# liuliu/ccv

Measured on AMD Instinct MI355X. Metric: images/sec fwd+bwd VGG-D 224x224 bs256, higher is better.
Workload: dtype f32 (Winograd-domain / fc GEMMs: exact bf16x3 split, all 9 products, fp32 accumulate); 1 GPU; VGG-D (ccv vgg_d_params, 225x225x3 crop, NHWC) forward+backward+SGD, batch 256 per GPU, random-init weights; global_batch=256, parallelism=dp1, conv_relu=convolution epilogue (NNC_MI355X_CONV_ALGO_FUSE_RELU)

## Files before the change

### ccv_amd/csrc/cmd_conv.cpp

```cpp
#include "gemm_launch.h"
#include "winograd.h"
#include "wino_fused.h"
#include "wino_wgrad_fused.h"
#include "conv_c3.h"

using namespace nnc;

namespace {

static size_t align256(size_t x) { return (x + 255) & ~(size_t)255; }

static thread_local int tl_relu_want = 0, tl_relu_done = 0;
static thread_local int tl_mask_want = 0, tl_mask_done = 0;
static thread_local Image4 tl_mask = { 0, 0, 0, 0, 0, 0, 0, 0, 0 };
static bool mask_fits(const Image4& dst)
{
	const Image4& m = tl_mask;
	return m.p && m.n == dst.n && m.h == dst.h && m.w == dst.w && m.c == dst.c && m.sc == 1 && aligned16(m.p) && m.sw % 4 == 0 && m.sh % 4 == 0 && (m.n == 1 || m.sn % 4 == 0);
}

struct conv_geom_t {
	int N, H, W, C;
	int OH, OW, K;
	int kh, kw, Cg, Kg, groups;
	int sy, sx, pby, pbx, dy, dx;
};

static bool conv_geometry(const ccv_nnc_cmd_t& cmd, const ccv_nnc_hint_t& hint, const Image4& a, const Image4& b, const ccv_nnc_tensor_t* w, conv_geom_t* g)
{
	g->N = a.n; g->H = a.h; g->W = a.w; g->C = a.c;
	g->OH = b.h; g->OW = b.w; g->K = b.c;
	g->groups = cmd.info.convolution.groups > 0 ? cmd.info.convolution.groups : 1;
	g->kh = cmd.info.size.dim[0]; g->kw = cmd.info.size.dim[1];
	if (g->K != cmd.info.convolution.count || g->K % g->groups || g->C % g->groups || a.n != b.n) return false;
	g->Cg = g->C / g->groups; g->Kg = g->K / g->groups;
	g->sy = hint.stride.dim[0] > 0 ? hint.stride.dim[0] : 1;
	g->sx = hint.stride.dim[1] > 0 ? hint.stride.dim[1] : 1;
	g->pby = hint.border.begin[0]; g->pbx = hint.border.begin[1];
	g->dy = cmd.info.convolution.dilation[0] > 1 ? cmd.info.convolution.dilation[0] : 1;
	g->dx = cmd.info.convolution.dilation[1] > 1 ? cmd.info.convolution.dilation[1] : 1;
	(void)w;
	return true;
}

static bool image_fits_int(const Image4& t)
{
	return (long)t.h * t.sh < 0x7fffffffL && (long)t.w * t.sw < 0x7fffffffL && (long)(t.h - 1) * t.sh + (long)(t.w - 1) * t.sw + t.c < 0x7fffffffL;
}

static bool pixel_linear(const Image4& t)
{
	return t.sc == 1 && t.sh == (long)t.w * t.sw && (t.n == 1 || t.sn == (long)t.h * t.sh);
}

static bool conv_pointwise(const conv_geom_t& g, const Image4& in, const Image4& out)
{
	return g.kh == 1 && g.kw == 1 && g.sy == 1 && g.sx == 1 && g.pby == 0 && g.pbx == 0 && g.groups == 1 && g.OH == g.H && g.OW == g.W && pixel_linear(in) && pixel_linear(out)
		&& (long)g.N * g.H * g.W <= 0x7fffffffL;
}

enum { CONV_ALGO_IMPLICIT_GEMM = 0, CONV_ALGO_WINOGRAD = 1, CONV_ALGO_WINOGRAD_FUSED = 2, CONV_ALGO_COUNT = 3 };

static unsigned blocks_exact(const size_t n, const int threads) { return (unsigned)((n + threads - 1) / threads); }

struct wino_plan_t {
	int TH, TW, T;
	size_t u_bytes, v_bytes, m_bytes;
	size_t total() const { return u_bytes + v_bytes + m_bytes; }
};

static bool wino_plan(const conv_geom_t& g, const int dst_h, const int dst_w, const int C_src, const int C_dst, wino_plan_t* p)
{
	if (g.kh != 3 || g.kw != 3 || g.sy != 1 || g.sx != 1 || g.dy != 1 || g.dx != 1 || g.groups != 1) return false;
	if (C_src % 4 || C_dst % 4 || g.pby < 0 || g.pby > 2 || g.pbx < 0 || g.pbx > 2) return false;
	p->TH = (dst_h + 3) / 4; p->TW = (dst_w + 3) / 4;
	const long T = (long)g.N * p->TH * p->TW;
	if (T <= 0 || T * (C_src > C_dst ? C_src : C_dst) > 0x7fffffffL) return false;
	p->T = (int)T;
	p->u_bytes = (sizeof(float) * 36 * (size_t)C_src * C_dst + 255) & ~(size_t)255;
	p->v_bytes = (sizeof(float) * 36 * (size_t)T * C_src + 255) & ~(size_t)255;
	p->m_bytes = (sizeof(float) * 36 * (size_t)T * C_dst + 255) & ~(size_t)255;
	return true;
}

static int wino_slice_images(const int N, const int tiles_per_image, const int C_src, const int C_dst)
{
	const long kb = tune(TUNE_WINO_SLICE_KB);
	if (kb <= 0) return N;
	const double per_image = 36.0 * sizeof(float) * (double)tiles_per_image * (double)(C_src + C_dst);
	long nb = (long)((double)kb * 1024.0 / per_image);
	if (nb < 1) nb = 1;
	return nb > N ? N : (int)nb;
}

template <bool FLIP>
static int conv_wino_run(const char* name, const conv_geom_t& g, const wino_plan_t& p, const Image4& src, const float* w, const float* bias, const Image4& dst, const int pad_y, const int pad_x, const int flags, ccv_nnc_stream_context_t* const ctx)
{
	const int Cs = src.c, Cd = dst.c;
	const int per_image = p.TH * p.TW;
	const int nb = wino_slice_images(g.N, per_image, Cs, Cd);
	const size_t v_bytes = nb == g.N ? p.v_bytes : (sizeof(float) * 36 * (size_t)nb * per_image * Cs + 255) & ~(size_t)255;
	const size_t m_bytes = nb == g.N ? p.m_bytes : (sizeof(float) * 36 * (size_t)nb * per_image * Cd + 255) & ~(size_t)255;
	char* ws = (char*)workspace_of(ctx, p.u_bytes + v_bytes + m_bytes);
	if (!ws) return CCV_NNC_EXEC_OOM;
	float* const U = (float*)ws;
	float* const V = (float*)(ws + p.u_bytes);
	float* const M = (float*)(ws + p.u_bytes + v_bytes);
	hipStream_t stream = stream_of(ctx);
	hipLaunchKernelGGL(HIP_KERNEL_NAME(wino_weight_kernel<FLIP>), dim3(blocks_exact((size_t)Cs * Cd, 256)), dim3(256), 0, stream, w, U, g.K, g.C);
	HIP_ENFORCE(hipGetLastError());
	for (int n0 = 0; n0 < g.N; n0 += nb) {
		const int ns = g.N - n0 < nb ? g.N - n0 : nb;
		const int T = ns * per_image;
		WinoTiles ti;
		ti.TH = p.TH; ti.TW = p.TW; ti.T = T;
		ti.H = src.h; ti.W = src.w; ti.sn = src.sn; ti.sh = src.sh; ti.sw = src.sw; ti.oy = -pad_y; ti.ox = -pad_x; ti.C4 = Cs / 4;
		ti.relu = (!FLIP && tl_relu_want) ? 1 : 0;
		if (ti.relu) tl_relu_done = 1;
		ti.mask = 0; ti.m_sn = ti.m_sh = ti.m_sw = 0;
		ti.d_c4.init(ti.C4); ti.d_tw.init(ti.TW); ti.d_th.init(ti.TH);
		hipLaunchKernelGGL(wino_input_kernel, dim3(blocks_exact((size_t)T * ti.C4, 256)), dim3(256), 0, stream, (const float*)src.p + (long)n0 * src.sn, V, ti);
		HIP_ENFORCE(hipGetLastError());
		MatLoader<true, true> la, lb;
		la.p = V; la.ldr = Cs; la.ldk = 1; la.R = T; la.K = Cs;
		lb.p = U; lb.ldr = Cs; lb.ldk = 1; lb.R = Cd; lb.K = Cs;
		GemmOut out = { M, Cd, 1, 0, 1.f, 0 };
		const int ret = gemm_run(name, la, lb, out, T, Cd, Cs, 36, (long)T * Cs, (long)Cd * Cs, (long)T * Cd, 0L, 1, flags, ctx);
		if (ret != CCV_NNC_EXEC_SUCCESS) return ret;
		ti.H = dst.h; ti.W = dst.w; ti.sn = dst.sn; ti.sh = dst.sh; ti.sw = dst.sw; ti.C4 = Cd / 4;
		ti.d_c4.init(ti.C4);
		if (FLIP && mask_fits(dst)) {
			ti.mask = tl_mask.p + (long)n0 * tl_mask.sn; ti.m_sn = tl_mask.sn; ti.m_sh = tl_mask.sh; ti.m_sw = tl_mask.sw;
			tl_mask_done = 1;
		}
		hipLaunchKernelGGL(wino_output_kernel, dim3(blocks_exact((size_t)T * ti.C4, 256)), dim3(256), 0, stream, (const float*)M, bias, dst.p + (long)n0 * dst.sn, ti);
		HIP_ENFORCE(hipGetLastError());
	}
	return CCV_NNC_EXEC_SUCCESS;
}

struct wino_fused_plan_t {
	int GH, GW, GYn, GXn, groups, KB, CCn;
	size_t uf_bytes;
};

static bool wino_fused_plan(const conv_geom_t& g, const Image4& src, const Image4& dst, wino_fused_plan_t* p)
{
	if (g.kh != 3 || g.kw != 3 || g.sy != 1 || g.sx != 1 || g.dy != 1 || g.dx != 1 || g.groups != 1) return false;
	if (src.c % WF_CC || src.c < 2 * WF_CC || src.sc != 1 || dst.sc != 1 || !aligned16(src.p) || src.sw % 4 || src.sh % 4 || (src.n > 1 && src.sn % 4)) return false;
	if (dst.c % 4 || !aligned16(dst.p) || dst.sw % 4 || dst.sh % 4 || (dst.n > 1 && dst.sn % 4)) return false;
	if (((long)(dst.h - 1) * dst.sh + (long)(dst.w - 1) * dst.sw + dst.c) * 4 >= (long)WF_OOB) return false;
	if (((long)(src.h - 1) * src.sh + (long)(src.w - 1) * src.sw + src.c) * 4 >= (long)WF_OOB) return false;
	const int TH = (dst.h + 3) / 4, TW = (dst.w + 3) / 4;
	static const int shapes[3][2] = { { 4, 4 }, { 2, 8 }, { 8, 2 } };
	long best = -1;
	for (int i = 0; i < 3; i++) {
		const long cover = (long)((TH + shapes[i][0] - 1) / shapes[i][0]) * ((TW + shapes[i][1] - 1) / shapes[i][1]);
		if (best < 0 || cover < best) { best = cover; p->GH = shapes[i][0]; p->GW = shapes[i][1]; }
	}
	p->GYn = (TH + p->GH - 1) / p->GH; p->GXn = (TW + p->GW - 1) / p->GW;
	const long groups = (long)src.n * p->GYn * p->GXn;
	p->KB = (dst.c + WF_KT - 1) / WF_KT; p->CCn = src.c / WF_CC;
	if (groups <= 0 || (groups + 3) / 4 * p->KB > 0x7fffffffL || (size_t)p->CCn * WF_U_FLOATS * 4 > 0xffffffffUL) return false;
	p->groups = (int)groups;
	p->uf_bytes = (sizeof(float) * (size_t)p->KB * p->CCn * WF_U_FLOATS + 255) & ~(size_t)255;
	return true;
}

static size_t wino_fused_scratch_bound(const int Kout, const int Cred)
{
	if (Cred % WF_CC || Kout <= 0) return 0;
	return ((sizeof(float) * (size_t)((Kout + WF_KT - 1) / WF_KT) * (Cred / WF_CC) * WF_U_FLOATS + 255) & ~(size_t)255);
}

static size_t wino_fused_mask_bound(const conv_geom_t& g)
{
	if (!tl_mask_want) return 0;
	const long TH = (g.H + 3) / 4, TW = (g.W + 3) / 4;
	long most = 0;
	static const int shapes[3][2] = { { 4, 4 }, { 2, 8 }, { 8, 2 } };
	for (int i = 0; i < 3; i++) {
		const long cover = ((TH + shapes[i][0] - 1) / shapes[i][0]) * ((TW + shapes[i][1] - 1) / shapes[i][1]);
		if (cover > most) most = cover;
	}
	return (size_t)g.N * most * ((g.C + WF_KT - 1) / WF_KT) * 1024;
}

template <bool FLIP>
static int conv_wino_fused_run(const char* name, const conv_geom_t& g, const wino_fused_plan_t& p, const Image4& src, const float* w, const float* bias, const Image4& dst, const int pad_y, const int pad_x, ccv_nnc_stream_context_t* const ctx)
{
	size_t bits_bytes = FLIP && mask_fits(dst) && (long)p.groups * p.KB <= 0x7fffffffL ? (size_t)p.groups * p.KB * 1024 : 0;
	float* UF = (float*)workspace_of(ctx, p.uf_bytes + bits_bytes);
	if (!UF && bits_bytes) { bits_bytes = 0; UF = (float*)workspace_of(ctx, p.uf_bytes); }
	if (!UF) return CCV_NNC_EXEC_OOM;
	hipStream_t stream = stream_of(ctx);
	unsigned* const bits = bits_bytes ? (unsigned*)((char*)UF + p.uf_bytes) : 0;
	if (bits) {
		const dim3 grid((unsigned)((long)p.groups * p.KB));
		const Image4& m = tl_mask;
		if (p.GH == 4) hipLaunchKernelGGL(HIP_KERNEL_NAME(wino_mask_pack_kernel<4, 4>), grid, dim3(256), 0, stream, (const float*)m.p, m.sn, m.sh, m.sw, bits, dst.h, dst.w, dst.c, p.GYn, p.GXn, p.KB);
		else if (p.GH == 2) hipLaunchKernelGGL(HIP_KERNEL_NAME(wino_mask_pack_kernel<2, 8>), grid, dim3(256), 0, stream, (const float*)m.p, m.sn, m.sh, m.sw, bits, dst.h, dst.w, dst.c, p.GYn, p.GXn, p.KB);
		else hipLaunchKernelGGL(HIP_KERNEL_NAME(wino_mask_pack_kernel<8, 2>), grid, dim3(256), 0, stream, (const float*)m.p, m.sn, m.sh, m.sw, bits, dst.h, dst.w, dst.c, p.GYn, p.GXn, p.KB);
		HIP_ENFORCE(hipGetLastError());
		tl_mask_done = 1;
	}
	const int Kout = dst.c, Cred = src.c;
	hipLaunchKernelGGL(HIP_KERNEL_NAME(wino_weight_frag_kernel<FLIP>), dim3(blocks_exact((size_t)p.KB * WF_KT * Cred, 256)), dim3(256), 0, stream, w, UF, Kout, Cred, g.K, g.C);
	HIP_ENFORCE(hipGetLastError());
	WinoFusedArgs a;
	a.src = src.p; a.dst = dst.p; a.uf = UF; a.bias = bias;
	a.s_sn = src.sn; a.s_sh = src.sh; a.s_sw = src.sw; a.d_sn = dst.sn; a.d_sh = dst.sh; a.d_sw = dst.sw;
	a.H = src.h; a.W = src.w; a.OH = dst.h; a.OW = dst.w; a.pad_y = pad_y; a.pad_x = pad_x;
	a.GYn = p.GYn; a.GXn = p.GXn; a.groups = p.groups; a.C = Cred; a.K = Kout; a.CCn = p.CCn; a.KB = p.KB;
	a.dst_image_bytes = (unsigned)(((long)(dst.h - 1) * dst.sh + (long)(dst.w - 1) * dst.sw + dst.c) * 4);
	a.src_image_bytes = (unsigned)(((long)(src.h - 1) * src.sh + (long)(src.w - 1) * src.sw + src.c) * 4);
	a.uf_kb_bytes = (unsigned)((size_t)p.CCn * WF_U_FLOATS * 4);
	long wgs = tune(TUNE_WINO_FUSED_GRID) > 0 ? tune(TUNE_WINO_FUSED_GRID) : device_cu_count();
	int team = p.KB % 8 == 0 ? 8 : (p.KB % 4 == 0 ? 4 : (p.KB % 2 == 0 ? 2 : 1));
	while (team > 1 && wgs < 8 * team) team >>= 1;
	if (wgs < 8 * team) wgs = 8 * team;
	const unsigned grid = (unsigned)(wgs / (8 * team) * (8 * team));
	a.team = team;
	a.relu = (!FLIP && tl_relu_want) ? 1 : 0;
	if (a.relu) tl_relu_done = 1;
	a.mask_bits = bits;
	note_kernel(name);
	char prof_name[96];
	snprintf(prof_name, sizeof(prof_name), bits ? "%s|nnc::wino_fused_kernel<%d, %d, 0, true>" : "%s|nnc::wino_fused_kernel<%d, %d>", name, p.GH, p.GW);
	const long T = (long)src.n * ((dst.h + 3) / 4) * ((dst.w + 3) / 4);
	ProfScope prof(prof_name, 2.0 * 36.0 * (double)T * Kout * Cred, 0, (int)T, Kout, Cred, 36, 1, stream);
	if (bits) {
		if (p.GH == 4) hipLaunchKernelGGL(HIP_KERNEL_NAME(wino_fused_kernel<4, 4, 0, true>), dim3(grid), dim3(256), 0, stream, a);
		else if (p.GH == 2) hipLaunchKernelGGL(HIP_KERNEL_NAME(wino_fused_kernel<2, 8, 0, true>), dim3(grid), dim3(256), 0, stream, a);
		else hipLaunchKernelGGL(HIP_KERNEL_NAME(wino_fused_kernel<8, 2, 0, true>), dim3(grid), dim3(256), 0, stream, a);
	} else if (p.GH == 4) hipLaunchKernelGGL(HIP_KERNEL_NAME(wino_fused_kernel<4, 4>), dim3(grid), dim3(256), 0, stream, a);
	else if (p.GH == 2) hipLaunchKernelGGL(HIP_KERNEL_NAME(wino_fused_kernel<2, 8>), dim3(grid), dim3(256), 0, stream, a);
	else hipLaunchKernelGGL(HIP_KERNEL_NAME(wino_fused_kernel<8, 2>), dim3(grid), dim3(256), 0, stream, a);
	HIP_ENFORCE(hipGetLastError());
	return CCV_NNC_EXEC_SUCCESS;
}

static bool wino_fused_preferred(const int C_red, const wino_fused_plan_t& p, const Image4& dst)
{
	const long maxc = tune(TUNE_WINO_FUSED_MAX_C);
	if (C_red <= maxc) return true;
	const long tiles = (long)((dst.h + 3) / 4) * ((dst.w + 3) / 4), padded = (long)p.GYn * p.GH * p.GXn * p.GW;
	return C_red <= 2 * maxc && padded * 5 < tiles * 6;
}

struct wino_wgrad_plan_t {
	wino_plan_t t;
	int splits;
	size_t w_bytes, du_bytes, head_bytes, bp_bytes;
	long blocks;
	size_t total() const { return head_bytes + t.v_bytes + w_bytes + du_bytes + bp_bytes; }
};

static bool wino_wgrad_plan(const conv_geom_t& g, wino_wgrad_plan_t* p)
{
	if (!wino_plan(g, g.OH, g.OW, g.C, g.K, &p->t)) return false;
	const long tiles = (long)((g.K + 127) / 128) * ((g.C + 127) / 128) * 36;
	long s = ((long)device_cu_count() * 8 + tiles - 1) / tiles;
	const long max_s = p->t.T / (GEMM_BK * 8);
	if (s > max_s) s = max_s;
	if (s > 64) s = 64;
	p->splits = s <= 1 ? 1 : (int)(((s < 8 ? 8 : s) + 7) & ~7);
	p->w_bytes = p->t.m_bytes;
	p->du_bytes = (sizeof(float) * 36 * (size_t)g.K * g.C + 255) & ~(size_t)255;
	p->head_bytes = p->splits > 1 ? sizeof(float) * 36 * (size_t)g.K * g.C * p->splits : 0;
	const size_t colsum_bound = sizeof(float) * (size_t)device_cu_count() * 4 * g.K;
	if (p->head_bytes < colsum_bound) p->head_bytes = colsum_bound;
	p->head_bytes = (p->head_bytes + 255) & ~(size_t)255;
	p->blocks = ((long)p->t.T * (g.K / 4) + 255) / 256;
	p->bp_bytes = sizeof(float) * (size_t)p->blocks * g.K;
	return true;
}

static int conv_wino_wgrad(const conv_geom_t& g, const wino_wgrad_plan_t& p, const Image4& gr, const Image4& a, float* dw, float* dbias, bool* bias_done, const int flags, ccv_nnc_stream_context_t* const ctx)
{
	char* ws = (char*)workspace_of(ctx, p.total());
	if (!ws) return CCV_NNC_EXEC_OOM;
	float* const V = (float*)(ws + p.head_bytes);
	float* const W = (float*)(ws + p.head_bytes + p.t.v_bytes);
	float* const dU = (float*)(ws + p.head_bytes + p.t.v_bytes + p.w_bytes);
	float* const BP = (float*)(ws + p.head_bytes + p.t.v_bytes + p.w_bytes + p.du_bytes);
	const bool fuse_bias = dbias && 256 % (g.K / 4) == 0;
	const int acc = (flags & CCV_NNC_ACCUMULATE_OUTPUT) ? 1 : 0;
	hipStream_t stream = stream_of(ctx);
	const int per_image = p.t.TH * p.t.TW;
	const int nb = wino_slice_images(g.N, per_image, g.C, g.K);
	for (int n0 = 0; n0 < g.N; n0 += nb) {
		const int ns = g.N - n0 < nb ? g.N - n0 : nb;
		const int T = ns * per_image;
		WinoTiles ti;
		ti.TH = p.t.TH; ti.TW = p.t.TW; ti.T = T;
		ti.H = a.h; ti.W = a.w; ti.sn = a.sn; ti.sh = a.sh; ti.sw = a.sw; ti.oy = -g.pby; ti.ox = -g.pbx; ti.C4 = g.C / 4;
		ti.d_c4.init(ti.C4); ti.d_tw.init(ti.TW); ti.d_th.init(ti.TH);
		hipLaunchKernelGGL(wino_input_kernel, dim3(blocks_exact((size_t)T * ti.C4, 256)), dim3(256), 0, stream, (const float*)a.p + (long)n0 * a.sn, V, ti);
		HIP_ENFORCE(hipGetLastError());
		ti.H = gr.h; ti.W = gr.w; ti.sn = gr.sn; ti.sh = gr.sh; ti.sw = gr.sw; ti.oy = 0; ti.ox = 0; ti.C4 = g.K / 4;
		ti.d_c4.init(ti.C4);
		const long blocks = ((long)T * (g.K / 4) + 255) / 256;
		const float* const grs = (const float*)gr.p + (long)n0 * gr.sn;
		if (fuse_bias) hipLaunchKernelGGL(HIP_KERNEL_NAME(wino_outgrad_kernel<true>), dim3((unsigned)blocks), dim3(256), 0, stream, grs, W, ti, BP);
		else hipLaunchKernelGGL(HIP_KERNEL_NAME(wino_outgrad_kernel<false>), dim3((unsigned)blocks), dim3(256), 0, stream, grs, W, ti, (float*)0);
		HIP_ENFORCE(hipGetLastError());
		MatLoader<false, true> la, lb;
		la.p = W; la.ldr = 1; la.ldk = g.K; la.R = g.K; la.K = T;
		lb.p = V; lb.ldr = 1; lb.ldk = g.C; lb.R = g.C; lb.K = T;
		GemmOut out = { dU, g.C, 1, 0, 1.f, n0 > 0 ? 1 : 0 };
		int splits = p.splits;
		if (nb < g.N) {
			const long max_s = T / (GEMM_BK * 8);
			if (splits > max_s) splits = max_s <= 1 ? 1 : (int)(max_s & ~7L);
			if (splits < 8) splits = 1;
		}
		const int ret = gemm_run("conv_wgrad_wino", la, lb, out, g.K, g.C, T, 36, (long)T * g.K, (long)T * g.C, (long)g.K * g.C, 0L, splits, flags, ctx);
		if (ret != CCV_NNC_EXEC_SUCCESS) return ret;
		if (fuse_bias) {
			const int r = colsum_f32(BP, blocks, g.K, g.K, dbias, acc || n0 > 0, ctx);
			if (r != CCV_NNC_EXEC_SUCCESS) return r;
		}
	}
	hipLaunchKernelGGL(wino_wgrad_final_kernel, dim3(blocks_exact((size_t)g.K * g.C, 256)), dim3(256), 0, stream, (const float*)dU, dw, g.K, g.C, acc);
	HIP_ENFORCE(hipGetLastError());
	if (bias_done) *bias_done = fuse_bias;
	return CCV_NNC_EXEC_SUCCESS;
}

struct wino_wgrad_fused_plan_t {
	int TH, TW, GYn, GXn, groups, kblocks, cblocks, slices, per_slice;
	size_t partial_bytes, bias_bytes, du_bytes;
	size_t total() const { return partial_bytes + bias_bytes + du_bytes; }
};
static bool wino_wgrad_fused_plan(const conv_geom_t& g, wino_wgrad_fused_plan_t* p)
{
	if (g.kh != 3 || g.kw != 3 || g.sy != 1 || g.sx != 1 || g.dy != 1 || g.dx != 1 || g.groups != 1) return false;
	if (g.C % WG_CB || g.K % WG_KB || g.pby < 0 || g.pby > 2 || g.pbx < 0 || g.pbx > 2) return false;
	p->TH = (g.OH + 3) / 4; p->TW = (g.OW + 3) / 4;
	p->GYn = (p->TH + WG_GH - 1) / WG_GH; p->GXn = (p->TW + WG_GW - 1) / WG_GW;
	const long groups = (long)g.N * p->GYn * p->GXn;
	if (groups <= 0 || groups > 0x7fffffffL) return false;
	p->groups = (int)groups;
	p->kblocks = g.K / WG_KB; p->cblocks = g.C / WG_CB;
	const long nb = (long)p->kblocks * p->cblocks;
	long s = (device_cu_count() / nb) & ~7L;
	if (s < 8) s = 8;
	while (s > 8 && (groups + s - 1) / s < 8) s -= 8;
	p->slices = (int)s;
	p->per_slice = (int)((groups + s - 1) / s);
	p->partial_bytes = (sizeof(float) * 36 * (size_t)s * g.K * g.C + 255) & ~(size_t)255;
	p->bias_bytes = (sizeof(float) * 4 * (size_t)s * g.K + 255) & ~(size_t)255;
	p->du_bytes = (sizeof(float) * 36 * (size_t)g.K * g.C + 255) & ~(size_t)255;
	return true;
}
static bool wino_wgrad_fused_images_ok(const Image4& a, const Image4& gr, const float* dw)
{
	const auto ok = [](const Image4& t) { return t.sc == 1 && aligned16(t.p) && t.sw % 4 == 0 && t.sh % 4 == 0 && (t.n == 1 || t.sn % 4 == 0) && ((long)(t.h - 1) * t.sh + (long)(t.w - 1) * t.sw + t.c) * 4 < 0x7ffff000L; };
	return ok(a) && ok(gr) && dw != 0;
}
static bool wino_wgrad_fused_preferred(const conv_geom_t& g)
{
	const long m = tune(TUNE_WINO_WGRAD_FUSED_MAX);
	return m > 0 && g.C <= m && g.K <= m;
}
static int conv_wino_wgrad_fused(const conv_geom_t& g, const wino_wgrad_fused_plan_t& p, const Image4& gr, const Image4& a, float* dw, float* dbias, bool* bias_done, const int flags, ccv_nnc_stream_context_t* const ctx)
{
	char* const ws = (char*)workspace_of(ctx, p.total());
	if (!ws) return CCV_NNC_EXEC_OOM;
	hipStream_t stream = stream_of(ctx);
	WinoWgradFusedArgs k;
	k.a = a.p; k.g = gr.p; k.partial = (float*)ws; k.bias_partial = dbias ? (float*)(ws + p.partial_bytes) : 0;
	k.a_sn = a.sn; k.a_sh = a.sh; k.a_sw = a.sw; k.g_sn = gr.sn; k.g_sh = gr.sh; k.g_sw = gr.sw;
	k.H = a.h; k.W = a.w; k.OH = gr.h; k.OW = gr.w; k.pad_y = g.pby; k.pad_x = g.pbx;
	k.GYn = p.GYn; k.GXn = p.GXn; k.groups = p.groups; k.C = g.C; k.K = g.K; k.kblocks = p.kblocks; k.cblocks = p.cblocks;
	k.slices = p.slices; k.per_slice = p.per_slice;
	k.a_image_bytes = (unsigned)(((long)(a.h - 1) * a.sh + (long)(a.w - 1) * a.sw + a.c) * 4);
	k.g_image_bytes = (unsigned)(((long)(gr.h - 1) * gr.sh + (long)(gr.w - 1) * gr.sw + gr.c) * 4);
	note_kernel("conv_wgrad_wino_fused");
	{
		const long T = (long)g.N * p.TH * p.TW;
		ProfScope prof("conv_wgrad_wino_fused|nnc::wino_wgrad_fused_kernel", 2.0 * 36.0 * (double)T * g.K * g.C, 0, g.K, g.C, (int)T, 36, p.slices, stream);
		hipLaunchKernelGGL(HIP_KERNEL_NAME(wino_wgrad_fused_kernel<0>), dim3((unsigned)(p.slices * p.kblocks * p.cblocks)), dim3(256), 0, stream, k);
		HIP_ENFORCE(hipGetLastError());
	}
	const long n = 36L * g.K * g.C;
	const int acc = (flags & CCV_NNC_ACCUMULATE_OUTPUT) ? 1 : 0;
	float* const dU = (float*)(ws + p.partial_bytes + p.bias_bytes);
	hipLaunchKernelGGL(wino_wgrad_fused_fold_kernel, dim3(blocks_exact((size_t)n, 256)), dim3(256), 0, stream, (const float*)k.partial, (const float*)k.bias_partial, dU, dbias, n, g.K, p.slices, acc);
	HIP_ENFORCE(hipGetLastError());
	hipLaunchKernelGGL(wino_wgrad_final_kernel, dim3(blocks_exact((size_t)g.K * g.C, 256)), dim3(256), 0, stream, (const float*)dU, dw, g.K, g.C, acc);
	HIP_ENFORCE(hipGetLastError());
	if (bias_done) *bias_done = dbias != 0;
	return CCV_NNC_EXEC_SUCCESS;
}

static bool wino_images_ok(const Image4& src, const Image4& dst, const float* w, const float* bias)
{
	return src.sc == 1 && dst.sc == 1 && aligned16(src.p) && aligned16(dst.p) && aligned16(w) && (!bias || aligned16(bias)) &&
		src.sw % 4 == 0 && src.sh % 4 == 0 && (src.n == 1 || src.sn % 4 == 0) && dst.sw % 4 == 0 && dst.sh % 4 == 0 && (dst.n == 1 || dst.sn % 4 == 0);
}

static bool wino_preferred(const wino_plan_t& p, const int C_src, const int C_dst)
{
	return C_src >= 32 && C_dst >= 32 && p.T >= 32;
}

static bool conv_c3_ok(const conv_geom_t& g, const Image4& a, const Image4& b)
{
	if (g.C != 3 || g.kh != 3 || g.kw != 3 || g.sy < 1 || g.sx < 1 || g.sy > 4 || g.sx > 4 || g.dy != 1 || g.dx != 1 || g.groups != 1) return false;
	if (g.K != 16 && g.K != 32 && g.K != 64) return false;
	if (a.sc != 1 || a.sw != 3 || b.sc != 1 || !aligned16(b.p) || b.sw % 4 || b.sh % 4 || (b.n > 1 && b.sn % 4)) return false;
	if ((long)a.h * a.sh >= 0x7fffffffL) return false;
	if (((long)(b.h - 1) * b.sh + (long)(b.w - 1) * b.sw + b.c) * 4 >= 0x7ffff000L) return false;
	return (long)b.n * b.h * ((b.w + 15) / 16) < 0x7fffffffL;
}
static void conv_c3_args(const conv_geom_t& g, const Image4& a, const float* w, const float* bias, const Image4& b, ConvC3Args* c)
{
	c->a = a.p; c->w = w; c->bias = bias; c->b = b.p;
	c->a_sn = a.sn; c->a_sh = a.sh; c->b_sn = b.sn; c->b_sh = b.sh; c->b_sw = b.sw;
	c->N = g.N; c->H = g.H; c->W = g.W; c->OH = g.OH; c->OW = g.OW; c->K = g.K; c->pad_y = g.pby; c->pad_x = g.pbx; c->sy = g.sy; c->sx = g.sx;
	c->groups_per_row = (g.OW + 15) / 16; c->groups = g.N * g.OH * c->groups_per_row;
	c->d_gpr.init(c->groups_per_row); c->d_oh.init(g.OH);
	c->b_image_bytes = (unsigned)((((long)b.h - 1) * b.sh + ((long)b.w - 1) * b.sw + b.c) * 4);
}
static int conv_c3_forw(const conv_geom_t& g, const Image4& a, const float* w, const float* bias, const Image4& b, ccv_nnc_stream_context_t* const ctx)
{
	ConvC3Args c;
	conv_c3_args(g, a, w, bias, b, &c);
	c.relu = tl_relu_want ? 1 : 0;
	if (c.relu) tl_relu_done = 1;
	hipStream_t stream = stream_of(ctx);
	const long want = ((long)c.groups + 3) / 4, cap = (long)device_cu_count() * 8;
	const unsigned grid = (unsigned)(want < cap ? want : cap);
	note_kernel("conv_fwd_c3");
	ProfScope prof("conv_fwd_c3|nnc::conv3x3_c3_fwd_kernel", 2.0 * g.N * g.OH * g.OW * (double)g.K * 27, 0, g.N * g.OH * g.OW, g.K, 27, 1, 1, stream);
	if (g.K == 64) hipLaunchKernelGGL(HIP_KERNEL_NAME(conv3x3_c3_fwd_kernel<4>), dim3(grid), dim3(256), 0, stream, c);
	else if (g.K == 32) hipLaunchKernelGGL(HIP_KERNEL_NAME(conv3x3_c3_fwd_kernel<2>), dim3(grid), dim3(256), 0, stream, c);
	else hipLaunchKernelGGL(HIP_KERNEL_NAME(conv3x3_c3_fwd_kernel<1>), dim3(grid), dim3(256), 0, stream, c);
	HIP_ENFORCE(hipGetLastError());
	return CCV_NNC_EXEC_SUCCESS;
}
static size_t conv_c3_wgrad_scratch_bound(const int K) { return sizeof(float) * (size_t)device_cu_count() * 4 * 4 * K * 32; }
static int conv_c3_wgrad(const conv_geom_t& g, const Image4& gr, const Image4& a, float* dw, float* dbias, const int flags, ccv_nnc_stream_context_t* const ctx)
{
	ConvC3Args c;
	conv_c3_args(g, a, 0, 0, gr, &c);
	const long want = ((long)c.groups + 3) / 4, cap = (long)device_cu_count() * 4;
	const unsigned grid = (unsigned)(want < cap ? want : cap);
	const int waves = (int)grid * 4;
	float* const part = (float*)workspace_of(ctx, sizeof(float) * (size_t)waves * g.K * 32);
	if (!part) return CCV_NNC_EXEC_OOM;
	hipStream_t stream = stream_of(ctx);
	note_kernel("conv_wgrad_c3");
	{
		ProfScope prof("conv_wgrad_c3|nnc::conv3x3_c3_wgrad_kernel", 2.0 * g.N * g.OH * g.OW * (double)g.K * 27, 0, g.K, 27, g.N * g.OH * g.OW, 1, 1, stream);
		if (g.K == 64) hipLaunchKernelGGL(HIP_KERNEL_NAME(conv3x3_c3_wgrad_kernel<4>), dim3(grid), dim3(256), 0, stream, c, part);
		else if (g.K == 32) hipLaunchKernelGGL(HIP_KERNEL_NAME(conv3x3_c3_wgrad_kernel<2>), dim3(grid), dim3(256), 0, stream, c, part);
		else hipLaunchKernelGGL(HIP_KERNEL_NAME(conv3x3_c3_wgrad_kernel<1>), dim3(grid), dim3(256), 0, stream, c, part);
	}
	HIP_ENFORCE(hipGetLastError());
	hipLaunchKernelGGL(convc3_wgrad_fold, dim3((unsigned)g.K), dim3(256), 0, stream, (const float*)part, (int)grid , g.K, dw, dbias, (flags & CCV_NNC_ACCUMULATE_OUTPUT) ? 1 : 0);
	HIP_ENFORCE(hipGetLastError());
	return CCV_NNC_EXEC_SUCCESS;
}

static int conv_forw_nhwc(const conv_geom_t& g, const Image4& a, const float* w, const float* bias, const Image4& b, const int algo, const int flags, ccv_nnc_stream_context_t* const ctx)
{
	if (a.sc != 1 || !pixel_linear(b) || !image_fits_int(a)) return CCV_NNC_EXEC_INVALID;
	if (algo != CONV_ALGO_IMPLICIT_GEMM && conv_c3_ok(g, a, b)) return conv_c3_forw(g, a, w, bias, b, ctx);
	wino_plan_t wp;
	wino_fused_plan_t fp;
	if (algo != CONV_ALGO_IMPLICIT_GEMM && algo != CONV_ALGO_WINOGRAD && g.pby <= 2 && g.pbx <= 2 && g.pby >= 0 && g.pbx >= 0 && wino_fused_plan(g, a, b, &fp) && (algo == CONV_ALGO_WINOGRAD_FUSED || wino_fused_preferred(g.C, fp, b))) {
		const int r = conv_wino_fused_run<false>("conv_fwd_wino_fused", g, fp, a, w, bias, b, g.pby, g.pbx, ctx);
		if (r != CCV_NNC_EXEC_OOM) return r;
	}
	if (algo != CONV_ALGO_IMPLICIT_GEMM && wino_plan(g, g.OH, g.OW, g.C, g.K, &wp) && wino_images_ok(a, b, w, bias) && (algo >= CONV_ALGO_WINOGRAD || wino_preferred(wp, g.C, g.K))) {
		const int r = conv_wino_run<false>("conv_fwd_wino", g, wp, a, w, bias, b, g.pby, g.pbx, flags, ctx);
		if (r != CCV_NNC_EXEC_OOM) return r;
	}
	const long M = (long)g.N * g.OH * g.OW;
	const int Kred = g.kh * g.kw * g.Cg;
	if (M > 0x7fffffffL) return CCV_NNC_EXEC_INVALID;
	const bool vec = (g.Cg % 4 == 0) && aligned16(a.p) && aligned16(w) && a.sw % 4 == 0 && a.sh % 4 == 0 && (a.n == 1 || a.sn % 4 == 0);
	GemmOut out = { b.p, b.sw, 1, bias, 1.f, 0 };
	if (vec && conv_pointwise(g, a, b)) {
		MatLoader<true, true> la, lb;
		la.p = a.p; la.ldr = a.sw; la.ldk = 1; la.R = (int)M; la.K = g.C;
		lb.p = w; lb.ldr = g.C; lb.ldk = 1; lb.R = g.K; lb.K = g.C;
		return gemm_run("conv_fwd_pointwise", la, lb, out, (int)M, g.K, g.C, 1, 0L, 0L, 0L, 0L, 1, flags, ctx);
	}
	KOrder ko;
	if (g.kh * g.kw > 1 && g.Cg % GEMM_BK == 0) ko.init(g.kh * g.kw, g.Cg);
#define CONV_FWD(VEC, INC) do { \
		Im2colKC<VEC, false, INC> la; \
		la.p = a.p; la.s_n = a.sn; la.s_h = (int)a.sh; la.s_w = (int)a.sw; la.H = g.H; la.W = g.W; \
		la.OW = g.OW; la.OHW = g.OH * g.OW; la.M = (int)M; la.C = g.Cg; la.KWC = g.kw * g.Cg; la.K = Kred; \
		la.my = g.sy; la.mx = g.sx; la.oy_off = -g.pby; la.ox_off = -g.pbx; la.ty = g.dy; la.tx = g.dx; la.dv_y = 1; la.dv_x = 1; \
		MatLoader<true, VEC> lb; \
		lb.p = w; lb.ldr = Kred; lb.ldk = 1; lb.R = g.Kg; lb.K = Kred; \
		return gemm_run("conv_fwd", la, lb, out, (int)M, g.Kg, Kred, g.groups, (long)g.Cg, (long)g.Kg * Kred, (long)g.Kg, (long)g.Kg, 1, flags, ctx, ko); \
	} while (0)
	if (vec) CONV_FWD(true, false);
	else CONV_FWD(false, false);
#undef CONV_FWD
}

static __global__ void __launch_bounds__(256) parity_filter_kernel(const float* __restrict__ w, float* __restrict__ f, const int K, const int C, const int kh, const int kw, const int ny, const int nx, const int ky_max, const int kx_max, const size_t total)
{
	for (size_t idx = (size_t)blockIdx.x * blockDim.x + threadIdx.x; idx < total; idx += (size_t)gridDim.x * blockDim.x) {
		size_t r = idx;
		const int k = (int)(r % K); r /= K;
		const int j = (int)(r % nx); r /= nx;
		const int i = (int)(r % ny); r /= ny;
		const int c = (int)r;
		f[idx] = w[(((size_t)k * kh + (ky_max - 2 * i)) * kw + (kx_max - 2 * j)) * C + c];
	}
}
static __global__ void __launch_bounds__(256) parity_scatter_kernel(const float* __restrict__ t, float* __restrict__ h, const int U, const int V, const int C4, const long h_sn, const long h_sh, const long h_sw, const int py, const int px, const size_t total)
{
	const int cn = C4 < 0 ? -C4 : C4;
	for (size_t idx = (size_t)blockIdx.x * blockDim.x + threadIdx.x; idx < total; idx += (size_t)gridDim.x * blockDim.x) {
		size_t r = idx;
		const int c = (int)(r % cn); r /= cn;
		const int v = (int)(r % V); r /= V;
		const int u = (int)(r % U); r /= U;
		const long o = (long)r * h_sn + (long)(2 * u + py) * h_sh + (long)(2 * v + px) * h_sw;
		if (C4 < 0) h[o + c] = t[idx];
		else *(float4*)(h + o + 4 * c) = ((const float4*)t)[idx];
	}
}
static bool conv_dgrad_parity_ok(const conv_geom_t& g)
{
	return g.sy == 2 && g.sx == 2 && g.dy == 1 && g.dx == 1 && g.groups == 1 && g.kh >= 1 && g.kw >= 1 && g.pby >= 0 && g.pbx >= 0 && g.pby < g.kh && g.pbx < g.kw && g.H >= 2 && g.W >= 2;
}
static size_t conv_dgrad_parity_prefix(const conv_geom_t& g)
{
	const size_t U = (g.H + 1) / 2, V = (g.W + 1) / 2;
	return align256(sizeof(float) * (size_t)g.N * U * V * g.C) + align256(sizeof(float) * (size_t)((g.kh + 1) / 2) * ((g.kw + 1) / 2) * g.C * g.K);
}
static size_t conv_dgrad_parity_scratch(const conv_geom_t& g)
{
	if (!conv_dgrad_parity_ok(g)) return 0;
	return conv_dgrad_parity_prefix(g) + gemm_workspace_bound((long)g.N * ((g.H + 1) / 2) * ((g.W + 1) / 2), g.C, (long)((g.kh + 1) / 2) * ((g.kw + 1) / 2) * g.K) + 256;
}
static int conv_forw_nhwc(const conv_geom_t& g, const Image4& a, const float* w, const float* bias, const Image4& b, const int algo, const int flags, ccv_nnc_stream_context_t* const ctx);
static int conv_dgrad_parity(const conv_geom_t& g, const Image4& gr, const float* w, const Image4& h, const int flags, ccv_nnc_stream_context_t* const ctx)
{
	const int U0 = (g.H + 1) / 2, V0 = (g.W + 1) / 2;
	const size_t tbytes = align256(sizeof(float) * (size_t)g.N * U0 * V0 * g.C);
	WorkspaceScope ws(ctx, conv_dgrad_parity_prefix(g), gemm_workspace_bound((long)g.N * U0 * V0, g.C, (long)((g.kh + 1) / 2) * ((g.kw + 1) / 2) * g.K));
	char* const p = (char*)ws.prefix();
	if (!p) return CCV_NNC_EXEC_OOM;
	float* const T = (float*)p;
	float* const Fw = (float*)(p + tbytes);
	hipStream_t stream = stream_of(ctx);
	const bool vec = g.C % 4 == 0 && aligned16(h.p) && h.sn % 4 == 0 && h.sh % 4 == 0 && h.sw % 4 == 0;
	for (int py = 0; py < 2; py++)
		for (int px = 0; px < 2; px++) {
			const int U = (g.H - py + 1) / 2, V = (g.W - px + 1) / 2;
			if (U <= 0 || V <= 0) continue;
			const int ky0 = (py + g.pby) & 1, kx0 = (px + g.pbx) & 1;
			const int ny = ky0 < g.kh ? (g.kh - ky0 + 1) / 2 : 0, nx = kx0 < g.kw ? (g.kw - kx0 + 1) / 2 : 0;
			const size_t cells = (size_t)g.N * U * V * (vec ? g.C / 4 : g.C);
			if (ny == 0 || nx == 0) {
				HIP_ENFORCE(hipMemsetAsync(T, 0, sizeof(float) * (size_t)g.N * U * V * g.C, stream));
			} else {
				const int ky_max = ky0 + 2 * (ny - 1), kx_max = kx0 + 2 * (nx - 1);
				const int pb_y = (ky_max - py - g.pby) / 2, pb_x = (kx_max - px - g.pbx) / 2;
				if (ky_max - py - g.pby < 0 || kx_max - px - g.pbx < 0) return CCV_NNC_EXEC_NO_KERNEL;
				const size_t fn = (size_t)g.C * ny * nx * g.K;
				hipLaunchKernelGGL(parity_filter_kernel, dim3(grid_for(fn, 256)), dim3(256), 0, stream, w, Fw, g.K, g.C, g.kh, g.kw, ny, nx, ky_max, kx_max, fn);
				HIP_ENFORCE(hipGetLastError());
				conv_geom_t q;
				q.N = g.N; q.H = g.OH; q.W = g.OW; q.C = g.K; q.OH = U; q.OW = V; q.K = g.C;
				q.kh = ny; q.kw = nx; q.Cg = g.K; q.Kg = g.C; q.groups = 1; q.sy = 1; q.sx = 1; q.pby = pb_y; q.pbx = pb_x; q.dy = 1; q.dx = 1;
				Image4 ti;
				ti.p = T; ti.n = g.N; ti.h = U; ti.w = V; ti.c = g.C; ti.sc = 1; ti.sw = g.C; ti.sh = (long)V * g.C; ti.sn = (long)U * V * g.C;
				const int r = conv_forw_nhwc(q, gr, Fw, 0, ti, CONV_ALGO_IMPLICIT_GEMM, flags & ~CCV_NNC_ACCUMULATE_OUTPUT, ctx);
				if (r != CCV_NNC_EXEC_SUCCESS) return r;
			}
			hipLaunchKernelGGL(parity_scatter_kernel, dim3(grid_for(cells, 256)), dim3(256), 0, stream, (const float*)T, h.p, U, V, vec ? g.C / 4 : -g.C, h.sn, h.sh, h.sw, py, px, cells);
			HIP_ENFORCE(hipGetLastError());
		}
	return CCV_NNC_EXEC_SUCCESS;
}

static int conv_dgrad_nhwc(const conv_geom_t& g, const Image4& gr, const float* w, const Image4& h, const int algo, const int flags, ccv_nnc_stream_context_t* const ctx)
{
	if (gr.sc != 1 || !pixel_linear(h) || !image_fits_int(gr)) return CCV_NNC_EXEC_INVALID;
	wino_plan_t wp;
	wino_fused_plan_t fp;
	if (algo != CONV_ALGO_IMPLICIT_GEMM && algo != CONV_ALGO_WINOGRAD && g.pby <= 2 && g.pbx <= 2 && g.pby >= 0 && g.pbx >= 0 && wino_fused_plan(g, gr, h, &fp) && (algo == CONV_ALGO_WINOGRAD_FUSED || wino_fused_preferred(g.K, fp, h))) {
		const int r = conv_wino_fused_run<true>("conv_dgrad_wino_fused", g, fp, gr, w, 0, h, 2 - g.pby, 2 - g.pbx, ctx);
		if (r != CCV_NNC_EXEC_OOM) return r;
	}
	if (algo != CONV_ALGO_IMPLICIT_GEMM && wino_plan(g, g.H, g.W, g.K, g.C, &wp) && wino_images_ok(gr, h, w, 0) && (algo >= CONV_ALGO_WINOGRAD || wino_preferred(wp, g.K, g.C))) {
		const int r = conv_wino_run<true>("conv_dgrad_wino", g, wp, gr, w, 0, h, 2 - g.pby, 2 - g.pbx, flags, ctx);
		if (r != CCV_NNC_EXEC_OOM) return r;
	}
	if (algo != CONV_ALGO_IMPLICIT_GEMM && !(flags & CCV_NNC_ACCUMULATE_OUTPUT) && conv_dgrad_parity_ok(g) && g.kh * g.kw > 1) {
		const int r = conv_dgrad_parity(g, gr, w, h, flags, ctx);
		if (r != CCV_NNC_EXEC_OOM && r != CCV_NNC_EXEC_NO_KERNEL) return r;
	}
	const long M = (long)g.N * g.H * g.W;
	const int Kred = g.kh * g.kw * g.Kg;
	if (M > 0x7fffffffL) return CCV_NNC_EXEC_INVALID;
	const bool vec = (g.Kg % 4 == 0) && (g.Cg % 4 == 0) && aligned16(gr.p) && aligned16(w) && gr.sw % 4 == 0 && gr.sh % 4 == 0 && (gr.n == 1 || gr.sn % 4 == 0);
	GemmOut out = { h.p, h.sw, 1, 0, 1.f, 0 };
	if (vec && conv_pointwise(g, h, gr)) {
		MatLoader<true, true> la;
		la.p = gr.p; la.ldr = gr.sw; la.ldk = 1; la.R = (int)M; la.K = g.K;
		MatLoader<false, true> lb;
		lb.p = w; lb.ldr = 1; lb.ldk = g.C; lb.R = g.C; lb.K = g.K;
		return gemm_run("conv_dgrad_pointwise", la, lb, out, (int)M, g.C, g.K, 1, 0L, 0L, 0L, 0L, 1, flags, ctx);
	}
	KOrder ko;
	if (g.kh * g.kw > 1 && g.Kg % GEMM_BK == 0) ko.init(g.kh * g.kw, g.Kg);
#define CONV_DGRAD(VEC, STRIDED, INC) do { \
		Im2colKC<VEC, STRIDED, INC> la; \
		la.p = gr.p; la.s_n = gr.sn; la.s_h = (int)gr.sh; la.s_w = (int)gr.sw; la.H = g.OH; la.W = g.OW; \
		la.OW = g.W; la.OHW = g.H * g.W; la.M = (int)M; la.C = g.Kg; la.KWC = g.kw * g.Kg; la.K = Kred; \
		la.my = 1; la.mx = 1; la.oy_off = g.pby; la.ox_off = g.pbx; la.ty = -g.dy; la.tx = -g.dx; la.dv_y = g.sy; la.dv_x = g.sx; \
		WgtDgradNC<VEC, INC> lb; \
		lb.p = w; lb.ko_stride = (long)g.kh * g.kw * g.Cg; lb.C = g.Cg; lb.Ko = g.Kg; lb.K = Kred; \
		return gemm_run("conv_dgrad", la, lb, out, (int)M, g.Cg, Kred, g.groups, (long)g.Kg, (long)g.Kg * g.kh * g.kw * g.Cg, (long)g.Cg, 0L, 1, flags, ctx, ko); \
	} while (0)
	if (g.sy != 1 || g.sx != 1) { if (vec) CONV_DGRAD(true, true, false); else CONV_DGRAD(false, true, false); }
	else { if (vec) CONV_DGRAD(true, false, false); else CONV_DGRAD(false, false, false); }
#undef CONV_DGRAD
}

static int conv_wgrad_nhwc(const conv_geom_t& g, const Image4& gr, const Image4& a, float* dw, float* dbias, bool* bias_done, const int algo, const int flags, ccv_nnc_stream_context_t* const ctx)
{
	if (bias_done) *bias_done = false;
	if (a.sc != 1 || !pixel_linear(gr) || !image_fits_int(a)) return CCV_NNC_EXEC_INVALID;
	if (algo != CONV_ALGO_IMPLICIT_GEMM && conv_c3_ok(g, a, gr)) {
		const int r = conv_c3_wgrad(g, gr, a, dw, dbias, flags, ctx);
		if (r == CCV_NNC_EXEC_SUCCESS && bias_done) *bias_done = dbias != 0;
		if (r != CCV_NNC_EXEC_OOM) return r;
	}
	wino_wgrad_fused_plan_t wfp;
	if (algo != CONV_ALGO_IMPLICIT_GEMM && algo != CONV_ALGO_WINOGRAD && wino_wgrad_fused_plan(g, &wfp) && wino_wgrad_fused_images_ok(a, gr, dw) && wino_wgrad_fused_preferred(g)) {
		const int r = conv_wino_wgrad_fused(g, wfp, gr, a, dw, dbias, bias_done, flags, ctx);
		if (r != CCV_NNC_EXEC_OOM) return r;
	}
	wino_wgrad_plan_t wp;
	if (algo != CONV_ALGO_IMPLICIT_GEMM && wino_wgrad_plan(g, &wp) && wino_images_ok(a, gr, dw, 0) && (algo >= CONV_ALGO_WINOGRAD || wino_preferred(wp.t, g.C, g.K))) {
		const int r = conv_wino_wgrad(g, wp, gr, a, dw, dbias, bias_done, flags, ctx);
		if (r != CCV_NNC_EXEC_OOM) return r;
	}
	const long P = (long)g.N * g.OH * g.OW;
	if (P > 0x7fffffffL) return CCV_NNC_EXEC_INVALID;
	const int NN = g.kh * g.kw * g.Cg;
	const bool vec = (g.Cg % 4 == 0) && (g.Kg % 4 == 0) && aligned16(a.p) && aligned16(gr.p) && a.sw % 4 == 0 && a.sh % 4 == 0 && (a.n == 1 || a.sn % 4 == 0) && gr.sw % 4 == 0;
	GemmOut out = { dw, (long)NN, 1, 0, 1.f, (flags & CCV_NNC_ACCUMULATE_OUTPUT) ? 1 : 0 };
	if (vec && conv_pointwise(g, a, gr)) {
		MatLoader<false, true> la, lb;
		la.p = gr.p; la.ldr = 1; la.ldk = gr.sw; la.R = g.K; la.K = (int)P;
		lb.p = a.p; lb.ldr = 1; lb.ldk = a.sw; lb.R = g.C; lb.K = (int)P;
		return gemm_run("conv_wgrad_pointwise", la, lb, out, g.K, g.C, (int)P, 1, 0L, 0L, 0L, 0L, 0, flags, ctx);
	}
#define CONV_WGRAD(VEC, INC) do { \
		MatLoader<false, VEC> la; \
		la.p = gr.p; la.ldr = 1; la.ldk = gr.sw; la.R = g.Kg; la.K = (int)P; \
		Im2colNC<VEC, INC> lb; \
		lb.p = a.p; lb.s_n = a.sn; lb.s_h = (int)a.sh; lb.s_w = (int)a.sw; lb.H = g.H; lb.W = g.W; lb.OW = g.OW; lb.OHW = g.OH * g.OW; \
		lb.C = g.Cg; lb.KWC = g.kw * g.Cg; lb.NN = NN; lb.K = (int)P; lb.sy = g.sy; lb.sx = g.sx; lb.py = g.pby; lb.px = g.pbx; lb.dy = g.dy; lb.dx = g.dx; \
		return gemm_run("conv_wgrad", la, lb, out, g.Kg, NN, (int)P, g.groups, (long)g.Kg, (long)g.Cg, (long)g.Kg * NN, 0L, 0, flags, ctx); \
	} while (0)
	if (vec) CONV_WGRAD(true, false);
	else CONV_WGRAD(false, false);
#undef CONV_WGRAD
}

template <class T> struct conv1x1_types;
template <> struct conv1x1_types<float> { typedef GemmOut Out; };
template <> struct conv1x1_types<half_t> { typedef GemmOutH Out; };
template <class LA, class LB> static int conv1x1_run(const char* name, float*, LA la, LB lb, const GemmOut out, int M, int N, int K, int z, long a_z, long b_z, long c_z, int splits, int flags, ccv_nnc_stream_context_t* ctx) { return gemm_run(name, la, lb, out, M, N, K, z, a_z, b_z, c_z, 0L, splits, flags, ctx); }
template <class LA, class LB> static int conv1x1_run(const char* name, half_t*, LA la, LB lb, const GemmOutH out, int M, int N, int K, int z, long a_z, long b_z, long c_z, int splits, int flags, ccv_nnc_stream_context_t* ctx) { return gemm_run_h(name, la, lb, out, M, N, K, z, a_z, b_z, c_z, 0L, splits, flags, ctx); }

static bool nchw_dense(const ccv_nnc_tensor_t* t, int* N, int* C, int* P)
{
	if (t->info.format != CCV_TENSOR_FORMAT_NCHW || !tensor_contiguous(t)) return false;
	const int nd = tensor_nd(t->info.dim);
	if (nd != 3 && nd != 4) return false;
	const int b = nd == 4;
	*N = b ? t->info.dim[0] : 1; *C = t->info.dim[b]; *P = t->info.dim[b + 1] * t->info.dim[b + 2];
	return true;
}
static bool conv1x1_cmd_ok(const ccv_nnc_cmd_t& cmd, const ccv_nnc_hint_t& hint)
{
	if (cmd.info.size.dim[0] != 1 || cmd.info.size.dim[1] != 1 || cmd.info.convolution.groups > 1) return false;
	for (int i = 0; i < 2; i++)
		if ((hint.stride.dim[i] > 1) || hint.border.begin[i] != 0 || hint.border.end[i] != 0) return false;
	return true;
}
template <class T> static bool chunk_aligned(const void* p) { return (((uintptr_t)p) & (4 * sizeof(T) - 1)) == 0; }

template <class T>
static int conv1x1_nchw_forw(const ccv_nnc_cmd_t cmd, const ccv_nnc_hint_t hint, const int flags, const ccv_nnc_tensor_t* a, const ccv_nnc_tensor_t* w, const ccv_nnc_tensor_t* bias, ccv_nnc_tensor_t* b, ccv_nnc_stream_context_t* const ctx)
{
	typedef typename conv1x1_types<T>::Out Out;
	int N, C, P, Nb, K, Pb;
	if (!conv1x1_cmd_ok(cmd, hint) || !nchw_dense(a, &N, &C, &P) || !nchw_dense(b, &Nb, &K, &Pb) || N != Nb || P != Pb) return CCV_NNC_EXEC_NO_KERNEL;
	if (K != cmd.info.convolution.count || !tensor_contiguous(w) || (long)tensor_count(w->info) != (long)K * C || (bias && (!tensor_contiguous(bias) || (int)tensor_count(bias->info) != K))) return CCV_NNC_EXEC_NO_KERNEL;
	if (P % 4 || C % 4 || ((long)C * P) % 4 || !chunk_aligned<T>(a->data.u8) || !chunk_aligned<T>(w->data.u8) || N <= 0 || P <= 0) return CCV_NNC_EXEC_NO_KERNEL;
	MatLoader<true, true> la;
	la.p = (const float*)w->data.u8; la.ldr = C; la.ldk = 1; la.R = K; la.K = C;
	MatLoader<false, true> lb;
	lb.p = (const float*)a->data.u8; lb.ldr = 1; lb.ldk = P; lb.R = P; lb.K = C;
	Out out = { (T*)b->data.u8, (long)P, 1, bias ? (const T*)bias->data.u8 : 0, 1.f, 0, 1 };
	out.bias_ldn = 0;
	return conv1x1_run("conv1x1_nchw_fwd", (T*)0, la, lb, out, K, P, C, N, 0L, (long)C * P, (long)K * P, 1, flags, ctx);
}

template <class T>
static int conv1x1_nchw_back(const ccv_nnc_cmd_t cmd, const ccv_nnc_hint_t hint, const int flags, const ccv_nnc_tensor_t* g, const ccv_nnc_tensor_t* a, const ccv_nnc_tensor_t* w, ccv_nnc_tensor_t* h, ccv_nnc_tensor_t* dw, ccv_nnc_tensor_t* dbias, ccv_nnc_stream_context_t* const ctx)
{
	typedef typename conv1x1_types<T>::Out Out;
	int N, K, P;
	if (!conv1x1_cmd_ok(cmd, hint) || !nchw_dense(g, &N, &K, &P) || K != cmd.info.convolution.count) return CCV_NNC_EXEC_NO_KERNEL;
	const ccv_nnc_tensor_t* shape_src = a ? a : h;
	int Na, C, Pa;
	if (!shape_src || !nchw_dense(shape_src, &Na, &C, &Pa) || Na != N || Pa != P) return CCV_NNC_EXEC_NO_KERNEL;
	if (h && (!nchw_dense(h, &Na, &C, &Pa) || Na != N || Pa != P || !w || !tensor_contiguous(w) || (long)tensor_count(w->info) != (long)K * C)) return CCV_NNC_EXEC_NO_KERNEL;
	if (dw && (!a || !tensor_contiguous(dw) || (long)tensor_count(dw->info) != (long)K * C)) return CCV_NNC_EXEC_NO_KERNEL;
	if (dbias && (!tensor_contiguous(dbias) || (int)tensor_count(dbias->info) != K)) return CCV_NNC_EXEC_NO_KERNEL;
	if (P % 4 || C % 4 || K % 4 || !chunk_aligned<T>(g->data.u8) || (a && !chunk_aligned<T>(a->data.u8)) || (w && !chunk_aligned<T>(w->data.u8)) || (long)N * P > 0x7fffffffL) return CCV_NNC_EXEC_NO_KERNEL;
	const int acc = (flags & CCV_NNC_ACCUMULATE_OUTPUT) ? 1 : 0;
	int ret;
	if (dw) {
		PlaneKC<true> la, lb;
		la.p = (const float*)g->data.u8; la.ldr = P; la.s_n = (long)K * P; la.R = K; la.K = N * P; la.P = P;
		lb.p = (const float*)a->data.u8; lb.ldr = P; lb.s_n = (long)C * P; lb.R = C; lb.K = N * P; lb.P = P;
		Out out = { (T*)dw->data.u8, (long)C, 1, 0, 1.f, acc, 0 };
		if ((ret = conv1x1_run("conv1x1_nchw_wgrad", (T*)0, la, lb, out, K, C, N * P, 1, 0L, 0L, 0L, 0, flags, ctx)) != CCV_NNC_EXEC_SUCCESS) return ret;
	}
	if (dbias && (ret = (sizeof(T) == sizeof(float) ? chan_sum_planes(g->data.f32, N, K, P, dbias->data.f32, acc, ctx) : chan_sum_planes_f16(g->data.u8, N, K, P, dbias->data.u8, acc, ctx))) != CCV_NNC_EXEC_SUCCESS) return ret;
	if (h) {
		MatLoader<false, true> la;
		la.p = (const float*)w->data.u8; la.ldr = 1; la.ldk = C; la.R = C; la.K = K;
		MatLoader<false, true> lb;
		lb.p = (const float*)g->data.u8; lb.ldr = 1; lb.ldk = P; lb.R = P; lb.K = K;
		Out out = { (T*)h->data.u8, (long)P, 1, 0, 1.f, 0, 0 };
		if ((ret = conv1x1_run("conv1x1_nchw_dgrad", (T*)0, la, lb, out, C, P, K, N, 0L, (long)K * P, (long)C * P, 1, flags, ctx)) != CCV_NNC_EXEC_SUCCESS) return ret;
	}
	return CCV_NNC_EXEC_SUCCESS;
}


static bool weights_shape(const ccv_nnc_tensor_t* w, int* K, int* kh, int* kw, int* Cg)
{
	if (!w || tensor_nd(w->info.dim) != 4 || !tensor_contiguous(w)) return false;
	const int* d = w->info.dim;
	if (w->info.format == CCV_TENSOR_FORMAT_NCHW) { *K = d[0]; *Cg = d[1]; *kh = d[2]; *kw = d[3]; }
	else if (w->info.format == CCV_TENSOR_FORMAT_NHWC) { *K = d[0]; *kh = d[1]; *kw = d[2]; *Cg = d[3]; }
	else return false;
	return true;
}

static void dense_nhwc_like(const ccv_nnc_tensor_t* like, const Image4& li, float* data, ccv_nnc_tensor_t* out)
{
	memset(out, 0, sizeof(*out));
	out->type = like->info.type & ~CCV_TENSOR_VIEW;
	out->info = like->info;
	out->info.format = CCV_TENSOR_FORMAT_NHWC;
	const int b = tensor_nd(like->info.dim) == 4;
	memset(out->info.dim, 0, sizeof(out->info.dim));
	if (b) out->info.dim[0] = li.n;
	out->info.dim[b] = li.h; out->info.dim[b + 1] = li.w; out->info.dim[b + 2] = li.c;
	out->data.f32 = data;
}

static int _conv_forw(const ccv_nnc_cmd_t cmd, const ccv_nnc_hint_t hint, const int flags, ccv_nnc_tensor_t* const* const inputs, const int input_size, ccv_nnc_tensor_t* const* const outputs, const int output_size, ccv_nnc_stream_context_t* const stream_context)
{
	if (input_size < 2 || output_size < 1 || !inputs[0] || !inputs[1] || !outputs[0]) return CCV_NNC_EXEC_INVALID;
	const ccv_nnc_tensor_t* a = inputs[0];
	const ccv_nnc_tensor_t* w = inputs[1];
	const ccv_nnc_tensor_t* bias = input_size > 2 ? inputs[2] : 0;
	ccv_nnc_tensor_t* b = outputs[0];
	if (CCV_GET_DATA_TYPE(a->info.datatype) != CCV_32F) return CCV_NNC_EXEC_INVALID;
	if (a->info.format != b->info.format) return CCV_NNC_EXEC_INVALID;
	if (a->info.format == CCV_TENSOR_FORMAT_NCHW && cmd.algorithm != CONV_ALGO_IMPLICIT_GEMM) {
		const int r = conv1x1_nchw_forw<float>(cmd, hint, flags, a, w, bias, b, stream_context);
		if (r != CCV_NNC_EXEC_NO_KERNEL) return r;
	}
	Image4 ai, bi;
	if (!image4(a, &ai) || !image4(b, &bi)) return CCV_NNC_EXEC_INVALID;
	int K, kh, kw, Cg;
	if (!weights_shape(w, &K, &kh, &kw, &Cg)) return CCV_NNC_EXEC_INVALID;
	conv_geom_t g;
	if (!conv_geometry(cmd, hint, ai, bi, 0, &g) || K != g.K || kh != g.kh || kw != g.kw || Cg != g.Cg) return CCV_NNC_EXEC_INVALID;
	if (bias && (bias->info.dim[0] != g.K || !tensor_contiguous(bias))) return CCV_NNC_EXEC_INVALID;
	const bool stage_io = a->info.format == CCV_TENSOR_FORMAT_NCHW, stage_w = w->info.format == CCV_TENSOR_FORMAT_NCHW;
	if (!stage_io && !stage_w) return conv_forw_nhwc(g, ai, w->data.f32, bias ? bias->data.f32 : 0, bi, cmd.algorithm, flags, stream_context);
	const size_t na = stage_io ? align256(sizeof(float) * tensor_count(a->info)) : 0, nb = stage_io ? align256(sizeof(float) * tensor_count(b->info)) : 0;
	const size_t nw = stage_w ? align256(sizeof(float) * tensor_count(w->info)) : 0;
	size_t inner = gemm_workspace_bound((long)g.N * g.OH * g.OW, g.Kg, (long)g.kh * g.kw * g.Cg);
	wino_plan_t wpl;
	if (cmd.algorithm != CONV_ALGO_IMPLICIT_GEMM && wino_plan(g, g.OH, g.OW, g.C, g.K, &wpl) && wpl.total() > inner) inner = wpl.total();
	if (cmd.algorithm != CONV_ALGO_IMPLICIT_GEMM && wino_fused_scratch_bound(g.K, g.C) > inner) inner = wino_fused_scratch_bound(g.K, g.C);
	WorkspaceScope ws(stream_context, na + nb + nw, inner);
	char* p = (char*)ws.prefix();
	if (!p) return CCV_NNC_EXEC_OOM;
	int ret;
	const float* wp = w->data.f32;
	if (stage_w) {
		if ((ret = weights_nchw_to_nhwc(w->data.f32, (float*)(p + na + nb), g.K, g.Cg, g.kh * g.kw, stream_context)) != CCV_NNC_EXEC_SUCCESS) return ret;
		wp = (const float*)(p + na + nb);
	}
	if (!stage_io) return conv_forw_nhwc(g, ai, wp, bias ? bias->data.f32 : 0, bi, cmd.algorithm, flags, stream_context);
	ccv_nnc_tensor_t at, bt;
	dense_nhwc_like(a, ai, (float*)p, &at);
	dense_nhwc_like(b, bi, (float*)(p + na), &bt);
	if ((ret = format_transform(a, &at, stream_context)) != CCV_NNC_EXEC_SUCCESS) return ret;
	Image4 as, bs;
	image4(&at, &as); image4(&bt, &bs);
	if ((ret = conv_forw_nhwc(g, as, wp, bias ? bias->data.f32 : 0, bs, cmd.algorithm, flags, stream_context)) != CCV_NNC_EXEC_SUCCESS) return ret;
	return format_transform(&bt, b, stream_context);
}

static int _conv_back(const ccv_nnc_cmd_t cmd, const ccv_nnc_hint_t hint, const int flags, ccv_nnc_tensor_t* const* const inputs, const int input_size, ccv_nnc_tensor_t* const* const outputs, const int output_size, ccv_nnc_stream_context_t* const stream_context)
{
	if (input_size < 2 || output_size < 1 || !inputs[0]) return CCV_NNC_EXEC_INVALID;
	const ccv_nnc_tensor_t* gt = inputs[0];
	const ccv_nnc_tensor_t* a = inputs[1];
	const ccv_nnc_tensor_t* w = input_size > 2 ? inputs[2] : 0;
	ccv_nnc_tensor_t* h = outputs[0];
	ccv_nnc_tensor_t* dw = output_size > 1 ? outputs[1] : 0;
	ccv_nnc_tensor_t* dbias = output_size > 2 ? outputs[2] : 0;
	if (CCV_GET_DATA_TYPE(gt->info.datatype) != CCV_32F) return CCV_NNC_EXEC_INVALID;
	if (gt->info.format == CCV_TENSOR_FORMAT_NCHW && cmd.algorithm != CONV_ALGO_IMPLICIT_GEMM) {
		const int r = conv1x1_nchw_back<float>(cmd, hint, flags, gt, a, w, h, dw, dbias, stream_context);
		if (r != CCV_NNC_EXEC_NO_KERNEL) return r;
	}
	Image4 gi;
	if (!image4(gt, &gi)) return CCV_NNC_EXEC_INVALID;
	const ccv_nnc_tensor_t* shape_src = a ? a : h;
	if (!shape_src || shape_src->info.format != gt->info.format) return CCV_NNC_EXEC_INVALID;
	Image4 ai;
	if (!image4(shape_src, &ai)) return CCV_NNC_EXEC_INVALID;
	const ccv_nnc_tensor_t* wshape = dw ? dw : w;
	int K, kh, kw, Cg;
	if (!weights_shape(wshape, &K, &kh, &kw, &Cg)) return CCV_NNC_EXEC_INVALID;
	if (w && dw && w->info.format != dw->info.format) return CCV_NNC_EXEC_INVALID;
	conv_geom_t g;
	if (!conv_geometry(cmd, hint, ai, gi, 0, &g) || K != g.K || kh != g.kh || kw != g.kw || Cg != g.Cg) return CCV_NNC_EXEC_INVALID;
	if (dw && !a) return CCV_NNC_EXEC_INVALID;
	if (h && (!w || !tensor_contiguous(w))) return CCV_NNC_EXEC_INVALID;
	Image4 hi;
	if (h && (!image4(h, &hi) || hi.h != g.H || hi.w != g.W || hi.c != g.C || hi.n != g.N || h->info.format != gt->info.format)) return CCV_NNC_EXEC_INVALID;
	if (dbias && (!tensor_contiguous(dbias) || dbias->info.dim[0] != g.K)) return CCV_NNC_EXEC_INVALID;
	const int acc = (flags & CCV_NNC_ACCUMULATE_OUTPUT) ? 1 : 0;
	const bool stage_io = gt->info.format == CCV_TENSOR_FORMAT_NCHW, stage_w = wshape->info.format == CCV_TENSOR_FORMAT_NCHW;
	const size_t wbytes = align256(sizeof(float) * (size_t)g.K * g.kh * g.kw * g.Cg);
	const size_t ng = stage_io ? align256(sizeof(float) * tensor_count(gt->info)) : 0;
	const size_t na = stage_io && a && dw ? align256(sizeof(float) * tensor_count(a->info)) : 0;
	const size_t nh = stage_io && h ? align256(sizeof(float) * tensor_count(h->info)) : 0;
	const size_t nw = stage_w && h ? wbytes : 0, ndw = stage_w && dw ? wbytes : 0;
	const long P = (long)g.N * g.OH * g.OW;
	size_t inner = gemm_workspace_bound(g.Kg, (long)g.kh * g.kw * g.Cg, P);
	const size_t inner_d = gemm_workspace_bound((long)g.N * g.H * g.W, g.Cg, (long)g.kh * g.kw * g.Kg), inner_b = sizeof(float) * (size_t)g.K * 4096;
	if (inner_d > inner) inner = inner_d;
	if (inner_b > inner) inner = inner_b;
	wino_plan_t wpl;
	if (h && cmd.algorithm != CONV_ALGO_IMPLICIT_GEMM && wino_plan(g, g.H, g.W, g.K, g.C, &wpl) && wpl.total() > inner) inner = wpl.total();
	wino_wgrad_plan_t wgp;
	if (dw && cmd.algorithm != CONV_ALGO_IMPLICIT_GEMM && wino_wgrad_plan(g, &wgp) && wgp.total() > inner) inner = wgp.total();
	wino_wgrad_fused_plan_t wfgp;
	if (dw && cmd.algorithm != CONV_ALGO_IMPLICIT_GEMM && wino_wgrad_fused_plan(g, &wfgp) && wfgp.total() > inner) inner = wfgp.total();
	if (h && cmd.algorithm != CONV_ALGO_IMPLICIT_GEMM && wino_fused_scratch_bound(g.C, g.K) + wino_fused_mask_bound(g) > inner) inner = wino_fused_scratch_bound(g.C, g.K) + wino_fused_mask_bound(g);
	if (h && cmd.algorithm != CONV_ALGO_IMPLICIT_GEMM && conv_dgrad_parity_scratch(g) > inner) inner = conv_dgrad_parity_scratch(g);
	if (dw && cmd.algorithm != CONV_ALGO_IMPLICIT_GEMM && g.C == 3 && conv_c3_wgrad_scratch_bound(g.K) > inner) inner = conv_c3_wgrad_scratch_bound(g.K);
	WorkspaceScope ws(stream_context, ng + na + nh + nw + ndw, inner);
	char* p = (char*)ws.prefix();
	if ((ng + na + nh + nw + ndw) && !p) return CCV_NNC_EXEC_OOM;
	int ret;
	ccv_nnc_tensor_t gs, as, hs;
	Image4 gim = gi, aim = ai, him = hi;
	if (stage_io) {
		dense_nhwc_like(gt, gi, (float*)p, &gs);
		if ((ret = format_transform(gt, &gs, stream_context)) != CCV_NNC_EXEC_SUCCESS) return ret;
		image4(&gs, &gim);
		if (na) {
			dense_nhwc_like(a, ai, (float*)(p + ng), &as);
			if ((ret = format_transform(a, &as, stream_context)) != CCV_NNC_EXEC_SUCCESS) return ret;
			image4(&as, &aim);
		}
		if (nh) { dense_nhwc_like(h, hi, (float*)(p + ng + na), &hs); image4(&hs, &him); }
	}
	bool bias_done = false;
	if (dw) {
		float* dwp = dw->data.f32;
		if (stage_w) {
			dwp = (float*)(p + ng + na + nh + nw);
			if (acc && (ret = weights_nchw_to_nhwc(dw->data.f32, dwp, g.K, g.Cg, g.kh * g.kw, stream_context)) != CCV_NNC_EXEC_SUCCESS) return ret;
		}
		if ((ret = conv_wgrad_nhwc(g, gim, aim, dwp, dbias ? dbias->data.f32 : 0, &bias_done, cmd.algorithm, flags, stream_context)) != CCV_NNC_EXEC_SUCCESS) return ret;
		if (stage_w && (ret = weights_nhwc_to_nchw(dwp, dw->data.f32, g.K, g.Cg, g.kh * g.kw, stream_context)) != CCV_NNC_EXEC_SUCCESS) return ret;
	}
	if (dbias && !bias_done) {
		if (!pixel_linear(gim)) return CCV_NNC_EXEC_INVALID;
		if ((ret = colsum_f32(gim.p, P, g.K, gim.sw, dbias->data.f32, acc, stream_context)) != CCV_NNC_EXEC_SUCCESS) return ret;
	}
	if (h) {
		const float* wp = w->data.f32;
		if (stage_w) {
			if ((ret = weights_nchw_to_nhwc(w->data.f32, (float*)(p + ng + na + nh), g.K, g.Cg, g.kh * g.kw, stream_context)) != CCV_NNC_EXEC_SUCCESS) return ret;
			wp = (const float*)(p + ng + na + nh);
		}
		if (tl_mask_want) tl_mask = aim;
		ret = conv_dgrad_nhwc(g, gim, wp, him, cmd.algorithm, flags, stream_context);
		tl_mask.p = 0;
		if (ret != CCV_NNC_EXEC_SUCCESS) return ret;
		if (stage_io && (ret = format_transform(&hs, h, stream_context)) != CCV_NNC_EXEC_SUCCESS) return ret;
	}
	return CCV_NNC_EXEC_SUCCESS;
}

static __global__ void __launch_bounds__(256) chan_bias_add_kernel(float* b, const float* bias, const size_t n, const int C, const long inner)
{
	const size_t stride = (size_t)gridDim.x * blockDim.x;
	for (size_t i = (size_t)blockIdx.x * blockDim.x + threadIdx.x; i < n; i += stride) b[i] += bias[(int)((inner == 1 ? i : i / inner) % C)];
}
static int _conv_transpose_forw(const ccv_nnc_cmd_t cmd, const ccv_nnc_hint_t hint, const int flags, ccv_nnc_tensor_t* const* const inputs, const int input_size, ccv_nnc_tensor_t* const* const outputs, const int output_size, ccv_nnc_stream_context_t* const stream_context)
{
	if (input_size < 2 || output_size < 1 || !inputs[0] || !inputs[1] || !outputs[0]) return CCV_NNC_EXEC_INVALID;
	ccv_nnc_tensor_t* a = inputs[0];
	ccv_nnc_tensor_t* w = inputs[1];
	ccv_nnc_tensor_t* bias = input_size > 2 ? inputs[2] : 0;
	ccv_nnc_tensor_t* b = outputs[0];
	Image4 ai, bi;
	if (!image4(a, &ai) || !image4(b, &bi) || a->info.format != b->info.format || !tensor_contiguous(b)) return CCV_NNC_EXEC_INVALID;
	if (bi.c != cmd.info.convolution.count) return CCV_NNC_EXEC_INVALID;
	ccv_nnc_cmd_t conv = cmd;
	conv.cmd = CCV_NNC_CONVOLUTION_BACKWARD;
	conv.info.convolution.count = ai.c;
	ccv_nnc_tensor_t* ins[3] = { a, 0, w };
	ccv_nnc_tensor_t* outs[1] = { b };
	const int ret = _conv_back(conv, hint, flags & ~CCV_NNC_ACCUMULATE_OUTPUT, ins, 3, outs, 1, stream_context);
	if (ret != CCV_NNC_EXEC_SUCCESS) return ret;
	if (bias) {
		if (!tensor_contiguous(bias) || (int)tensor_count(bias->info) != bi.c) return CCV_NNC_EXEC_INVALID;
		const size_t n = tensor_count(b->info);
		const long inner = b->info.format == CCV_TENSOR_FORMAT_NCHW ? (long)bi.h * bi.w : 1;
		hipLaunchKernelGGL(chan_bias_add_kernel, dim3(grid_for(n, 256)), dim3(256), 0, stream_of(stream_context), b->data.f32, (const float*)bias->data.f32, n, bi.c, inner);
		HIP_ENFORCE(hipGetLastError());
	}
	return CCV_NNC_EXEC_SUCCESS;
}

static bool aligned8(const void* p) { return (((uintptr_t)p) & 7) == 0; }
static bool half_image_ok(const Image4& t) { return t.sc == 1 && aligned8(t.p) && t.sw % 4 == 0 && t.sh % 4 == 0 && (t.n == 1 || t.sn % 4 == 0) && image_fits_int(t); }

static bool conv_h_small_tiles(const conv_geom_t& g, const long M, const int N, const int Kred)
{
	if (g.groups != 1 || g_force_tile || g_force_splits) return false;
	const long tiles = ((M + 127) / 128) * ((N + 127) / 128);
	return tiles <= (long)device_cu_count() && Kred >= 2304;
}
static int conv_h_splits(const conv_geom_t& g, const long M, const int N, const int Kred)
{
	return g.groups == 1 && g_force_splits > 1 ? g_force_splits : 1;
}

static bool conv_h_planar_ok(const conv_geom_t& g, const long M, const int N, const int Kred, const long P, const void* dst)
{
	return tune(TUNE_GEMM_VEC_EPILOGUE) == 1 && g.groups == 1 && P % 4 == 0 && M % 4 == 0 && aligned8(dst) && conv_h_splits(g, M, N, Kred) == 1 && M * (long)N < 0x7fffffff0L && M <= 0x7fffffffL;
}

static double conv_h_bytes(const conv_geom_t& g) { return 2.0 * ((double)g.N * g.H * g.W * g.C + (double)g.K * g.kh * g.kw * g.Cg + (double)g.N * g.OH * g.OW * g.K); }
static int conv_forw_h(const conv_geom_t& g, const Image4& a, const void* w, const void* bias, const Image4& b, const int flags, ccv_nnc_stream_context_t* const ctx, void* const planar = 0)
{
	prof_next_bytes(conv_h_bytes(g));
	const long M = (long)g.N * g.OH * g.OW;
	const int Kred = g.kh * g.kw * g.Cg;
	GemmOutH out = { (half_t*)b.p, b.sw, 1, (const half_t*)bias, 1.f, 0, 0 };
	KOrder ko;
	if (g.kh * g.kw > 1 && g.Cg % GEMM_BK == 0) ko.init(g.kh * g.kw, g.Cg);
	Im2colKC<true, false, false> la;
	la.p = a.p; la.s_n = a.sn; la.s_h = (int)a.sh; la.s_w = (int)a.sw; la.H = g.H; la.W = g.W;
	la.OW = g.OW; la.OHW = g.OH * g.OW; la.M = (int)M; la.C = g.Cg; la.KWC = g.kw * g.Cg; la.K = Kred;
	la.my = g.sy; la.mx = g.sx; la.oy_off = -g.pby; la.ox_off = -g.pbx; la.ty = g.dy; la.tx = g.dx; la.dv_y = 1; la.dv_x = 1;
	MatLoader<true, true> lb;
	lb.p = (const float*)w; lb.ldr = Kred; lb.ldk = 1; lb.R = g.Kg; lb.K = Kred;
	if (!planar && g.C % 8 == 0 && a.sw % 8 == 0 && conv_pointwise(g, a, b)) {
		MatLoader<true, true> pa;
		pa.p = a.p; pa.ldr = a.sw; pa.ldk = 1; pa.R = (int)M; pa.K = g.C;
		return gemm_run_h("conv_fwd_h_pointwise", pa, lb, out, (int)M, g.K, g.C, 1, 0L, 0L, 0L, 0L, 1, flags, ctx);
	}
	if (planar) {
		EpiStoreHT epi;
		epi.c = (half_t*)planar; epi.bias = (const half_t*)bias; epi.M = (int)M; epi.N = g.Kg; epi.P = g.OH * g.OW;
		return gemm_run_h_planar("conv_fwd_h", la, lb, epi, Kred, ctx, ko, conv_h_small_tiles(g, M, g.Kg, Kred));
	}
	return gemm_run_h("conv_fwd_h", la, lb, out, (int)M, g.Kg, Kred, g.groups, (long)g.Cg, (long)g.Kg * Kred, (long)g.Kg, (long)g.Kg, conv_h_splits(g, M, g.Kg, Kred), flags, ctx, ko, conv_h_small_tiles(g, M, g.Kg, Kred));
}

static int conv_dgrad_h(const conv_geom_t& g, const Image4& gr, const void* w, const Image4& h, const int flags, ccv_nnc_stream_context_t* const ctx, void* const planar = 0)
{
	prof_next_bytes(conv_h_bytes(g));
	const long M = (long)g.N * g.H * g.W;
	const int Kred = g.kh * g.kw * g.Kg;
	GemmOutH out = { (half_t*)h.p, h.sw, 1, 0, 1.f, 0, 0 };
	if (!planar && g.C % 8 == 0 && g.K % 8 == 0 && gr.sw % 8 == 0 && conv_pointwise(g, h, gr)) {
		MatLoader<true, true> pa;
		pa.p = gr.p; pa.ldr = gr.sw; pa.ldk = 1; pa.R = (int)M; pa.K = g.K;
		MatLoader<false, true> pb;
		pb.p = (const float*)w; pb.ldr = 1; pb.ldk = g.C; pb.R = g.C; pb.K = g.K;
		return gemm_run_h("conv_dgrad_h_pointwise", pa, pb, out, (int)M, g.C, g.K, 1, 0L, 0L, 0L, 0L, 1, flags, ctx);
	}
	KOrder ko;
	if (g.kh * g.kw > 1 && g.Kg % GEMM_BK == 0) ko.init(g.kh * g.kw, g.Kg);
#define CONV_DGRAD_H(STRIDED) do { \
		Im2colKC<true, STRIDED, false> la; \
		la.p = gr.p; la.s_n = gr.sn; la.s_h = (int)gr.sh; la.s_w = (int)gr.sw; la.H = g.OH; la.W = g.OW; \
		la.OW = g.W; la.OHW = g.H * g.W; la.M = (int)M; la.C = g.Kg; la.KWC = g.kw * g.Kg; la.K = Kred; \
		la.my = 1; la.mx = 1; la.oy_off = g.pby; la.ox_off = g.pbx; la.ty = -g.dy; la.tx = -g.dx; la.dv_y = g.sy; la.dv_x = g.sx; \
		WgtDgradNC<true, false> lb; \
		lb.p = (const float*)w; lb.ko_stride = (long)g.kh * g.kw * g.Cg; lb.C = g.Cg; lb.Ko = g.Kg; lb.K = Kred; \
		if (planar) { \
			EpiStoreHT epi; \
			epi.c = (half_t*)planar; epi.bias = 0; epi.M = (int)M; epi.N = g.Cg; epi.P = g.H * g.W; \
			return gemm_run_h_planar("conv_dgrad_h", la, lb, epi, Kred, ctx, ko, conv_h_small_tiles(g, M, g.Cg, Kred)); \
		} \
		return gemm_run_h("conv_dgrad_h", la, lb, out, (int)M, g.Cg, Kred, g.groups, (long)g.Kg, (long)g.Kg * g.kh * g.kw * g.Cg, (long)g.Cg, 0L, conv_h_splits(g, M, g.Cg, Kred), flags, ctx, ko, conv_h_small_tiles(g, M, g.Cg, Kred)); \
// ... 210 lines not shown
		const int r = conv1x1_nchw_back<half_t>(cmd, hint, flags, gt, a, w, h, dw, dbias, stream_context);
		return r != CCV_NNC_EXEC_NO_KERNEL ? r : conv_nchw_half_back(cmd, hint, flags, gt, a, w, h, dw, dbias, stream_context);
	}
	if (gt->info.format != CCV_TENSOR_FORMAT_NHWC || shape_src->info.format != CCV_TENSOR_FORMAT_NHWC || wshape->info.format != CCV_TENSOR_FORMAT_NHWC || (w && w->info.format != CCV_TENSOR_FORMAT_NHWC) || (h && h->info.format != CCV_TENSOR_FORMAT_NHWC)) return CCV_NNC_EXEC_NO_KERNEL;
	Image4 gi, ai, hi;
	if (!image4(gt, &gi) || !image4(shape_src, &ai)) return CCV_NNC_EXEC_NO_KERNEL;
	int K, kh, kw, Cg;
	if (!weights_shape(wshape, &K, &kh, &kw, &Cg)) return CCV_NNC_EXEC_NO_KERNEL;
	conv_geom_t g;
	if (!conv_geometry(cmd, hint, ai, gi, 0, &g) || K != g.K || kh != g.kh || kw != g.kw || Cg != g.Cg) return CCV_NNC_EXEC_INVALID;
	if (dw && !a) return CCV_NNC_EXEC_INVALID;
	if (h && (!w || !tensor_contiguous(w))) return CCV_NNC_EXEC_INVALID;
	if (h && (!image4(h, &hi) || hi.h != g.H || hi.w != g.W || hi.c != g.C || hi.n != g.N)) return CCV_NNC_EXEC_INVALID;
	if (dbias && (!tensor_contiguous(dbias) || dbias->info.dim[0] != g.K)) return CCV_NNC_EXEC_INVALID;
	if (g.Cg % 4 || g.Kg % 4 || !half_image_ok(gi) || !pixel_linear(gi) || (long)g.N * g.OH * g.OW > 0x7fffffffL || (long)g.N * g.H * g.W > 0x7fffffffL) return CCV_NNC_EXEC_NO_KERNEL;
	if (dw && (!half_image_ok(ai) || !aligned8(dw->data.u8))) return CCV_NNC_EXEC_NO_KERNEL;
	if (h && (!pixel_linear(hi) || !aligned8(w->data.u8) || !aligned8(hi.p))) return CCV_NNC_EXEC_NO_KERNEL;
	int ret;
	if (dw && (ret = conv_wgrad_h(g, gi, ai, dw->data.u8, flags, stream_context)) != CCV_NNC_EXEC_SUCCESS) return ret;
	if (dbias && (ret = colsum_f16(gi.p, (long)g.N * g.OH * g.OW, g.K, gi.sw, dbias->data.u8, (flags & CCV_NNC_ACCUMULATE_OUTPUT) ? 1 : 0, stream_context)) != CCV_NNC_EXEC_SUCCESS) return ret;
	if (h && (ret = conv_dgrad_h(g, gi, w->data.u8, hi, flags, stream_context)) != CCV_NNC_EXEC_SUCCESS) return ret;
	return CCV_NNC_EXEC_SUCCESS;
}

static bool all_half(ccv_nnc_tensor_t* const* const inputs, const int input_size, ccv_nnc_tensor_t* const* const outputs, const int output_size)
{
	for (int i = 0; i < input_size + output_size; i++) {
		const ccv_nnc_tensor_t* t = i < input_size ? inputs[i] : outputs[i - input_size];
		if (t && CCV_GET_DATA_TYPE(t->info.datatype) != CCV_16F) return false;
	}
	return true;
}

static int conv_forw_dispatch(const ccv_nnc_cmd_t cmd, const ccv_nnc_hint_t hint, const int flags, ccv_nnc_tensor_t* const* const inputs, const int input_size, ccv_nnc_tensor_t* const* const outputs, const int output_size, ccv_nnc_stream_context_t* const stream_context)
{
	if (!any_half_tensor(inputs, input_size, outputs, output_size)) return _conv_forw(cmd, hint, flags, inputs, input_size, outputs, output_size, stream_context);
	if (all_half(inputs, input_size, outputs, output_size)) {
		const int r = _conv_forw_half(cmd, hint, flags, inputs, input_size, outputs, output_size, stream_context);
		if (r != CCV_NNC_EXEC_NO_KERNEL) return r;
	}
	return half_staged_exec(_conv_forw, cmd, hint, flags, inputs, input_size, outputs, output_size, stream_context);
}
static int conv_forw_entry(const ccv_nnc_cmd_t cmd, const ccv_nnc_hint_t hint, const int flags, ccv_nnc_tensor_t* const* const inputs, const int input_size, ccv_nnc_tensor_t* const* const outputs, const int output_size, ccv_nnc_stream_context_t* const stream_context);
static int _conv_forw_any(const ccv_nnc_cmd_t cmd, const ccv_nnc_hint_t hint, const int flags, ccv_nnc_tensor_t* const* const inputs, const int input_size, ccv_nnc_tensor_t* const* const outputs, const int output_size, ccv_nnc_stream_context_t* const stream_context)
{
	uint64_t sig;
	if (const int e = deferred_take_error(stream_context)) return e;
	if (deferred_try(_conv_forw_any, DEFER_CONV_FORWARD, cmd, hint, flags, inputs, input_size, outputs, output_size, stream_context, &sig)) return CCV_NNC_EXEC_SUCCESS;
	const int r = conv_forw_entry(cmd, hint, flags, inputs, input_size, outputs, output_size, stream_context);
	if (r == CCV_NNC_EXEC_SUCCESS) deferred_mark_good(sig);
	return r;
}
static int conv_forw_entry(const ccv_nnc_cmd_t cmd, const ccv_nnc_hint_t hint, const int flags, ccv_nnc_tensor_t* const* const inputs, const int input_size, ccv_nnc_tensor_t* const* const outputs, const int output_size, ccv_nnc_stream_context_t* const stream_context)
{
	MarkerScope marker(cmd.cmd);
	if (cmd.algorithm < 0 || !(cmd.algorithm & NNC_MI355X_CONV_ALGO_FUSE_RELU)) return conv_forw_dispatch(cmd, hint, flags, inputs, input_size, outputs, output_size, stream_context);
	if (flags & CCV_NNC_ACCUMULATE_OUTPUT) return CCV_NNC_EXEC_INVALID;
	ccv_nnc_cmd_t plain = cmd;
	plain.algorithm = (cmd.algorithm & 0xff) == 0xff ? -1 : (cmd.algorithm & 0xff);
	tl_relu_want = 1; tl_relu_done = 0;
	const int r = conv_forw_dispatch(plain, hint, flags, inputs, input_size, outputs, output_size, stream_context);
	const int done = tl_relu_done;
	tl_relu_want = 0; tl_relu_done = 0;
	if (r != CCV_NNC_EXEC_SUCCESS || done) return r;
	return relu_inplace(outputs[0], stream_context);
}
static int conv_back_dispatch(const ccv_nnc_cmd_t cmd, const ccv_nnc_hint_t hint, const int flags, ccv_nnc_tensor_t* const* const inputs, const int input_size, ccv_nnc_tensor_t* const* const outputs, const int output_size, ccv_nnc_stream_context_t* const stream_context);
static int conv_back_entry(const ccv_nnc_cmd_t cmd, const ccv_nnc_hint_t hint, const int flags, ccv_nnc_tensor_t* const* const inputs, const int input_size, ccv_nnc_tensor_t* const* const outputs, const int output_size, ccv_nnc_stream_context_t* const stream_context);
static int _conv_back_any(const ccv_nnc_cmd_t cmd, const ccv_nnc_hint_t hint, const int flags, ccv_nnc_tensor_t* const* const inputs, const int input_size, ccv_nnc_tensor_t* const* const outputs, const int output_size, ccv_nnc_stream_context_t* const stream_context)
{
	uint64_t sig;
	if (const int e = deferred_take_error(stream_context)) return e;
	if (deferred_try(_conv_back_any, DEFER_CONV_BACKWARD, cmd, hint, flags, inputs, input_size, outputs, output_size, stream_context, &sig)) return CCV_NNC_EXEC_SUCCESS;
	const int r = conv_back_entry(cmd, hint, flags, inputs, input_size, outputs, output_size, stream_context);
	if (r == CCV_NNC_EXEC_SUCCESS) deferred_mark_good(sig);
	return r;
}
static int conv_back_report(const int r, const int flags, ccv_nnc_tensor_t* const* const outputs, const int output_size, ccv_nnc_stream_context_t* const stream_context)
{
	if (r == CCV_NNC_EXEC_SUCCESS && g_comm_overlap_on.load(std::memory_order_relaxed))
	{
		if (flags & CCV_NNC_ACCUMULATE_OUTPUT) { for (int i = 1; i < output_size && i < 3; i++) comm_gradient_touched(outputs[i]); }
		else if (output_size > 1) comm_gradients_written(outputs + 1, output_size > 3 ? 2 : output_size - 1, stream_context);
	}
	return r;
}
static int conv_back_entry(const ccv_nnc_cmd_t cmd, const ccv_nnc_hint_t hint, const int flags, ccv_nnc_tensor_t* const* const inputs, const int input_size, ccv_nnc_tensor_t* const* const outputs, const int output_size, ccv_nnc_stream_context_t* const stream_context)
{
	MarkerScope marker(cmd.cmd);
	if (cmd.algorithm < 0 || !(cmd.algorithm & NNC_MI355X_CONV_ALGO_FUSE_RELU)) return conv_back_report(conv_back_dispatch(cmd, hint, flags, inputs, input_size, outputs, output_size, stream_context), flags, outputs, output_size, stream_context);
	ccv_nnc_cmd_t plain = cmd;
	plain.algorithm = (cmd.algorithm & 0xff) == 0xff ? -1 : (cmd.algorithm & 0xff);
	ccv_nnc_tensor_t* const h = output_size > 0 ? outputs[0] : 0;
	const ccv_nnc_tensor_t* const a = input_size > 1 ? inputs[1] : 0;
	if (!h) return conv_back_report(conv_back_dispatch(plain, hint, flags, inputs, input_size, outputs, output_size, stream_context), flags, outputs, output_size, stream_context);
	if ((flags & CCV_NNC_ACCUMULATE_OUTPUT) || !a || !tensor_contiguous(h) || !tensor_contiguous(a) || h->info.datatype != a->info.datatype || h->info.format != a->info.format || tensor_count(h->info) != tensor_count(a->info)) return CCV_NNC_EXEC_INVALID;
	tl_mask_want = 1; tl_mask_done = 0;
	const int r = conv_back_report(conv_back_dispatch(plain, hint, flags, inputs, input_size, outputs, output_size, stream_context), flags, outputs, output_size, stream_context);
	const int done = tl_mask_done;
	tl_mask_want = 0; tl_mask_done = 0; tl_mask.p = 0;
	if (r != CCV_NNC_EXEC_SUCCESS || done) return r;
	return relu_back_inplace(h, a, stream_context);
}
static int conv_back_dispatch(const ccv_nnc_cmd_t cmd, const ccv_nnc_hint_t hint, const int flags, ccv_nnc_tensor_t* const* const inputs, const int input_size, ccv_nnc_tensor_t* const* const outputs, const int output_size, ccv_nnc_stream_context_t* const stream_context)
{
	if (!any_half_tensor(inputs, input_size, outputs, output_size)) return _conv_back(cmd, hint, flags, inputs, input_size, outputs, output_size, stream_context);
	if (all_half(inputs, input_size, outputs, output_size)) {
		const int r = _conv_back_half(cmd, hint, flags, inputs, input_size, outputs, output_size, stream_context);
		if (r != CCV_NNC_EXEC_NO_KERNEL) return r;
	}
	return half_staged_exec(_conv_back, cmd, hint, flags, inputs, input_size, outputs, output_size, stream_context);
}

static int _conv_autotune(const ccv_nnc_cmd_t cmd, const size_t max_workspace_size, const ccv_nnc_hint_t hint, const int flags, ccv_nnc_tensor_t* const* const inputs, const int input_size, ccv_nnc_tensor_t* const* const outputs, const int output_size, ccv_nnc_stream_context_t* const stream_context)
{
	(void)max_workspace_size;
	if (any_half_tensor(inputs, input_size, outputs, output_size)) return -1;
	if (any_palettized(inputs, input_size)) return -1;
	{
		static int trials = -1;
		if (trials < 0) { const char* e = getenv("NNC_MI355X_CONV_AUTOTUNE"); trials = (e && *e == '0') ? 0 : 1; }
		if (!trials) return -1;
	}
	const bool fwd = cmd.cmd == CCV_NNC_CONVOLUTION_FORWARD;
	hipStream_t stream = stream_of(stream_context);
	hipEvent_t e0, e1;
	HIP_ENFORCE(hipEventCreate(&e0));
	HIP_ENFORCE(hipEventCreate(&e1));
	int best = 0, have_best = 0;
	float best_ms = 0;
	const int trial_flags = flags & ~CCV_NNC_ACCUMULATE_OUTPUT;
	for (int algo = 0; algo < CONV_ALGO_COUNT; algo++) {
		ccv_nnc_cmd_t c = cmd;
		c.algorithm = algo;
		float ms = 0;
		int ok = 1;
		for (int trial = 0; trial < 2 && ok; trial++) {
			HIP_ENFORCE(hipEventRecord(e0, stream));
			const int ret = fwd ? _conv_forw(c, hint, trial_flags, inputs, input_size, outputs, output_size, stream_context) : _conv_back(c, hint, trial_flags, inputs, input_size, outputs, output_size, stream_context);
			HIP_ENFORCE(hipEventRecord(e1, stream));
			HIP_ENFORCE(hipEventSynchronize(e1));
			if (ret != CCV_NNC_EXEC_SUCCESS) ok = 0;
			else HIP_ENFORCE(hipEventElapsedTime(&ms, e0, e1));
		}
		if (ok && (!have_best || ms < best_ms)) { best = algo; best_ms = ms; have_best = 1; }
	}
	HIP_ENFORCE(hipEventDestroy(e0));
	HIP_ENFORCE(hipEventDestroy(e1));
	return best;
}

}

extern "C" void _register_command_CCV_NNC_CONVOLUTION_FORWARD_backend_CCV_NNC_BACKEND_GPU_CUDNN(ccv_nnc_cmd_backend_registry_t* const registry)
{
	registry->tensor_formats = CCV_TENSOR_FORMAT_NCHW | CCV_TENSOR_FORMAT_NHWC;
	registry->tensor_datatypes = CCV_32F | CCV_16F;
	registry->tensor_memory = CCV_TENSOR_GPU_MEMORY;
	registry->algorithms = CONV_ALGO_COUNT;
	registry->exec = _conv_forw_any;
	registry->autotune = _conv_autotune;
	NNC_DEPALETTIZED(registry, _conv_forw_any);
}

extern "C" void _register_command_CCV_NNC_CONVOLUTION_BACKWARD_backend_CCV_NNC_BACKEND_GPU_CUDNN(ccv_nnc_cmd_backend_registry_t* const registry)
{
	registry->tensor_formats = CCV_TENSOR_FORMAT_NCHW | CCV_TENSOR_FORMAT_NHWC;
	registry->tensor_datatypes = CCV_32F | CCV_16F;
	registry->tensor_memory = CCV_TENSOR_GPU_MEMORY;
	registry->algorithms = CONV_ALGO_COUNT;
	registry->exec = _conv_back_any;
	registry->autotune = _conv_autotune;
	NNC_DEPALETTIZED(registry, _conv_back_any);
}

extern "C" void _register_command_CCV_NNC_CONVOLUTION_TRANSPOSE_FORWARD_backend_CCV_NNC_BACKEND_GPU_CUDNN(ccv_nnc_cmd_backend_registry_t* const registry)
{
	registry->tensor_formats = CCV_TENSOR_FORMAT_NCHW | CCV_TENSOR_FORMAT_NHWC;
	registry->tensor_datatypes = CCV_32F;
	registry->tensor_memory = CCV_TENSOR_GPU_MEMORY;
	registry->algorithms = 1;
	registry->exec = _conv_transpose_forw;
	NNC_HALF_STAGED(registry, _conv_transpose_forw);
	NNC_DEPALETTIZED(registry, nnc::half_staged<_conv_transpose_forw>);
}
```

### ccv_amd/csrc/common.h

```cpp
#pragma once
#include <hip/hip_runtime.h>
#include <atomic>
#include <stdio.h>
#include <stdlib.h>
#include <string.h>
#include <assert.h>
#include "../../include/nnc_mi355x.h"

#define HIP_ENFORCE(expr) do { \
	const hipError_t _st = (expr); \
	if (_st != hipSuccess) { \
		fprintf(stderr, "[%s:%d]:HIP - Error: %d (%s)\n", __FILE__, __LINE__, (int)_st, hipGetErrorString(_st)); \
		abort(); \
	} \
} while (0)

extern "C" void* nnc_staging_of(const ccv_nnc_stream_context_t* stream_context, size_t size);
extern "C" void* nnc_palette_of(const ccv_nnc_stream_context_t* stream_context, size_t size);

namespace nnc {

static inline int tensor_nd(const int dim[CCV_NNC_MAX_DIM_ALLOC])
{
	int i;
// ... 44 lines not shown

struct Image4 {
	float* p;
	int n, h, w, c;
	long sn, sh, sw, sc;
};
static inline bool image4(const ccv_nnc_tensor_t* t, Image4* o)
{
	const int nd = tensor_nd(t->info.dim);
	if (nd != 3 && nd != 4) return false;
	int st[CCV_NNC_MAX_DIM_ALLOC];
	tensor_strides(t, st);
	const int* d = t->info.dim;
	const int b = (nd == 4);
	o->p = t->data.f32;
	o->n = b ? d[0] : 1;
	o->sn = b ? st[0] : 0;
	if (t->info.format == CCV_TENSOR_FORMAT_NHWC) {
		o->h = d[b]; o->w = d[b + 1]; o->c = d[b + 2];
		o->sh = st[b]; o->sw = st[b + 1]; o->sc = st[b + 2];
	} else if (t->info.format == CCV_TENSOR_FORMAT_NCHW) {
		o->c = d[b]; o->h = d[b + 1]; o->w = d[b + 2];
		o->sc = st[b]; o->sh = st[b + 1]; o->sw = st[b + 2];
	} else
		return false;
	return true;
}

extern std::atomic<int> g_comm_pending;
void comm_flush(void);
void comm_release_context(const void* ctx);
extern std::atomic<int> g_comm_overlap_on;
extern std::atomic<unsigned long> g_comm_overlap_epoch;
void comm_gradients_written(ccv_nnc_tensor_t* const* ts, int n, ccv_nnc_stream_context_t* ctx);
void comm_gradient_touched(const ccv_nnc_tensor_t* t);
void comm_overlap_join(hipStream_t stream, unsigned long* seen);
hipStream_t stream_peek(const ccv_nnc_stream_context_t* ctx);
void stream_registered(int device, hipStream_t st);
typedef int (*exec_fn_t)(const ccv_nnc_cmd_t, const ccv_nnc_hint_t, const int, ccv_nnc_tensor_t* const*, const int, ccv_nnc_tensor_t* const*, const int, ccv_nnc_stream_context_t*);
enum { DEFER_CONV_FORWARD = 1, DEFER_CONV_BACKWARD = 2, DEFER_POOL_BACKWARD = 3, DEFER_BNORM_FORWARD = 4, DEFER_EWSUM_FORWARD = 5, DEFER_SGD_BATCH = 6 };
extern std::atomic<int> g_deferred_live;
bool deferred_try(exec_fn_t fn, int kind, const ccv_nnc_cmd_t cmd, const ccv_nnc_hint_t hint, int flags, ccv_nnc_tensor_t* const* inputs, int input_size, ccv_nnc_tensor_t* const* outputs, int output_size, ccv_nnc_stream_context_t* ctx, uint64_t* sig);
void deferred_mark_good(uint64_t sig);
int deferred_fuse_relu_forw(const ccv_nnc_tensor_t* a, ccv_nnc_tensor_t* b, ccv_nnc_stream_context_t* ctx);
int deferred_fuse_relu_back(const ccv_nnc_tensor_t* g, const ccv_nnc_tensor_t* b, ccv_nnc_tensor_t* h, ccv_nnc_stream_context_t* ctx);
bool deferred_signal_op(int emit, const ccv_nnc_stream_context_t* ctx, const ccv_nnc_stream_signal_t* signal);
bool deferred_trail_cmd(exec_fn_t fn, const ccv_nnc_cmd_t cmd, const ccv_nnc_hint_t hint, int flags, ccv_nnc_tensor_t* const* inputs, int input_size, ccv_nnc_tensor_t* const* outputs, int output_size, ccv_nnc_stream_context_t* ctx);
bool deferred_sgd_head(exec_fn_t fn, const ccv_nnc_cmd_t cmd, const ccv_nnc_hint_t hint, int flags, ccv_nnc_tensor_t* const* inputs, int input_size, ccv_nnc_tensor_t* const* outputs, int output_size, ccv_nnc_stream_context_t* ctx);
extern std::atomic<unsigned long> g_launch_seq;
void deferred_sgd_launched(const ccv_nnc_stream_context_t* ctx);
bool sgd_is_exec(exec_fn_t fn);
int sgd_forw_multi(const ccv_nnc_cmd_t* const* cmds, ccv_nnc_tensor_t* const* const* ins, ccv_nnc_tensor_t* const* const* outs, int n, ccv_nnc_stream_context_t* ctx);
void signal_emit_now(const ccv_nnc_stream_context_t* ctx, const ccv_nnc_stream_signal_t* signal);
void signal_wait_now(const ccv_nnc_stream_context_t* ctx, const ccv_nnc_stream_signal_t* signal);
void deferred_flush(const ccv_nnc_stream_context_t* ctx);
int deferred_take_error(const ccv_nnc_stream_context_t* ctx);
void deferred_suppress(int delta);
static inline void comm_flush_if_pending(void) { if (g_comm_pending) comm_flush(); if (g_deferred_live) deferred_flush(0); }

hipStream_t stream_of(const ccv_nnc_stream_context_t* ctx);
const unsigned* capture_tick_of(hipStream_t st);
void* workspace_of(const ccv_nnc_stream_context_t* ctx, size_t size);
const float* zero_page_of(const ccv_nnc_stream_context_t* ctx);
int device_cu_count(void);
struct cluster_sync_t { unsigned ticket, done; unsigned pad[62]; };
constexpr size_t CLUSTER_SYNC_BYTES = 2u << 20;
constexpr unsigned CLUSTER_SPIN_LIMIT = 1u << 21;
void* cluster_sync_of(const ccv_nnc_stream_context_t* ctx, size_t granule_bytes, unsigned* epoch, unsigned** timeout_word);
struct ClusterTurn {
	hipStream_t stream;
	int device;
	explicit ClusterTurn(const ccv_nnc_stream_context_t* ctx);
	~ClusterTurn();
	ClusterTurn(const ClusterTurn&) = delete;
	ClusterTurn& operator=(const ClusterTurn&) = delete;
};
long cluster_turns_chained(void);
void note_kernel(const char* name);

long tune(int key);
static inline int grid_for(size_t n, int threads)
{
	size_t b = (n + threads - 1) / threads;
	const long per_cu = tune(3 );
	const size_t cap = per_cu > 0 ? (size_t)device_cu_count() * (size_t)per_cu : (size_t)0x7fffffff;
	if (b > cap) b = cap;
	if (b < 1) b = 1;
	return (int)b;
}

struct WorkspaceScope {
	char* base;
	size_t prev, prev_limit;
	WorkspaceScope(const ccv_nnc_stream_context_t* ctx, size_t prefix_bytes, size_t inner_bytes);
	~WorkspaceScope();
	void* prefix() const { return base; }
};
size_t gemm_workspace_bound(long M, long N, long K);

int format_transform(const ccv_nnc_tensor_t* a, ccv_nnc_tensor_t* b, ccv_nnc_stream_context_t* ctx);
int transpose_half_to_float(const void* in, float* out, int batch, int R, int C, ccv_nnc_stream_context_t* ctx);
int transpose_float_to_half(const float* in, void* out, int batch, int R, int C, ccv_nnc_stream_context_t* ctx);
int transpose_half(const void* in, void* out, int batch, int R, int C, ccv_nnc_stream_context_t* ctx);
int transpose_half_rowsum(const void* in, void* out, int batch, int R, int C, float* row_partial, ccv_nnc_stream_context_t* ctx);
inline long transpose_half_rowsum_slices(const int batch, const int C) { return (long)batch * ((C + 63) / 64); }
int relu_inplace(ccv_nnc_tensor_t* t, ccv_nnc_stream_context_t* ctx);
int relu_back_inplace(ccv_nnc_tensor_t* h, const ccv_nnc_tensor_t* b, ccv_nnc_stream_context_t* ctx);
int weights_nchw_to_nhwc(const float* w, float* out, int K, int C, int khw, ccv_nnc_stream_context_t* ctx);
int weights_nhwc_to_nchw(const float* w, float* out, int K, int C, int khw, ccv_nnc_stream_context_t* ctx);

int colsum_f32(const float* x, long rows, int cols, long ld, float* out, int accumulate, ccv_nnc_stream_context_t* ctx);
int fill_f32(float* p, size_t n, float v, ccv_nnc_stream_context_t* ctx);
int chan_sum_planes(const float* x, long outer, int C, long inner, float* out, int accumulate, ccv_nnc_stream_context_t* ctx);

struct ProfScope {
	void* rec;
	hipStream_t stream;
	ProfScope(const char* name, double flops, double bytes, int M, int N, int K, int Z, int S, hipStream_t stream);
	~ProfScope();
};

void prof_next_bytes(double bytes);

struct MarkerScope {
	int active;
	explicit MarkerScope(uint32_t cmd);
	~MarkerScope();
};
void markers_enable(int on);
const char* command_row_name(uint32_t cmd);

extern int g_force_tile;
extern int g_force_splits;

enum {
	TUNE_WINO_SLICE_KB = 0,
	TUNE_WINO_FUSED_MAX_C,
	TUNE_WINO_FUSED_GRID,
	TUNE_GRID_WG_PER_CU,
	TUNE_WINO_WGRAD_FUSED_MAX,
	TUNE_GEMM_BUFFER_LOADS,
	TUNE_CONV_NCHW_HALF_F16,
	TUNE_BN_SMALL_PLANES,
	TUNE_SDPA_MFMA,
	TUNE_BN_CLUSTER,
	TUNE_GEMM_VEC_EPILOGUE,
	TUNE_POOL_ROWS,
	TUNE_GEMM_HALF_CHUNK8,
	TUNE_LSTM_PERSISTENT,
	TUNE_LSTM_ROWS,
	TUNE_GEMM_BF16X3,
	TUNE_BN_CLUSTER_SLOTS,
	TUNE_GEMM_BATCH_XCD,
	TUNE_COUNT
};
static_assert(TUNE_GRID_WG_PER_CU == 3, "grid_for() above names this key by value");
long tune(int key);

constexpr int FOLD_CH = 16, FOLD_PH = 16;
__device__ __forceinline__ float fold_slices(const float* __restrict__ p, const long slices, const int C, const int c, const int phase)
{
	float s0 = 0.f, s1 = 0.f, s2 = 0.f, s3 = 0.f;
	long i = phase;
	for (; i + 3 * FOLD_PH < slices; i += 4 * FOLD_PH) {
		s0 += p[i * C + c]; s1 += p[(i + FOLD_PH) * C + c]; s2 += p[(i + 2 * FOLD_PH) * C + c]; s3 += p[(i + 3 * FOLD_PH) * C + c];
	}
	for (; i < slices; i += FOLD_PH) s0 += p[i * C + c];
	return (s0 + s1) + (s2 + s3);
}
__device__ __forceinline__ float fold_phases(float (*red)[FOLD_CH], const int ch)
{
	float a[FOLD_PH];
#pragma unroll
	for (int k = 0; k < FOLD_PH; k++) a[k] = red[k][ch];
#pragma unroll
	for (int w = FOLD_PH / 2; w >= 1; w >>= 1)
#pragma unroll
		for (int k = 0; k < w; k++) a[k] = a[k] + a[k + w];
	return a[0];
}

typedef int (*nnc_exec_f)(const ccv_nnc_cmd_t, const ccv_nnc_hint_t, const int, ccv_nnc_tensor_t* const* const, const int, ccv_nnc_tensor_t* const* const, const int, ccv_nnc_stream_context_t* const);
int half_staged_exec(nnc_exec_f inner, const ccv_nnc_cmd_t cmd, const ccv_nnc_hint_t hint, const int flags, ccv_nnc_tensor_t* const* const inputs, const int input_size, ccv_nnc_tensor_t* const* const outputs, const int output_size, ccv_nnc_stream_context_t* const ctx);
template <nnc_exec_f F>
static int half_staged(const ccv_nnc_cmd_t cmd, const ccv_nnc_hint_t hint, const int flags, ccv_nnc_tensor_t* const* const inputs, const int input_size, ccv_nnc_tensor_t* const* const outputs, const int output_size, ccv_nnc_stream_context_t* const ctx)
{
	return half_staged_exec(F, cmd, hint, flags, inputs, input_size, outputs, output_size, ctx);
}
#define NNC_HALF_STAGED(registry, EXEC) do { if (((registry)->tensor_datatypes & CCV_32F) && !((registry)->tensor_datatypes & CCV_16F)) {  (registry)->tensor_datatypes |= CCV_16F; (registry)->exec = nnc::half_staged<EXEC>; } } while (0)
bool any_half_tensor(ccv_nnc_tensor_t* const* const inputs, const int input_size, ccv_nnc_tensor_t* const* const outputs, const int output_size);
int half_to_float(const void* in, float* out, size_t n, ccv_nnc_stream_context_t* ctx);
int float_to_half(const float* in, void* out, size_t n, ccv_nnc_stream_context_t* ctx);
int chan_sum_planes_f16(const void* x, long outer, int C, long inner, void* out, int accumulate, ccv_nnc_stream_context_t* ctx);
int colsum_f16(const void* x, long rows, int cols, long ld, void* out, int accumulate, ccv_nnc_stream_context_t* ctx);
int colsum_partials_f16(const float* partial, long slices, int cols, void* out, int accumulate, ccv_nnc_stream_context_t* ctx);

int depalettize(const void* input, int datatype, size_t input_length, int qbits, int number_in_blocks, void* output, size_t output_length, ccv_nnc_stream_context_t* ctx);
size_t palettized_bytes(int palette_datatype, size_t count, int qbits, int number_in_blocks);
bool any_palettized(ccv_nnc_tensor_t* const* const inputs, const int input_size);
int depalettized_exec(nnc_exec_f inner, const ccv_nnc_cmd_t cmd, const ccv_nnc_hint_t hint, const int flags, ccv_nnc_tensor_t* const* const inputs, const int input_size, ccv_nnc_tensor_t* const* const outputs, const int output_size, ccv_nnc_stream_context_t* const ctx);
template <nnc_exec_f F>
static int depalettized(const ccv_nnc_cmd_t cmd, const ccv_nnc_hint_t hint, const int flags, ccv_nnc_tensor_t* const* const inputs, const int input_size, ccv_nnc_tensor_t* const* const outputs, const int output_size, ccv_nnc_stream_context_t* const ctx)
{
	return depalettized_exec(F, cmd, hint, flags, inputs, input_size, outputs, output_size, ctx);
}
#define NNC_DEPALETTIZED(registry, EXEC) do { (registry)->tensor_datatypes |= CCV_QX; (registry)->exec = nnc::depalettized<EXEC>; } while (0)

typedef void (*register_fn_t)(ccv_nnc_cmd_backend_registry_t* const);

}
```

### ccv_amd/csrc/device_rt.cpp

```cpp
#include "common.h"
#include <atomic>
#include <pthread.h>
#include <dlfcn.h>
#include <vector>
#include <list>
#include <deque>
#include <mutex>
#include <unordered_map>

namespace {

struct device_local_t {
	hipStream_t stream;
	void* workspace;
	size_t workspace_size;
	int device;
	void* staging;
	size_t staging_size;
	void* palette;
	size_t palette_size;
	void* cluster_sync;
	unsigned cluster_epoch;
	unsigned long cluster_capture;
	unsigned long capture_alias;
	unsigned long comm_seen;
};
struct stream_cpu_t {
	ccv_nnc_stream_context_s super;
	size_t workspace_size;
	void* workspace;
};
struct stream_gpu_t {
	ccv_nnc_stream_context_s super;
	struct { size_t workspace_size; void* workspace; } cpu;
	device_local_t one;
	device_local_t* any;
	int any_size;
};
struct signal_gpu_t {
	ccv_nnc_stream_signal_s super;
	hipEvent_t event;
	unsigned long capture_id;
	int capture_dev;
};
constexpr int MAX_DEVICES = 64;
thread_local device_local_t tl_default[MAX_DEVICES];
thread_local struct { size_t workspace_size; void* workspace; } tl_default_cpu;
thread_local const char* tl_last_kernel = "";

struct mem_pressure_t { int device_id; nnc_mi355x_mem_pressure_f func; void* ctx; };
pthread_mutex_t g_mp_mutex = PTHREAD_MUTEX_INITIALIZER;
std::vector<mem_pressure_t>& g_mp = *new std::vector<mem_pressure_t>;

void trigger_mem_pressure()
{
	int device_id = 0;
	HIP_ENFORCE(hipGetDevice(&device_id));
	pthread_mutex_lock(&g_mp_mutex);
	for (size_t i = 0; i < g_mp.size(); i++)
		if (g_mp[i].func && g_mp[i].device_id == device_id) g_mp[i].func(device_id, g_mp[i].ctx);
	pthread_mutex_unlock(&g_mp_mutex);
	HIP_ENFORCE(hipSetDevice(device_id));
}

int current_device()
{
	int d = 0;
	HIP_ENFORCE(hipGetDevice(&d));
	return d;
}

std::atomic<unsigned long> g_pool_seq(0);
std::atomic<int> g_capture_active(0);
std::atomic<unsigned long> g_capture_id(0);
std::atomic<unsigned long> g_graph_max_end_seq(0);
hipStream_t g_cap_origin = 0;
int g_cap_device = 0;
constexpr int CAP_MAX_DEVICES = 64;
hipStream_t g_cap_rep[CAP_MAX_DEVICES];
hipEvent_t g_cap_relay[CAP_MAX_DEVICES];
int g_cap_keep_streams = -1;
inline bool pool_pinned(const unsigned long seq) { return g_capture_active.load(std::memory_order_acquire) > 0 || seq <= g_graph_max_end_seq.load(std::memory_order_acquire); }
inline bool stream_capturing(hipStream_t st)
{
	if (!st || g_capture_active.load(std::memory_order_acquire) <= 0) return false;
	hipStreamCaptureStatus status = hipStreamCaptureStatusNone;
	HIP_ENFORCE(hipStreamIsCapturing(st, &status));
	return status == hipStreamCaptureStatusActive;
}

void release_device_block(void* ptr, bool drained);
void pool_stream_created(int device, hipStream_t st);
void pool_stream_destroyed(int device, hipStream_t st);

bool is_any(const ccv_nnc_stream_context_t* ctx) { return (ctx->type & CCV_COMPUTE_DEVICE_ANY) == CCV_COMPUTE_DEVICE_ANY; }

device_local_t* bind(const ccv_nnc_stream_context_t* ctx)
{
	stream_gpu_t* s = (stream_gpu_t*)ctx;
	if (!is_any(ctx)) {
		if (current_device() != s->one.device) HIP_ENFORCE(hipSetDevice(s->one.device));
		return &s->one;
	}
	const int device = current_device();
	if (device >= s->any_size) {
		s->any = (device_local_t*)realloc(s->any, sizeof(device_local_t) * (device + 1));
		memset(s->any + s->any_size, 0, sizeof(device_local_t) * (device + 1 - s->any_size));
		s->any_size = device + 1;
	}
	device_local_t* l = s->any + device;
	if (!l->stream) {
		l->device = device;
		HIP_ENFORCE(hipStreamCreateWithFlags(&l->stream, hipStreamDefault));
		pool_stream_created(device, l->stream);
	}
	return l;
}

inline hipStream_t effective_stream(device_local_t* const l)
{
	if (g_capture_active.load(std::memory_order_acquire) > 0 && l->capture_alias == g_capture_id.load(std::memory_order_acquire) && l->capture_alias && l->device >= 0 && l->device < CAP_MAX_DEVICES && g_cap_rep[l->device]) return g_cap_rep[l->device];
	return l->stream;
}

}

namespace nnc {
int g_force_tile = 0;
int g_force_splits = 0;
static const char* const g_tune_names[TUNE_COUNT] = { "WINO_SLICE_KB", "WINO_FUSED_MAX_C", "WINO_FUSED_GRID", "GRID_WG_PER_CU", "WINO_WGRAD_FUSED_MAX", "GEMM_BUFFER_LOADS", "CONV_NCHW_HALF_F16", "BN_SMALL_PLANES", "SDPA_MFMA", "BN_CLUSTER", "GEMM_VEC_EPILOGUE", "POOL_ROWS", "GEMM_HALF_CHUNK8", "LSTM_PERSISTENT", "LSTM_ROWS", "GEMM_BF16X3", "BN_CLUSTER_SLOTS", "GEMM_BATCH_XCD" };
static long g_tune_values[TUNE_COUNT] = { 0, 128, 0, 0, 128, 1, 32, 1, 1, 1, 1, 1, 1, 1, 1, 1, 0, 1 };
static int g_tune_env_read = 0;
long tune(int key)
{
	if (!g_tune_env_read) {
		for (int i = 0; i < TUNE_COUNT; i++) {
			char name[64];
			snprintf(name, sizeof(name), "NNC_MI355X_%s", g_tune_names[i]);
			const char* v = getenv(name);
			if (v && *v) g_tune_values[i] = atol(v);
		}
		g_tune_env_read = 1;
	}
	return key >= 0 && key < TUNE_COUNT ? g_tune_values[key] : 0;
}
}
namespace nnc {

static inline device_local_t* joined(device_local_t* const l)
{
	if (g_comm_overlap_epoch.load(std::memory_order_acquire) != l->comm_seen) comm_overlap_join(l->stream, &l->comm_seen);
	return l;
}
std::atomic<unsigned long> g_launch_seq(0);
hipStream_t stream_of(const ccv_nnc_stream_context_t* ctx)
{
	g_launch_seq.fetch_add(1, std::memory_order_relaxed);
	if (g_comm_pending) comm_flush();
	if (g_deferred_live) deferred_flush(ctx);
	if (!ctx) return (hipStream_t)0;
	if (CCV_STREAM_GET_CONTEXT(ctx->type) != CCV_STREAM_CONTEXT_GPU) return (hipStream_t)0;
	return effective_stream(joined(bind(ctx)));
}
void stream_registered(const int device, hipStream_t st) { pool_stream_created(device, st); }
hipStream_t stream_peek(const ccv_nnc_stream_context_t* ctx)
{
	if (!ctx || CCV_STREAM_GET_CONTEXT(ctx->type) != CCV_STREAM_CONTEXT_GPU) return (hipStream_t)0;
	return effective_stream(bind(ctx));
}

static thread_local size_t tl_ws_prefix = 0;
static thread_local size_t tl_ws_limit = 0;

void* workspace_of(const ccv_nnc_stream_context_t* ctx, size_t size)
{
	if (tl_ws_limit && tl_ws_prefix + size > tl_ws_limit) return 0;
	char* p = (char*)ccv_nnc_stream_compat_get_workspace(ctx, tl_ws_prefix + size, CCV_TENSOR_GPU_MEMORY);
	return p ? p + tl_ws_prefix : 0;
}

WorkspaceScope::WorkspaceScope(const ccv_nnc_stream_context_t* ctx, size_t prefix_bytes, size_t inner_bytes)
{
	prefix_bytes = (prefix_bytes + 255) & ~(size_t)255;
	prev = tl_ws_prefix;
	prev_limit = tl_ws_limit;
	if (tl_ws_limit && tl_ws_prefix + prefix_bytes + inner_bytes > tl_ws_limit) { base = 0; return; }
	char* p = (char*)ccv_nnc_stream_compat_get_workspace(ctx, tl_ws_prefix + prefix_bytes + inner_bytes, CCV_TENSOR_GPU_MEMORY);
	base = p ? p + tl_ws_prefix : 0;
	if (!tl_ws_limit) tl_ws_limit = tl_ws_prefix + prefix_bytes + inner_bytes;
	tl_ws_prefix += prefix_bytes;
}
WorkspaceScope::~WorkspaceScope() { tl_ws_prefix = prev; tl_ws_limit = prev_limit; }

static unsigned* g_cluster_timeout = 0;
static pthread_mutex_t g_cluster_mutex = PTHREAD_MUTEX_INITIALIZER;
static void cluster_check_timeout()
{
	if (g_cluster_timeout && *(volatile unsigned*)g_cluster_timeout) {
		fprintf(stderr, "[nnc_mi355x] a cluster kernel gave up waiting for its sibling workgroups (code %u): its results are invalid\n", *(volatile unsigned*)g_cluster_timeout);
		abort();
	}
}
static struct { pthread_mutex_t mutex; hipEvent_t event; hipStream_t last; int have; } g_cluster_turn[MAX_DEVICES];
static pthread_once_t g_cluster_turn_once = PTHREAD_ONCE_INIT;
static long g_cluster_turns_chained = 0;
static void cluster_turn_init() { for (int i = 0; i < MAX_DEVICES; i++) pthread_mutex_init(&g_cluster_turn[i].mutex, 0); }
long cluster_turns_chained(void) { return __atomic_load_n(&g_cluster_turns_chained, __ATOMIC_RELAXED); }
ClusterTurn::ClusterTurn(const ccv_nnc_stream_context_t* ctx) : stream(stream_of(ctx)), device(current_device())
{
	pthread_once(&g_cluster_turn_once, cluster_turn_init);
	if (device < 0 || device >= MAX_DEVICES) { device = -1; return; }
	auto& t = g_cluster_turn[device];
	pthread_mutex_lock(&t.mutex);
	if (t.have && t.last != stream) {
		if (!t.event) HIP_ENFORCE(hipEventCreateWithFlags(&t.event, hipEventDisableTiming));
		HIP_ENFORCE(hipEventRecord(t.event, t.last));
		HIP_ENFORCE(hipStreamWaitEvent(stream, t.event, 0));
		__atomic_add_fetch(&g_cluster_turns_chained, 1, __ATOMIC_RELAXED);
	}
}
ClusterTurn::~ClusterTurn()
{
	if (device < 0) return;
	auto& t = g_cluster_turn[device];
	t.last = stream;
	t.have = 1;
	pthread_mutex_unlock(&t.mutex);
}
static void cluster_turn_forget(const int device, hipStream_t stream)
{
	pthread_once(&g_cluster_turn_once, cluster_turn_init);
	if (device < 0 || device >= MAX_DEVICES) return;
	auto& t = g_cluster_turn[device];
	pthread_mutex_lock(&t.mutex);
	if (t.have && t.last == stream) t.have = 0;
	pthread_mutex_unlock(&t.mutex);
}

void* cluster_sync_of(const ccv_nnc_stream_context_t* ctx, size_t granule_bytes, unsigned* epoch, unsigned** timeout_word)
{
	if (granule_bytes > CLUSTER_SYNC_BYTES - 256) return 0;
	if (g_deferred_live) deferred_flush(ctx);
	device_local_t* l;
	if (ctx && CCV_STREAM_GET_CONTEXT(ctx->type) == CCV_STREAM_CONTEXT_GPU) l = bind(ctx);
	else {
		const int device = current_device();
		if (device >= MAX_DEVICES) return 0;
		l = &tl_default[device];
		l->device = device;
	}
	if (!g_cluster_timeout) {
		pthread_mutex_lock(&g_cluster_mutex);
		if (!g_cluster_timeout) {
			unsigned* w = 0;
			HIP_ENFORCE(hipHostMalloc((void**)&w, 256, hipHostMallocDefault));
			memset(w, 0, 256);
			g_cluster_timeout = w;
		}
		pthread_mutex_unlock(&g_cluster_mutex);
	}
	if (!l->cluster_sync) {
		void* p = nnc_mi355x_malloc(l->device, CLUSTER_SYNC_BYTES);
		if (!p) return 0;
		HIP_ENFORCE(hipMemset(p, 0, CLUSTER_SYNC_BYTES));
		l->cluster_sync = p;
		l->cluster_epoch = 0;
	}
	hipStream_t const es = l->stream ? effective_stream(l) : (hipStream_t)0;
	if (es && stream_capturing(es) && l->cluster_capture != g_capture_id.load(std::memory_order_acquire)) {
		HIP_ENFORCE(hipMemsetAsync(l->cluster_sync, 0, CLUSTER_SYNC_BYTES, es));
		l->cluster_capture = g_capture_id.load(std::memory_order_acquire);
	}
	if (++l->cluster_epoch == 0) l->cluster_epoch = 1;
	*epoch = l->cluster_epoch;
	*timeout_word = g_cluster_timeout;
	return l->cluster_sync;
}

const float* zero_page_of(const ccv_nnc_stream_context_t* ctx)
{
	static void* pages[MAX_DEVICES];
	static pthread_mutex_t mutex = PTHREAD_MUTEX_INITIALIZER;
	const int device = (ctx && CCV_STREAM_GET_CONTEXT(ctx->type) == CCV_STREAM_CONTEXT_GPU) ? bind(ctx)->device : current_device();
	assert(device >= 0 && device < MAX_DEVICES);
// ... 1096 lines not shown
```

### ccv_amd/csrc/wino_fused.h

```cpp
#pragma once
#include <utility>
#include "winograd.h"

namespace nnc {

constexpr int WF_KT = 32;
constexpr int WF_CC = 8;
constexpr int WF_U_FLOATS = 36 * 64 * 2 * 2;
constexpr int WF_HP = 352;
constexpr int WF_P_FLOATS = 2 * WF_HP * 4;
constexpr int WF_P_PIECES = 11;
constexpr int WF_Z_AGPR = 30;
constexpr unsigned WF_OOB = 0x7ffff000u;

template <class F, int... I> __device__ __forceinline__ void wf_static_for_impl(F&& f, std::integer_sequence<int, I...>) { (f(GroupId<I>()), ...); }
template <int N, class F> __device__ __forceinline__ void wf_static_for(F&& f) { wf_static_for_impl(f, std::make_integer_sequence<int, N>()); }

typedef float f2 __attribute__((ext_vector_type(2)));

template <int GH, int GW>
struct WfGeom {
	static constexpr int RH = 4 * GH + 2, RW = 4 * GW + 2, NPIX = RH * RW;
	static_assert(GH * GW == 16 && NPIX <= WF_HP, "tile group must be 16 tiles whose patch region fits the buffer");
	static constexpr __host__ __device__ int cy(int yy) { return GH + (yy < 2 ? 1 : 0); }
// ... 316 lines not shown
				}
				__builtin_amdgcn_sched_barrier(0);
			});
		});
	};

	auto epilogue = [&](const Item& it, const int par) {
		NNC_ASM_NOPS("s_nop 15\n\ts_nop 15");
		if constexpr (DBG & 64) { if (a.bias == (const float*)1) a.dst[t] = acc[0][0][0] + acc[35][1][3] + acc[17][0][1]; return; }
		if constexpr (!(DBG & 32)) __builtin_amdgcn_s_barrier();
		constexpr int TS = 16 * 32 + 16;
		float* const st = ubuf + par * WF_U_FLOATS + wave * 2304;
		static_assert(4 * TS <= 2304, "staging area of a wave: a quarter of a U buffer");
		typedef unsigned int u4 __attribute__((ext_vector_type(4)));
		const __amdgpu_buffer_rsrc_t rs_dst = __builtin_amdgcn_make_buffer_rsrc((void*)(a.dst + (long)it.n * a.d_sn), 0, a.dst_image_bytes, 0x00020000);
		const int kq = it.kb * WF_KT + (lane & 7) * 4;
		const bool kok = (it.live != 0) & (kq < a.K);
		float bv[4];
#pragma unroll
		for (int i = 0; i < 4; i++) bv[i] = (a.bias && kq < a.K) ? a.bias[kq + i] : 0.f;
		const int dh4 = (int)a.d_sh * 4, dw4 = (int)a.d_sw * 4;
		const wf_rsrc_t rs_item = wf_make_rsrc(a.dst + (long)it.n * a.d_sn, a.dst_image_bytes);
		const int base_y = it.gy * GH * 4, base_x = it.gx * GW * 4;
		const unsigned s_item = (unsigned)base_y * (unsigned)dh4 + (unsigned)base_x * (unsigned)dw4 + (unsigned)it.kb * (WF_KT * 4);
		const int hy0 = a.OH - base_y, hx0 = a.OW - base_x;
		const int ly = lane >> 5, lx = (lane >> 3) & 3;
		const unsigned lane_off_item = kok ? (unsigned)(ly * dh4 + lx * dw4 + (lane & 7) * 16) : WF_OOB;
		const float relu_lo = a.relu ? 0.f : -__builtin_inff();
		unsigned mb[4] = { ~0u, ~0u, ~0u, ~0u };
		if constexpr (MASK) {
			const unsigned* const mp = a.mask_bits + ((((long)it.n * a.GYn + it.gy) * a.GXn + it.gx) * a.KB + it.kb) * 256 + lane;
#pragma unroll
			for (int r = 0; r < 4; r++) mb[r] = it.live ? mp[r * 64] : 0u;
		}
#pragma unroll
		for (int r = 0; r < 4; r++) {
#pragma unroll
			for (int j = 0; j < 2; j++) {
				float s[4][6];
				if constexpr (DBG & 2048) {
#pragma unroll
					for (int i = 0; i < 4; i++)
#pragma unroll
						for (int jj = 0; jj < 4; jj++) st[g * TS + (i * 4 + jj) * 32 + j * 16 + ti] = acc[i * 4 + jj][j][r];
					continue;
				}
#pragma unroll
				for (int zx = 0; zx < 6; zx++) {
					const float col[6] = { acc[0 * 6 + zx][j][r], acc[1 * 6 + zx][j][r], acc[2 * 6 + zx][j][r], acc[3 * 6 + zx][j][r], acc[4 * 6 + zx][j][r], acc[5 * 6 + zx][j][r] };
					float y[4];
					wino_at(col, y);
#pragma unroll
					for (int i = 0; i < 4; i++) s[i][zx] = y[i];
				}
#pragma unroll
				for (int i = 0; i < 4; i++) {
					float y[4];
					wino_at(s[i], y);
#pragma unroll
					for (int jj = 0; jj < 4; jj++) st[g * TS + (i * 4 + jj) * 32 + j * 16 + ti] = y[jj];
				}
			}
			__builtin_amdgcn_wave_barrier();
			if (r == 0) WF_WAIT_VMCNT(0);
			if constexpr (NEWST) {
#pragma unroll
				for (int e = 0; e < 8; e++) {
					const int tile = 4 * (e >> 1) + r;
					const int cy = (tile >> GWL) * 4 + (e & 1) * 2, cx = (tile & (GW - 1)) * 4;
					const float4 v = *(const float4*)(st + (e >> 1) * TS + ((e & 1) * 8 + (lane >> 3)) * 32 + (lane & 7) * 4);
					const unsigned soff = s_item + (unsigned)cy * (unsigned)dh4 + (unsigned)cx * (unsigned)dw4;
					const bool ok = (ly < hy0 - cy) & (lx < hx0 - cx);
					const unsigned voff = ok ? lane_off_item : WF_OOB;
					float o0 = wf_max(v.x + bv[0], relu_lo), o1 = wf_max(v.y + bv[1], relu_lo), o2 = wf_max(v.z + bv[2], relu_lo), o3 = wf_max(v.w + bv[3], relu_lo);
					if constexpr (MASK) {
						const unsigned m = mb[r] >> (4 * e);
						o0 = (m & 1) ? o0 : 0.f; o1 = (m & 2) ? o1 : 0.f; o2 = (m & 4) ? o2 : 0.f; o3 = (m & 8) ? o3 : 0.f;
					}
					if constexpr (DBG & 128) { NNC_PIN_V(o0); NNC_PIN_V(o1); NNC_PIN_V(o2); NNC_PIN_V(o3); }
					else wf_store16<ST_POLICY>(rs_item, voff, soff, o0, o1, o2, o3);
				}
			} else {
#pragma unroll
			for (int e = 0; e < 8; e++) {
				const int pid = e * 8 + (lane >> 3);
				const int gp = pid >> 4, px = pid & 15;
				const int tile = 4 * gp + r;
				const int oy = (it.gy * GH + (tile >> GWL)) * 4 + (px >> 2), ox = (it.gx * GW + (tile & (GW - 1))) * 4 + (px & 3);
				const float4 v = *(const float4*)(st + gp * TS + px * 32 + (lane & 7) * 4);
				const unsigned voff = (kok & (oy < a.OH) & (ox < a.OW)) ? (unsigned)(oy * dh4 + ox * dw4 + kq * 4) : WF_OOB;
				float o0 = v.x + bv[0], o1 = v.y + bv[1], o2 = v.z + bv[2], o3 = v.w + bv[3];
				if (a.relu) { o0 = fmaxf(o0, 0.f); o1 = fmaxf(o1, 0.f); o2 = fmaxf(o2, 0.f); o3 = fmaxf(o3, 0.f); }
				if constexpr (MASK) {
					const unsigned m = mb[r] >> (4 * e);
					o0 = (m & 1) ? o0 : 0.f; o1 = (m & 2) ? o1 : 0.f; o2 = (m & 4) ? o2 : 0.f; o3 = (m & 8) ? o3 : 0.f;
				}
				if constexpr (DBG & 128) { NNC_PIN_V(o0); NNC_PIN_V(o1); NNC_PIN_V(o2); NNC_PIN_V(o3); }
				else __builtin_amdgcn_raw_buffer_store_b128(u4{ __float_as_uint(o0), __float_as_uint(o1), __float_as_uint(o2), __float_as_uint(o3) }, rs_dst, voff, 0, 0);
			}
			}
			__builtin_amdgcn_wave_barrier();
		}
#pragma unroll
		for (int z = 0; z < 36; z++)
#pragma unroll
			for (int j = 0; j < 2; j++) acc[z][j] = floatx4{ 0.f, 0.f, 0.f, 0.f };
	};

	if constexpr (PAIR) {
		const int M = a.CCn >> 1;
		for (int ii = 0; ii < count; ii++) {
			const Item nxt = item_of(ii + 1 < count ? first + ii + 1 : first + ii);
			for (int m = 0; m < M; m++) {
				const bool last = m == M - 1;
				if constexpr (!(DBG & 256)) { if (m != 0 || ii == 0) WF_WAIT_VMCNT(0); }
				if constexpr (!(DBG & 32)) __builtin_amdgcn_s_barrier();
				if (last) set_patch(nxt);
				const unsigned sp = last ? 0u : (unsigned)(m + 1) * (2 * WF_CC * 4);
				trip(GroupId<0>(), GroupId<0>(), 0, sp, (unsigned)(2 * m + 1) * (WF_U_FLOATS * 4) + (unsigned)wave * 9216u);
				if constexpr (!(DBG & 256)) WF_WAIT_VMCNT(PS::W_ODD_START);
				if constexpr (!(DBG & 32)) __builtin_amdgcn_s_barrier();
				if (last) set_u(nxt);
				trip(GroupId<0>(), GroupId<1>(), 1, sp, (last ? 0u : (unsigned)(2 * m + 2) * (WF_U_FLOATS * 4)) + (unsigned)wave * 9216u);
			}
			epilogue(cur, 1);
			cur = nxt;
		}
	} else {
	int gtrip = 0;
	for (int ii = 0; ii < count; ii++) {
		const Item nxt = item_of(ii + 1 < count ? first + ii + 1 : first + ii);
		for (int cc = 0; cc < a.CCn; cc++, gtrip++) {
			const int par = gtrip & 1;
			if constexpr (!(DBG & 256)) { if (ii == 0 && cc == 0) WF_WAIT_VMCNT(0); else if (cc != 0) WF_WAIT_VMCNT(3); }
			if constexpr (!(DBG & 32)) __builtin_amdgcn_s_barrier();
			if (cc == a.CCn - 2) set_patch(nxt);
			if (cc == a.CCn - 1) set_u(nxt);
			const int c2 = cc + 2 >= a.CCn ? cc + 2 - a.CCn : cc + 2, c1 = cc + 1 >= a.CCn ? 0 : cc + 1;
			const unsigned sp = (unsigned)c2 * (WF_CC * 4), su = (unsigned)c1 * (WF_U_FLOATS * 4) + (unsigned)wave * 9216u;
			trip(GroupId<0>(), GroupId<0>(), par, sp, su);
		}
		epilogue(cur, (gtrip - 1) & 1);
		cur = nxt;
	}
	}
#undef WF_XFORM
}

template <int GH, int GW>
__global__ void __launch_bounds__(256) wino_mask_pack_kernel(const float* __restrict__ mask, const long m_sn, const long m_sh, const long m_sw, unsigned* __restrict__ bits, const int OH, const int OW, const int K, const int GYn, const int GXn, const int KB)
{
	constexpr int GWL = GW == 4 ? 2 : (GW == 8 ? 3 : (GW == 2 ? 1 : (GW == 16 ? 4 : 0)));
	static_assert(GH * GW == 16, "16 tiles per group");
	int b = (int)blockIdx.x;
	const int kb = b % KB; b /= KB;
	const int gx = b % GXn; b /= GXn;
	const int gy = b % GYn;
	const int n = b / GYn;
	const int r = (int)threadIdx.x >> 6, lane = (int)threadIdx.x & 63;
	const int kq = kb * WF_KT + (lane & 7) * 4;
	const float* const mp = mask + (long)n * m_sn + kq;
	unsigned m = 0;
#pragma unroll
	for (int e = 0; e < 8; e++) {
		const int pid = e * 8 + (lane >> 3);
		const int gp = pid >> 4, px = pid & 15;
		const int tile = 4 * gp + r;
		const int oy = (gy * GH + (tile >> GWL)) * 4 + (px >> 2), ox = (gx * GW + (tile & (GW - 1))) * 4 + (px & 3);
		if ((kq < K) & (oy < OH) & (ox < OW)) {
			const float4 v = *(const float4*)(mp + (long)oy * m_sh + (long)ox * m_sw);
			m |= ((v.x > 0.f ? 1u : 0u) | (v.y > 0.f ? 2u : 0u) | (v.z > 0.f ? 4u : 0u) | (v.w > 0.f ? 8u : 0u)) << (4 * e);
		}
	}
	bits[(size_t)blockIdx.x * 256 + threadIdx.x] = m;
}

}
```

### ccv_amd/csrc/wino_wgrad_fused.h

```cpp
#pragma once
#include "wino_fused.h"

namespace nnc {

typedef float f2v __attribute__((ext_vector_type(2)));

constexpr int WG_KB = 32, WG_CB = 64;
constexpr int WG_GH = 2, WG_GW = 4;
constexpr int WG_RH = 4 * WG_GH + 2, WG_RW = 4 * WG_GW + 2;
constexpr int WG_A_BYTES = WG_RH * WG_RW * WG_CB * 4;
constexpr int WG_G_BYTES = (4 * WG_GH) * (4 * WG_GW) * WG_KB * 4;
constexpr int WG_A_PIECES = WG_A_BYTES / 1024, WG_G_PIECES = WG_G_BYTES / 1024;
constexpr int WG_STAGE_BYTES = WG_A_BYTES + WG_G_BYTES;
static_assert(WG_A_BYTES % 1024 == 0 && WG_G_BYTES % 1024 == 0 && 2 * WG_STAGE_BYTES <= 160 * 1024, "two stages of whole DMA pieces in LDS");
constexpr int WG_A_PER_WAVE = (WG_A_PIECES + 3) / 4, WG_G_PER_WAVE = WG_G_PIECES / 4;
constexpr int WG_PIECES_PER_WAVE = WG_A_PER_WAVE + WG_G_PER_WAVE;

struct WinoWgradFusedArgs {
	const float* a;
	const float* g;
	float* partial;
	float* bias_partial;
	long a_sn, a_sh, a_sw, g_sn, g_sh, g_sw;
	int H, W, OH, OW;
	int pad_y, pad_x;
	int GYn, GXn;
	int groups;
	int C, K;
	int kblocks, cblocks;
	int slices;
	int per_slice;
	unsigned a_image_bytes, g_image_bytes;
};

template <int DBG = 0>
__global__ void __launch_bounds__(256, 1) wino_wgrad_fused_kernel(const WinoWgradFusedArgs p)
{
	__shared__ __attribute__((aligned(16))) float lds[2 * WG_STAGE_BYTES / 4 + 256];
	const int t = threadIdx.x, lane = t & 63;
	const int wave = __builtin_amdgcn_readfirstlane(t >> 6);
	const int wk = wave >> 1, wc = wave & 1;
	const int ch = lane & 15, slot = lane >> 4;
	const int nb = p.kblocks * p.cblocks;
	const int xcd = (int)blockIdx.x & 7, r = (int)blockIdx.x >> 3;
	const int slice = xcd * (p.slices >> 3) + r / nb, blk = r % nb;
	const int kb = blk / p.cblocks, cb = blk - kb * p.cblocks;
	int g_first = slice * p.per_slice, g_end = g_first + p.per_slice;
	if (g_end > p.groups) g_end = p.groups;
	const int gpi = p.GYn * p.GXn;

	floatx4 acc[36][2];
#pragma unroll
	for (int z = 0; z < 36; z++)
#pragma unroll
		for (int j = 0; j < 2; j++) acc[z][j] = floatx4{ 0.f, 0.f, 0.f, 0.f };
	float bsum = 0.f;

	int ayx[WG_A_PER_WAVE], gyx[WG_G_PER_WAVE];
#pragma unroll
	for (int i = 0; i < WG_A_PER_WAVE; i++) {
		const int q = wave + 4 * i, pi = q * 4 + (lane >> 4);
		ayx[i] = q < WG_A_PIECES ? ((pi / WG_RW) << 8 | (pi % WG_RW)) : 0xff00;
	}
#pragma unroll
	for (int i = 0; i < WG_G_PER_WAVE; i++) {
		const int pj = (wave + 4 * i) * 8 + (lane >> 3);
		gyx[i] = (pj / (4 * WG_GW)) << 8 | (pj % (4 * WG_GW));
	}
	const int a_coff = (cb * WG_CB + (lane & 15) * 4) * 4, g_coff = (kb * WG_KB + (lane & 7) * 4) * 4;
	const int a_sh4 = (int)p.a_sh * 4, a_sw4 = (int)p.a_sw * 4, g_sh4 = (int)p.g_sh * 4, g_sw4 = (int)p.g_sw * 4;
	const unsigned lds0 = __builtin_amdgcn_readfirstlane(wf_lds_addr(lds));
	wf_rsrc_t rs_a, rs_g;
	int aY0 = 0, aY1 = 0, aX0 = 0, aX1 = 0, gY1 = 0, gX1 = 0;
	auto set_group = [&](const int group) {
		const int n = group / gpi, gr = group - n * gpi;
		const int gy = gr / p.GXn, gx = gr - gy * p.GXn;
		const int ny0 = gy * 4 * WG_GH, nx0 = gx * 4 * WG_GW, nY0 = ny0 - p.pad_y, nX0 = nx0 - p.pad_x;
		rs_a = wf_make_rsrc(p.a + (long)n * p.a_sn + (long)nY0 * p.a_sh + (long)nX0 * p.a_sw, 0x7fff0000u);
		rs_g = wf_make_rsrc(p.g + (long)n * p.g_sn + (long)ny0 * p.g_sh + (long)nx0 * p.g_sw, 0x7fff0000u);
		aY0 = nY0 < 0 ? -nY0 : 0; aY1 = p.H - nY0 < WG_RH ? p.H - nY0 : WG_RH;
		aX0 = nX0 < 0 ? -nX0 : 0; aX1 = p.W - nX0 < WG_RW ? p.W - nX0 : WG_RW;
		gY1 = p.OH - ny0 < 4 * WG_GH ? p.OH - ny0 : 4 * WG_GH;
		gX1 = p.OW - nx0 < 4 * WG_GW ? p.OW - nx0 : 4 * WG_GW;
	};
	auto dma_piece = [&](auto ic, const int st, const bool live) {
		constexpr int i = decltype(ic)::value;
		if constexpr (i < WG_A_PER_WAVE) {
			const int Y = ayx[i] >> 8, X = ayx[i] & 255;
			const bool ok = live & (Y >= aY0) & (Y < aY1) & (X >= aX0) & (X < aX1);
			const unsigned voff = ok ? (unsigned)(Y * a_sh4 + X * a_sw4 + a_coff) : WF_OOB;
			const unsigned dst = wave + 4 * i < WG_A_PIECES ? lds0 + st * WG_STAGE_BYTES + (wave + 4 * i) * 1024 : lds0 + 2 * WG_STAGE_BYTES;
			wf_dma16(rs_a, lds, dst, voff, 0u);
		} else {
			constexpr int j = i - WG_A_PER_WAVE;
			const int y = gyx[j] >> 8, x = gyx[j] & 255;
			const bool ok = live & (y < gY1) & (x < gX1);
			const unsigned voff = ok ? (unsigned)(y * g_sh4 + x * g_sw4 + g_coff) : WF_OOB;
			wf_dma16(rs_g, lds, lds0 + st * WG_STAGE_BYTES + WG_A_BYTES + (wave + 4 * j) * 1024, voff, 0u);
		}
	};

	if (g_first < g_end) {
	set_group(g_first);
	NNC_ASM_NOPS("s_nop 4");
	wf_static_for<WG_PIECES_PER_WAVE>([&](auto nc) {
		constexpr int n = decltype(nc)::value, piece = n < 7 ? n : (n < 11 ? WG_A_PER_WAVE + (n - 7) : n - 4);
		dma_piece(GroupId<piece>(), 0, true);
	});

	for (int grp = g_first; grp < g_end; grp++) {
		const int st = (grp - g_first) & 1;
		if constexpr (!(DBG & 32)) {
			WF_WAIT_VMCNT(5);
			__builtin_amdgcn_s_barrier();
		}
		const bool has_next = grp + 1 < g_end;
		if (has_next) set_group(grp + 1);
		const float* const ab = lds + st * (WG_STAGE_BYTES / 4) + (4 * slot) * WG_CB + wc * 32 + 2 * ch;
		const float* const gb = lds + st * (WG_STAGE_BYTES / 4) + WG_A_BYTES / 4 + (4 * slot) * WG_KB + wk * 16 + ch;
		f2v W[36];
		if constexpr (DBG & 2) {
#pragma unroll
			for (int z = 0; z < 36; z++) W[z] = f2v{ 1.f + z, 2.f };
		} else {
			f2v e[4][4];
#pragma unroll
			for (int i = 0; i < 4; i++)
#pragma unroll
				for (int j = 0; j < 4; j++) e[i][j] = f2v{ gb[(i * (4 * WG_GW) + j) * WG_KB], gb[((4 + i) * (4 * WG_GW) + j) * WG_KB] };
			if (wc == 0 && cb == 0) {
#pragma unroll
				for (int i = 0; i < 4; i++) { const f2v r4 = (e[i][0] + e[i][1]) + (e[i][2] + e[i][3]); bsum += r4.x + r4.y; }
			}
			f2v t1[6][4];
#pragma unroll
			for (int j = 0; j < 4; j++) {
				const f2v col[4] = { e[0][j], e[1][j], e[2][j], e[3][j] };
				f2v y[6];
				wino_g4(col, y);
#pragma unroll
				for (int rr = 0; rr < 6; rr++) t1[rr][j] = y[rr];
			}
#pragma unroll
			for (int rr = 0; rr < 6; rr++) {
				f2v y[6];
				wino_g4(t1[rr], y);
#pragma unroll
				for (int q = 0; q < 6; q++) W[rr * 6 + q] = y[q];
			}
		}
#pragma unroll
		for (int z = 0; z < 36; z++) { NNC_PIN_V(W[z].x); NNC_PIN_V(W[z].y); }
		wf_static_for<2>([&](auto ksc) {
			constexpr int ks = decltype(ksc)::value;
			if constexpr (ks == 1 && !(DBG & 32)) {
				WF_WAIT_VMCNT(8);
				__builtin_amdgcn_s_barrier();
			}
			f2v V[36];
			if constexpr (DBG & 2) {
#pragma unroll
				for (int z = 0; z < 36; z++) V[z] = f2v{ 3.f, 1.f + z };
			} else {
				f2v sm[6][6];
#pragma unroll
				for (int c6 = 0; c6 < 6; c6++) {
					f2v col[6], y[6];
#pragma unroll
					for (int r6 = 0; r6 < 6; r6++) col[r6] = *(const f2v*)(ab + ((4 * ks + r6) * WG_RW + c6) * WG_CB);
					wino_bt(col, y);
#pragma unroll
					for (int r6 = 0; r6 < 6; r6++) sm[r6][c6] = y[r6];
				}
#pragma unroll
				for (int r6 = 0; r6 < 6; r6++) {
					f2v y[6];
					wino_bt(sm[r6], y);
#pragma unroll
					for (int q = 0; q < 6; q++) V[r6 * 6 + q] = y[q];
				}
			}
#pragma unroll
			for (int z = 0; z < 36; z++) { NNC_PIN_V(V[z].x); NNC_PIN_V(V[z].y); }
			NNC_ASM_NOPS("s_nop 1");
			wf_static_for<72>([&](auto mc) {
				constexpr int mm = decltype(mc)::value, z = mm >> 1, jf = mm & 1;
				if constexpr (!(DBG & 16)) {
					if constexpr (ks == 0 && jf == 0) WF_MFMA(acc[z][0], W[z].x, V[z].x, z < WF_Z_AGPR);
					else if constexpr (ks == 0) WF_MFMA(acc[z][1], W[z].x, V[z].y, z < WF_Z_AGPR);
					else if constexpr (jf == 0) WF_MFMA(acc[z][0], W[z].y, V[z].x, z < WF_Z_AGPR);
					else WF_MFMA(acc[z][1], W[z].y, V[z].y, z < WF_Z_AGPR);
				}
				constexpr int m = ks * 72 + mm;
// ... 46 lines not shown
```

### ccv_amd/csrc/winograd.h

```cpp
#pragma once
#include "mfma_gemm.h"

namespace nnc {

template <class T>
__device__ __forceinline__ void wino_bt(const T (&x)[6], T (&y)[6])
{
	const T a = x[4] - 4.f * x[2], b = x[3] - 4.f * x[1];
	const T c = x[4] - x[2], d = 2.f * (x[3] - x[1]);
	y[0] = 4.f * x[0] - 5.f * x[2] + x[4];
	y[1] = a + b;
	y[2] = a - b;
	y[3] = c + d;
	y[4] = c - d;
	y[5] = 4.f * x[1] - 5.f * x[3] + x[5];
}
template <class T>
__device__ __forceinline__ void wino_g(const T (&x)[3], T (&y)[6])
{
	const T s = x[0] + x[2];
	const T e = x[0] * (1.f / 24.f) + x[2] * (1.f / 6.f), o = x[1] * (1.f / 12.f);
	y[0] = x[0] * 0.25f;
	y[1] = (s + x[1]) * (-1.f / 6.f);
	y[2] = (s - x[1]) * (-1.f / 6.f);
	y[3] = e + o;
	y[4] = e - o;
	y[5] = x[2];
}
template <class T>
__device__ __forceinline__ void wino_at(const T (&x)[6], T (&y)[4])
{
	const T s1 = x[1] + x[2], d1 = x[1] - x[2], s2 = x[3] + x[4], d2 = x[3] - x[4];
	y[0] = x[0] + s1 + s2;
	y[1] = d1 + 2.f * d2;
	y[2] = s1 + 4.f * s2;
	y[3] = d1 + 8.f * d2 + x[5];
}

template <class T>
__device__ __forceinline__ void wino_g4(const T (&x)[4], T (&y)[6])
{
	const T e = x[0] + x[2], o = x[1] + x[3];
	const T e2 = x[0] * (1.f / 24.f) + x[2] * (1.f / 6.f), o2 = x[1] * (1.f / 12.f) + x[3] * (1.f / 3.f);
	y[0] = x[0] * 0.25f;
	y[1] = (e + o) * (-1.f / 6.f);
	y[2] = (e - o) * (-1.f / 6.f);
	y[3] = e2 + o2;
	y[4] = e2 - o2;
	y[5] = x[3];
}
template <class T>
__device__ __forceinline__ void wino_at3(const T (&x)[6], T (&y)[3])
{
	const T s1 = x[1] + x[2], d1 = x[1] - x[2], s2 = x[3] + x[4], d2 = x[3] - x[4];
	y[0] = x[0] + s1 + s2;
	y[1] = d1 + 2.f * d2;
	y[2] = s1 + 4.f * s2 + x[5];
}

struct f4 {
	float x, y, z, w;
	__device__ __forceinline__ f4() {}
	__device__ __forceinline__ f4(float a, float b, float c, float d) : x(a), y(b), z(c), w(d) {}
	__device__ __forceinline__ f4(const float4 v) : x(v.x), y(v.y), z(v.z), w(v.w) {}
	__device__ __forceinline__ operator float4() const { return make_float4(x, y, z, w); }
};
__device__ __forceinline__ f4 operator+(const f4 a, const f4 b) { return f4(a.x + b.x, a.y + b.y, a.z + b.z, a.w + b.w); }
__device__ __forceinline__ f4 operator-(const f4 a, const f4 b) { return f4(a.x - b.x, a.y - b.y, a.z - b.z, a.w - b.w); }
__device__ __forceinline__ f4 operator*(const float s, const f4 a) { return f4(s * a.x, s * a.y, s * a.z, s * a.w); }
__device__ __forceinline__ f4 operator*(const f4 a, const float s) { return f4(s * a.x, s * a.y, s * a.z, s * a.w); }

template <bool FLIP>
static __global__ void __launch_bounds__(256) wino_weight_kernel(const float* __restrict__ w, float* __restrict__ u, const int K, const int C)
{
	const int R = FLIP ? C : K, Q = FLIP ? K : C;
	const long idx = (long)blockIdx.x * blockDim.x + threadIdx.x;
	if (idx >= (long)R * Q) return;
	const int r = (int)(idx / Q), q = (int)(idx - (long)r * Q);
	const int k = FLIP ? q : r, c = FLIP ? r : q;
	float g[3][3];
#pragma unroll
	for (int i = 0; i < 3; i++)
#pragma unroll
		for (int j = 0; j < 3; j++)
			g[i][j] = w[((long)k * 9 + (FLIP ? (2 - i) * 3 + (2 - j) : i * 3 + j)) * C + c];
	float t[6][3];
#pragma unroll
	for (int j = 0; j < 3; j++) {
		const float col[3] = { g[0][j], g[1][j], g[2][j] };
		float y[6];
		wino_g(col, y);
#pragma unroll
		for (int i = 0; i < 6; i++) t[i][j] = y[i];
	}
	const long plane = (long)R * Q;
#pragma unroll
	for (int i = 0; i < 6; i++) {
		float y[6];
		wino_g(t[i], y);
#pragma unroll
		for (int j = 0; j < 6; j++) u[(long)(i * 6 + j) * plane + idx] = y[j];
	}
}

struct WinoTiles {
	int TH, TW, T;
	int H, W;
	long sn, sh, sw;
	int oy, ox;
	int C4;
	int relu;
	const float* mask; long m_sn, m_sh, m_sw;
	FastDiv d_c4, d_tw, d_th;
};

static __global__ void __launch_bounds__(256) wino_input_kernel(const float* __restrict__ a, float* __restrict__ v, const WinoTiles g)
{
	const long idx = (long)nnc_xcd_block(blockIdx.x, gridDim.x) * blockDim.x + threadIdx.x;
	if (idx >= (long)g.T * g.C4) return;
	const int t = g.d_c4.div((int)idx), c4 = (int)(idx - (long)t * g.C4);
	const int tn = g.d_tw.div(t), tx = t - tn * g.TW;
	const int n = g.d_th.div(tn), ty = tn - n * g.TH;
	const int y0 = ty * 4 + g.oy, x0 = tx * 4 + g.ox;
	const float* const src = a + (long)n * g.sn + (long)c4 * 4;
	f4 s[6][6];
#pragma unroll
	for (int r = 0; r < 6; r++) {
		const int y = y0 + r;
		const bool yok = (y >= 0) & (y < g.H);
		f4 d[6];
#pragma unroll
		for (int q = 0; q < 6; q++) {
			const int x = x0 + q;
			const bool ok = yok & (x >= 0) & (x < g.W);
			d[q] = ok ? f4(*(const float4*)(src + (long)y * g.sh + (long)x * g.sw)) : f4(0.f, 0.f, 0.f, 0.f);
		}
		wino_bt(d, s[r]);
	}
	const long plane = (long)g.T * g.C4 * 4;
	float* const dst = v + idx * 4;
#pragma unroll
	for (int q = 0; q < 6; q++) {
		const f4 col[6] = { s[0][q], s[1][q], s[2][q], s[3][q], s[4][q], s[5][q] };
		f4 y[6];
		wino_bt(col, y);
#pragma unroll
		for (int r = 0; r < 6; r++) *(float4*)(dst + (long)(r * 6 + q) * plane) = y[r];
	}
}

static __global__ void __launch_bounds__(256) wino_output_kernel(const float* __restrict__ m, const float* __restrict__ bias, float* __restrict__ b, const WinoTiles g)
{
	const long idx = (long)blockIdx.x * blockDim.x + threadIdx.x;
	if (idx >= (long)g.T * g.C4) return;
	const int t = g.d_c4.div((int)idx), k4 = (int)(idx - (long)t * g.C4);
	const int tn = g.d_tw.div(t), tx = t - tn * g.TW;
	const int n = g.d_th.div(tn), ty = tn - n * g.TH;
	const long plane = (long)g.T * g.C4 * 4;
	const float* const src = m + idx * 4;
	f4 s[4][6];
#pragma unroll
	for (int q = 0; q < 6; q++) {
		f4 col[6];
#pragma unroll
		for (int r = 0; r < 6; r++) col[r] = f4(*(const float4*)(src + (long)(r * 6 + q) * plane));
		f4 y[4];
		wino_at(col, y);
#pragma unroll
		for (int i = 0; i < 4; i++) s[i][q] = y[i];
	}
	const f4 bv = bias ? f4(*(const float4*)(bias + k4 * 4)) : f4(0.f, 0.f, 0.f, 0.f);
	float* const dst = b + (long)n * g.sn + (long)k4 * 4;
	const float* const msk = g.mask ? g.mask + (long)n * g.m_sn + (long)k4 * 4 : 0;
#pragma unroll
	for (int i = 0; i < 4; i++) {
		f4 y[4];
		wino_at(s[i], y);
		const int oy = ty * 4 + i;
#pragma unroll
		for (int j = 0; j < 4; j++) {
			const int ox = tx * 4 + j;
			if ((oy < g.H) & (ox < g.W)) {
				f4 o = y[j] + bv;
				if (g.relu) o = f4(fmaxf(o.x, 0.f), fmaxf(o.y, 0.f), fmaxf(o.z, 0.f), fmaxf(o.w, 0.f));
				if (msk) {
					const float4 mv = *(const float4*)(msk + (long)oy * g.m_sh + (long)ox * g.m_sw);
					o = f4(mv.x > 0.f ? o.x : 0.f, mv.y > 0.f ? o.y : 0.f, mv.z > 0.f ? o.z : 0.f, mv.w > 0.f ? o.w : 0.f);
				}
				*(float4*)(dst + (long)oy * g.sh + (long)ox * g.sw) = (float4)o;
			}
		}
	}
}

template <bool COLSUM>
static __global__ void __launch_bounds__(256) wino_outgrad_kernel(const float* __restrict__ gr, float* __restrict__ wt, const WinoTiles g, float* __restrict__ blockpart)
{
	__shared__ float4 red[COLSUM ? 256 : 1];
	const long idx = (long)blockIdx.x * blockDim.x + threadIdx.x;
	const bool live = idx < (long)g.T * g.C4;
	f4 sum(0.f, 0.f, 0.f, 0.f);
	if (live) {
		const int t = g.d_c4.div((int)idx), k4 = (int)(idx - (long)t * g.C4);
		const int tn = g.d_tw.div(t), tx = t - tn * g.TW;
		const int n = g.d_th.div(tn), ty = tn - n * g.TH;
		const float* const src = gr + (long)n * g.sn + (long)k4 * 4;
		f4 s[4][6];
#pragma unroll
		for (int r = 0; r < 4; r++) {
			const int y = ty * 4 + r;
			f4 d[4];
#pragma unroll
			for (int q = 0; q < 4; q++) {
				const int x = tx * 4 + q;
				const bool ok = (y < g.H) & (x < g.W);
				d[q] = ok ? f4(*(const float4*)(src + (long)y * g.sh + (long)x * g.sw)) : f4(0.f, 0.f, 0.f, 0.f);
				if (COLSUM) sum = sum + d[q];
			}
			wino_g4(d, s[r]);
		}
		const long plane = (long)g.T * g.C4 * 4;
		float* const dst = wt + idx * 4;
#pragma unroll
		for (int q = 0; q < 6; q++) {
			const f4 col[4] = { s[0][q], s[1][q], s[2][q], s[3][q] };
			f4 y[6];
			wino_g4(col, y);
#pragma unroll
			for (int r = 0; r < 6; r++) *(float4*)(dst + (long)(r * 6 + q) * plane) = y[r];
		}
	}
	if (COLSUM) {
		red[threadIdx.x] = (float4)sum;
		__syncthreads();
		if ((int)threadIdx.x < g.C4) {
			f4 acc(0.f, 0.f, 0.f, 0.f);
			for (int j = threadIdx.x; j < 256; j += g.C4) acc = acc + f4(red[j]);
			*(float4*)(blockpart + ((long)blockIdx.x * g.C4 + threadIdx.x) * 4) = (float4)acc;
		}
	}
}

static __global__ void __launch_bounds__(256) wino_wgrad_final_kernel(const float* __restrict__ du, float* __restrict__ dw, const int K, const int C, const int accumulate)
{
	const long idx = (long)blockIdx.x * blockDim.x + threadIdx.x;
	const long plane = (long)K * C;
	if (idx >= plane) return;
	const int k = (int)(idx / C), c = (int)(idx - (long)k * C);
	float s[3][6];
#pragma unroll
	for (int q = 0; q < 6; q++) {
		float col[6];
#pragma unroll
		for (int r = 0; r < 6; r++) col[r] = du[(long)(r * 6 + q) * plane + idx];
		float y[3];
		wino_at3(col, y);
#pragma unroll
		for (int i = 0; i < 3; i++) s[i][q] = y[i];
	}
#pragma unroll
	for (int i = 0; i < 3; i++) {
		float y[3];
		wino_at3(s[i], y);
#pragma unroll
		for (int j = 0; j < 3; j++) {
			float* const o = dw + ((long)k * 9 + i * 3 + j) * C + c;
			*o = accumulate ? *o + y[j] : y[j];
		}
	}
}

}
```

### include/nnc_mi355x.h

```cpp
#ifndef NNC_MI355X_H
#define NNC_MI355X_H

#include <stddef.h>
#include <stdint.h>
#include <sys/types.h>

#ifdef __cplusplus
extern "C" {
#endif

enum { CCV_TENSOR_FORMAT_NCHW = 0x01, CCV_TENSOR_FORMAT_NHWC = 0x02, CCV_TENSOR_FORMAT_CHWN = 0x04 };
enum { CCV_TENSOR_CPU_MEMORY = 0x1, CCV_TENSOR_GPU_MEMORY = 0x2 };
enum { CCV_COMPUTE_DEVICE_ANY = 0xfff00 };
#define CCV_TENSOR_GET_MEMORY(type) ((type) & 0x3)
#define CCV_TENSOR_GET_DEVICE(type) ((type) & 0xfff00)
#define CCV_TENSOR_GET_DEVICE_ID(type) (CCV_TENSOR_GET_DEVICE(type) >> 8)
enum { CCV_TENSOR_VIEW = 0x01000000, CCV_TENSOR_MULTIVIEW = 0x02000000, CCV_TENSOR_PINNED_MEM = 0x04000000 };
enum { CCV_8U = 0x01000, CCV_32S = 0x02000, CCV_32F = 0x04000, CCV_64S = 0x08000, CCV_64F = 0x10000, CCV_16F = 0x20000, CCV_QX = 0x40000 };
#define CCV_GET_DATA_TYPE(x) ((x) & 0xFF000)
enum { CCV_NNC_ACCUMULATE_OUTPUT = 0x01, CCV_NNC_ZERO_MEMORY_ALLOC = 0x02 };
enum { CCV_NNC_EXEC_SUCCESS = 0, CCV_NNC_EXEC_INVALID = -1, CCV_NNC_EXEC_NO_KERNEL = -2, CCV_NNC_EXEC_OOM = -3 };
enum { CCV_STREAM_CONTEXT_CPU = 0x1, CCV_STREAM_CONTEXT_GPU = 0x2 };
#define CCV_STREAM_GET_CONTEXT(type) ((type) & 0x3)
#define CCV_STREAM_GET_DEVICE_ID(type) CCV_TENSOR_GET_DEVICE_ID(type)
// ... 121 lines not shown
	int type;
	int refcount;
	ccv_numeric_data_t data;
	off_t dataof;
	uintptr_t alias_ref;
	uint64_t data_size;
	uint64_t sig;
	ccv_nnc_tensor_param_t info;
	int contiguous;
	off_t off;
	int stride[CCV_NNC_MAX_DIM_ALLOC];
} ccv_nnc_tensor_view_t;

#define CCV_IS_TENSOR_VIEW(x) ((*(const int*)(x)) & CCV_TENSOR_VIEW)
#define CCV_IS_TENSOR_CONTIGUOUS(x) (!CCV_IS_TENSOR_VIEW(x) || (((const ccv_nnc_tensor_view_t*)(x))->contiguous == 1))

typedef struct {
	struct { int dim[CCV_NNC_MAX_DIM_ALLOC]; } size;
	union {
		struct { int count; int groups; int dilation[CCV_NNC_MAX_DIM_ALLOC]; } convolution;
		struct { int reserved; } pool;
		struct { int axis[CCV_NNC_MAX_DIM_ALLOC]; int count; float epsilon; int is_test; float momentum; } bnorm;
		struct { int nesterov; float rate; float scale; float decay; float momentum; float dampening; } sgd;
		struct { int transpose_a[2]; int transpose_b[2]; float a[3]; int flags; } blas;
		struct { float trim0; float trim1; } label_smoothing;
		struct { int axis[CCV_NNC_MAX_DIM_ALLOC]; int count; } reduce;
		struct { int axis[2]; } transpose;
		struct { float p; int entirety; } dropout;
		struct { float min; float max; } clamp;
		struct { int tanh; } gelu;
		struct { int type; float width_scale; float height_scale; int align_corners; } upsample;
		struct { int axis[CCV_NNC_MAX_DIM_ALLOC]; int count; float epsilon; int elementwise_affine; } lnorm;
		struct { int axis[CCV_NNC_MAX_DIM_ALLOC]; int count; float epsilon; } rmsnorm;
		struct { int group_axis; int reduce_axis[CCV_NNC_MAX_DIM_ALLOC]; int reduce_count; int groups; float epsilon; int elementwise_affine; } gnorm;
		struct { int type; int end[CCV_NNC_MAX_DIM_ALLOC]; } pad;
		struct { float pos_weight; } binary_crossentropy;
		struct { float beta; } smooth_l1;
		struct { int reduce_op; } mse;
		struct { float negative_slope; } leaky_relu;
		struct { int step; float rate; float scale; float beta1; float beta2; float decay; float epsilon; int amsgrad; } adam;
		struct { float rate; float scale; float decay; float alpha; float momentum; float epsilon; } rmsprop;
		struct { int step; float rate; float scale; float beta1; float beta2; float decay; float epsilon; } lamb;
		struct { float iou_threshold; } nms;
		struct { float scale; int is_causal; int flags; int deterministic; } scaled_dot_product_attention;
		struct { int hidden_size; int proj_size; int num_layers; int bias; int batch_first; int bidirectional; float dropout; int is_test; } rnn;
		char _widest[68];
		void* userdata;
	};
} ccv_nnc_cmd_param_t;

typedef struct {
	struct { int dim[CCV_NNC_MAX_DIM_ALLOC]; } stride;
	struct { int begin[CCV_NNC_MAX_DIM_ALLOC]; int end[CCV_NNC_MAX_DIM_ALLOC]; } border;
} ccv_nnc_hint_t;

typedef struct ccv_nnc_stream_context_s ccv_nnc_stream_context_t;
typedef struct ccv_nnc_stream_signal_s ccv_nnc_stream_signal_t;
typedef struct ccv_nnc_cmd_vtab_s ccv_nnc_cmd_vtab_t;

typedef struct ccv_nnc_cmd_s {
	uint32_t cmd;
	uint32_t backend;
	int algorithm;
	ccv_nnc_cmd_param_t info;
	ccv_nnc_cmd_vtab_t* isa;
	void* data;
} ccv_nnc_cmd_t;

typedef int (*ccv_nnc_cmd_exec_f)(const ccv_nnc_cmd_t cmd, const ccv_nnc_hint_t hint, const int flags, ccv_nnc_tensor_t* const* const inputs, const int input_size, ccv_nnc_tensor_t* const* const outputs, const int output_size, ccv_nnc_stream_context_t* const stream_context);
typedef int (*ccv_nnc_cmd_autotune_f)(const ccv_nnc_cmd_t cmd, const size_t max_workspace_size, const ccv_nnc_hint_t hint, const int flags, ccv_nnc_tensor_t* const* const inputs, const int input_size, ccv_nnc_tensor_t* const* const outputs, const int output_size, ccv_nnc_stream_context_t* const stream_context);

typedef struct {
	int tensor_formats;
	int tensor_datatypes;
	int tensor_memory;
	int algorithms;
	ccv_nnc_cmd_exec_f exec;
	ccv_nnc_cmd_autotune_f autotune;
	void* aux;
} ccv_nnc_cmd_backend_registry_t;

struct ccv_nnc_stream_context_s {
	int type;
	void* _host_private[10];
};
struct ccv_nnc_stream_signal_s {
	int type;
	ccv_nnc_stream_context_t* emit_context;
};

typedef void (*ccv_nnc_callback_f)(void* const callback_context);
typedef struct { ccv_nnc_callback_f fn; void* callback_context; } ccv_nnc_async_callback_t;
typedef void (*ccv_nnc_async_callback_f)(ccv_nnc_async_callback_t* const async);
typedef void (*nnc_mi355x_mem_pressure_f)(int device_id, void* const context);

void* nnc_mi355x_malloc(int device, size_t size);
void  nnc_mi355x_free(int device, void* ptr);
void  nnc_mi355x_set_device(int device);
void  nnc_mi355x_memcpy(void* dest, const int dest_type, const void* src, const int src_type, size_t n);
void* nnc_mi355x_host_alloc(size_t size);
void  nnc_mi355x_host_free(void* ptr);
int   nnc_mi355x_host_register(void* ptr, size_t size);
void  nnc_mi355x_host_unregister(void* ptr);
int   nnc_mi355x_register_mem_pressure(int device_id, nnc_mi355x_mem_pressure_f func, void* const context);
void  nnc_mi355x_unregister_mem_pressure(const int id);
void  nnc_mi355x_set_profiler(int state);
int   nnc_mi355x_device_count(void);

ccv_nnc_stream_context_t* ccv_nnc_init_stream_context(ccv_nnc_stream_context_t* const stream_context);
void  ccv_nnc_deinit_stream_context(ccv_nnc_stream_context_t* const stream_context);
void  ccv_nnc_synchronize_stream_context(const ccv_nnc_stream_context_t* const stream_context);
void* ccv_nnc_stream_compat_get_workspace(const ccv_nnc_stream_context_t* const stream_context, const size_t workspace_size, const int mem);
void  ccv_nnc_stream_compat_drain(ccv_nnc_stream_context_t* const stream_context);
void  ccv_nnc_stream_compat_add_callback(ccv_nnc_stream_context_t* const stream, const ccv_nnc_callback_f callback, const ccv_nnc_async_callback_f async_callback, void* const callback_context);
ccv_nnc_stream_signal_t* ccv_nnc_init_stream_signal(ccv_nnc_stream_signal_t* const signal);
void  ccv_nnc_deinit_stream_signal(ccv_nnc_stream_signal_t* const signal);
void  ccv_nnc_stream_compat_emit_signal(const ccv_nnc_stream_context_t* const stream, const ccv_nnc_stream_signal_t* const signal);
void  ccv_nnc_stream_compat_wait_signal(const ccv_nnc_stream_context_t* const stream, const ccv_nnc_stream_signal_t* const signal);
int   ccv_nnc_stream_context_get_device(const ccv_nnc_stream_context_t* const stream_context);
void* nnc_mi355x_stream_context_get_stream(const ccv_nnc_stream_context_t* const stream_context);

ccv_nnc_stream_context_t* nnc_mi355x_stream_context_new(const int type);
void nnc_mi355x_stream_context_free(ccv_nnc_stream_context_t* const stream_context);
void nnc_mi355x_stream_context_wait(const ccv_nnc_stream_context_t* const stream_context);
ccv_nnc_stream_signal_t* nnc_mi355x_stream_signal_new(const int type);
void nnc_mi355x_stream_signal_free(ccv_nnc_stream_signal_t* const signal);

int nnc_mi355x_registry_count(void);
int nnc_mi355x_registry_get(int i, uint32_t* cmd, uint32_t* backend, ccv_nnc_cmd_backend_registry_t* registry);
const char* nnc_mi355x_registry_name(int i);

int nnc_mi355x_cmd_exec(const ccv_nnc_cmd_t cmd, const ccv_nnc_hint_t hint, const int flags, ccv_nnc_tensor_t* const* const inputs, const int input_size, ccv_nnc_tensor_t* const* const outputs, const int output_size, ccv_nnc_stream_context_t* const stream_context);
int nnc_mi355x_cmd_ok(const uint32_t cmd, const uint32_t backend);

int nnc_mi355x_comm_unique_id(void* id_out_128_bytes);
int nnc_mi355x_comm_init_rank(const void* id_128_bytes, int rank, int world_size);
void nnc_mi355x_comm_destroy(void);
void nnc_mi355x_comm_overlap(int on);
void nnc_mi355x_comm_overlap_stats(long* collectives, long* buckets);
int nnc_mi355x_comm_count(void);
void nnc_mi355x_comm_stats(long* collectives, long* groups);

#include "nnc_mi355x_pipeline.h"

void* nnc_mi355x_event_new(void);
void  nnc_mi355x_event_record(void* event, const ccv_nnc_stream_context_t* const stream_context);
float nnc_mi355x_event_elapsed_ms(void* start, void* stop);
void  nnc_mi355x_event_free(void* event);
void nnc_mi355x_profile_enable(int on);
int  nnc_mi355x_profile_count(void);
int  nnc_mi355x_profile_get(int i, char* name, int name_len, double* flops, double* bytes, float* ms, int dims[5]);
void nnc_mi355x_debug_force_tile(int wm, int wn);
void nnc_mi355x_debug_force_splits(int splits);
size_t nnc_mi355x_lstm_reserve_space_size(const ccv_nnc_cmd_t cmd, int datatype, int feature_size, int batch_count, int max_seq_count);
int nnc_mi355x_depalettize(const void* input, int datatype, size_t input_length, int qbits, int number_in_blocks, void* output, size_t output_length, ccv_nnc_stream_context_t* stream_context);
size_t nnc_mi355x_palettized_bytes(int datatype, size_t count, int qbits, int number_in_blocks);
#define NNC_MI355X_CONV_ALGO_FUSE_RELU 0x100
#define NNC_MI355X_POOL_ALGO_FUSE_RELU_BACKWARD 0x100
#define NNC_MI355X_BNORM_ALGO_FUSE_RELU 0x100
#define NNC_MI355X_EWSUM_ALGO_FUSE_RELU 0x100
#define NNC_MI355X_EWSUM_ALGO_FUSE_RELU_BACKWARD 0x200
void nnc_mi355x_set_peephole(int on);
void nnc_mi355x_debug_peephole_counts(long* recorded, long* folded, long* plain);
long nnc_mi355x_debug_peephole_trailed(void);
void nnc_mi355x_debug_pool_counts(long* allocs, long* retries, long* reserved_bytes, long* used_bytes);
long nnc_mi355x_debug_pool_trimmed(void);
void nnc_mi355x_pool_trim(int device);
int nnc_mi355x_capture_begin(ccv_nnc_stream_context_t* stream_context);
void* nnc_mi355x_capture_end(ccv_nnc_stream_context_t* stream_context);
int nnc_mi355x_graph_launch(void* graph, ccv_nnc_stream_context_t* stream_context);
int nnc_mi355x_graph_node_count(void* graph);
void nnc_mi355x_graph_free(void* graph);
void nnc_mi355x_capture_keep_streams(int on);
long nnc_mi355x_debug_pool_parked_bytes(void);
void nnc_mi355x_debug_pool_fences(long* events, long* waits);
long nnc_mi355x_debug_bn_cluster_launches(void);
long nnc_mi355x_debug_exec_count(void);
void nnc_mi355x_debug_half_counts(long* staged, long* native);
int  nnc_mi355x_tune_set(const char* name, long value);
long nnc_mi355x_tune_get(const char* name);
const char* nnc_mi355x_last_kernel_name(void);
const char* nnc_mi355x_version(void);

#ifdef __cplusplus
}
#endif

#include "nnc_mi355x_registry.h"

#endif
```

Baseline: 3347 images/s.

## Share winograd input transforms and relu mask bits between conv wgrad and dgrad

When a backward convolution computes both weight and data gradients, the wgrad pass now produces data the dgrad pass can reuse. In one case the output-gradient transform also writes the dgrad input-domain tile V. In the other, the activation input transform also emits packed relu mask bits. The dgrad pass then skips its own input transform or mask-pack kernel by reading these from an agreed workspace offset. This costs a larger workspace and adds thread-local coupling that relies on the workspace pointer staying stable between the two passes.

```diff
diff --git a/ccv_amd/csrc/cmd_conv.cpp b/ccv_amd/csrc/cmd_conv.cpp
--- a/ccv_amd/csrc/cmd_conv.cpp
+++ b/ccv_amd/csrc/cmd_conv.cpp
@@ -18,6 +18,20 @@
 	const Image4& m = tl_mask;
 	return m.p && m.n == dst.n && m.h == dst.h && m.w == dst.w && m.c == dst.c && m.sc == 1 && aligned16(m.p) && m.sw % 4 == 0 && m.sh % 4 == 0 && (m.n == 1 || m.sn % 4 == 0);
 }
+
+struct back_share_t {
+	int want_v;
+	int want_bits;
+	int GYn, GXn, KB;
+	float* v;
+	unsigned* bits;
+	size_t v_off, bits_off;
+};
+static thread_local back_share_t tl_share = { 0, 0, 0, 0, 0, 0, 0, 0, 0 };
+
+static void* g_dbg_bits_dst = 0;
+static size_t g_dbg_bits_cap = 0, g_dbg_bits_got = 0;
+static long g_back_shared[2] = { 0, 0 };
 
 struct conv_geom_t {
 	int N, H, W, C;
@@ -101,11 +115,15 @@
 	const int nb = wino_slice_images(g.N, per_image, Cs, Cd);
 	const size_t v_bytes = nb == g.N ? p.v_bytes : (sizeof(float) * 36 * (size_t)nb * per_image * Cs + 255) & ~(size_t)255;
 	const size_t m_bytes = nb == g.N ? p.m_bytes : (sizeof(float) * 36 * (size_t)nb * per_image * Cd + 255) & ~(size_t)255;
-	char* ws = (char*)workspace_of(ctx, p.u_bytes + v_bytes + m_bytes);
+	bool have_v = FLIP && tl_share.v && nb == g.N && p.u_bytes + m_bytes <= tl_share.v_off;
+	size_t need = p.u_bytes + v_bytes + m_bytes;
+	if (have_v && tl_share.v_off + v_bytes > need) need = tl_share.v_off + v_bytes;
+	char* ws = (char*)workspace_of(ctx, need);
 	if (!ws) return CCV_NNC_EXEC_OOM;
+	if (have_v && (float*)(ws + tl_share.v_off) != tl_share.v) have_v = false;
 	float* const U = (float*)ws;
-	float* const V = (float*)(ws + p.u_bytes);
-	float* const M = (float*)(ws + p.u_bytes + v_bytes);
+	float* const V = have_v ? tl_share.v : (float*)(ws + p.u_bytes);
+	float* const M = have_v ? (float*)(ws + p.u_bytes) : (float*)(ws + p.u_bytes + v_bytes);
 	hipStream_t stream = stream_of(ctx);
 	hipLaunchKernelGGL(HIP_KERNEL_NAME(wino_weight_kernel<FLIP>), dim3(blocks_exact((size_t)Cs * Cd, 256)), dim3(256), 0, stream, w, U, g.K, g.C);
 	HIP_ENFORCE(hipGetLastError());
@@ -119,7 +137,7 @@
 		if (ti.relu) tl_relu_done = 1;
 		ti.mask = 0; ti.m_sn = ti.m_sh = ti.m_sw = 0;
 		ti.d_c4.init(ti.C4); ti.d_tw.init(ti.TW); ti.d_th.init(ti.TH);
-		hipLaunchKernelGGL(wino_input_kernel, dim3(blocks_exact((size_t)T * ti.C4, 256)), dim3(256), 0, stream, (const float*)src.p + (long)n0 * src.sn, V, ti);
+		if (!have_v) hipLaunchKernelGGL(HIP_KERNEL_NAME(wino_input_kernel<false>), dim3(blocks_exact((size_t)T * ti.C4, 256)), dim3(256), 0, stream, (const float*)src.p + (long)n0 * src.sn, V, ti, WinoMaskOut());
 		HIP_ENFORCE(hipGetLastError());
 		MatLoader<true, true> la, lb;
 		la.p = V; la.ldr = Cs; la.ldk = 1; la.R = T; la.K = Cs;
@@ -190,12 +208,15 @@
 static int conv_wino_fused_run(const char* name, const conv_geom_t& g, const wino_fused_plan_t& p, const Image4& src, const float* w, const float* bias, const Image4& dst, const int pad_y, const int pad_x, ccv_nnc_stream_context_t* const ctx)
 {
 	size_t bits_bytes = FLIP && mask_fits(dst) && (long)p.groups * p.KB <= 0x7fffffffL ? (size_t)p.groups * p.KB * 1024 : 0;
-	float* UF = (float*)workspace_of(ctx, p.uf_bytes + bits_bytes);
+	bool have_bits = FLIP && bits_bytes && tl_share.bits && p.GH == 2 && p.GYn == tl_share.GYn && p.GXn == tl_share.GXn && p.KB == tl_share.KB && p.uf_bytes <= tl_share.bits_off;
+	float* UF = (float*)workspace_of(ctx, have_bits ? tl_share.bits_off + bits_bytes : p.uf_bytes + bits_bytes);
+	if (have_bits && (!UF || (unsigned*)((char*)UF + tl_share.bits_off) != tl_share.bits)) { have_bits = false; UF = (float*)workspace_of(ctx, p.uf_bytes + bits_bytes); }
 	if (!UF && bits_bytes) { bits_bytes = 0; UF = (float*)workspace_of(ctx, p.uf_bytes); }
 	if (!UF) return CCV_NNC_EXEC_OOM;
 	hipStream_t stream = stream_of(ctx);
-	unsigned* const bits = bits_bytes ? (unsigned*)((char*)UF + p.uf_bytes) : 0;
-	if (bits) {
+	unsigned* const bits = have_bits ? tl_share.bits : (bits_bytes ? (unsigned*)((char*)UF + p.uf_bytes) : 0);
+	if (have_bits) tl_mask_done = 1;
+	else if (bits) {
 		const dim3 grid((unsigned)((long)p.groups * p.KB));
 		const Image4& m = tl_mask;
 		if (p.GH == 4) hipLaunchKernelGGL(HIP_KERNEL_NAME(wino_mask_pack_kernel<4, 4>), grid, dim3(256), 0, stream, (const float*)m.p, m.sn, m.sh, m.sw, bits, dst.h, dst.w, dst.c, p.GYn, p.GXn, p.KB);
@@ -203,6 +224,12 @@
 		else hipLaunchKernelGGL(HIP_KERNEL_NAME(wino_mask_pack_kernel<8, 2>), grid, dim3(256), 0, stream, (const float*)m.p, m.sn, m.sh, m.sw, bits, dst.h, dst.w, dst.c, p.GYn, p.GXn, p.KB);
 		HIP_ENFORCE(hipGetLastError());
 		tl_mask_done = 1;
+	}
+	if (bits && g_dbg_bits_dst) {
+		g_dbg_bits_got = (size_t)p.groups * p.KB * 1024;
+		HIP_ENFORCE(hipMemcpyAsync(g_dbg_bits_dst, bits, g_dbg_bits_got < g_dbg_bits_cap ? g_dbg_bits_got : g_dbg_bits_cap, hipMemcpyDeviceToHost, stream));
+		HIP_ENFORCE(hipStreamSynchronize(stream));
+		g_dbg_bits_dst = 0;
 	}
 	const int Kout = dst.c, Cred = src.c;
 	hipLaunchKernelGGL(HIP_KERNEL_NAME(wino_weight_frag_kernel<FLIP>), dim3(blocks_exact((size_t)p.KB * WF_KT * Cred, 256)), dim3(256), 0, stream, w, UF, Kout, Cred, g.K, g.C);
@@ -278,17 +305,25 @@
 
 static int conv_wino_wgrad(const conv_geom_t& g, const wino_wgrad_plan_t& p, const Image4& gr, const Image4& a, float* dw, float* dbias, bool* bias_done, const int flags, ccv_nnc_stream_context_t* const ctx)
 {
-	char* ws = (char*)workspace_of(ctx, p.total());
+	const int per_image = p.t.TH * p.t.TW;
+	const int nb = wino_slice_images(g.N, per_image, g.C, g.K);
+	const size_t bits_bytes = (size_t)g.N * tl_share.GYn * tl_share.GXn * tl_share.KB * 1024;
+	const bool fuse_bias = dbias && 256 % (g.K / 4) == 0;
+	const size_t extra = nb != g.N ? 0 : (tl_share.want_v ? (fuse_bias ? p.w_bytes : 0) : (tl_share.want_bits ? bits_bytes : 0));
+	char* ws = (char*)workspace_of(ctx, p.total() + extra);
 	if (!ws) return CCV_NNC_EXEC_OOM;
+	float* const Vg = extra && tl_share.want_v ? (float*)(ws + p.total()) : 0;
+	unsigned* const bits = extra && tl_share.want_bits ? (unsigned*)(ws + p.total()) : 0;
 	float* const V = (float*)(ws + p.head_bytes);
 	float* const W = (float*)(ws + p.head_bytes + p.t.v_bytes);
 	float* const dU = (float*)(ws + p.head_bytes + p.t.v_bytes + p.w_bytes);
 	float* const BP = (float*)(ws + p.head_bytes + p.t.v_bytes + p.w_bytes + p.du_bytes);
-	const bool fuse_bias = dbias && 256 % (g.K / 4) == 0;
 	const int acc = (flags & CCV_NNC_ACCUMULATE_OUTPUT) ? 1 : 0;
 	hipStream_t stream = stream_of(ctx);
-	const int per_image = p.t.TH * p.t.TW;
-	const int nb = wino_slice_images(g.N, per_image, g.C, g.K);
+	if (bits && (tl_share.GYn * 2 != p.t.TH || tl_share.GXn * 8 != p.t.TW || g.C % WF_KT)) {
+		const int r = fill_f32((float*)bits, bits_bytes / sizeof(float), 0.f, ctx);
+		if (r != CCV_NNC_EXEC_SUCCESS) return r;
+	}
 	for (int n0 = 0; n0 < g.N; n0 += nb) {
 		const int ns = g.N - n0 < nb ? g.N - n0 : nb;
 		const int T = ns * per_image;
@@ -296,13 +331,24 @@
 		ti.TH = p.t.TH; ti.TW = p.t.TW; ti.T = T;
 		ti.H = a.h; ti.W = a.w; ti.sn = a.sn; ti.sh = a.sh; ti.sw = a.sw; ti.oy = -g.pby; ti.ox = -g.pbx; ti.C4 = g.C / 4;
 		ti.d_c4.init(ti.C4); ti.d_tw.init(ti.TW); ti.d_th.init(ti.TH);
-		hipLaunchKernelGGL(wino_input_kernel, dim3(blocks_exact((size_t)T * ti.C4, 256)), dim3(256), 0, stream, (const float*)a.p + (long)n0 * a.sn, V, ti);
+		if (bits) {
+			WinoMaskOut mo;
+			mo.bits = (unsigned char*)bits; mo.GYn = tl_share.GYn; mo.GXn = tl_share.GXn; mo.KB = tl_share.KB;
+			hipLaunchKernelGGL(HIP_KERNEL_NAME(wino_input_kernel<true>), dim3(blocks_exact((size_t)T * ti.C4, 256)), dim3(256), 0, stream, (const float*)a.p + (long)n0 * a.sn, V, ti, mo);
+			tl_share.bits = bits; tl_share.bits_off = p.total();
+			__atomic_fetch_add(&g_back_shared[1], 1L, __ATOMIC_RELAXED);
+		} else hipLaunchKernelGGL(HIP_KERNEL_NAME(wino_input_kernel<false>), dim3(blocks_exact((size_t)T * ti.C4, 256)), dim3(256), 0, stream, (const float*)a.p + (long)n0 * a.sn, V, ti, WinoMaskOut());
 		HIP_ENFORCE(hipGetLastError());
 		ti.H = gr.h; ti.W = gr.w; ti.sn = gr.sn; ti.sh = gr.sh; ti.sw = gr.sw; ti.oy = 0; ti.ox = 0; ti.C4 = g.K / 4;
 		ti.d_c4.init(ti.C4);
 		const long blocks = ((long)T * (g.K / 4) + 255) / 256;
 		const float* const grs = (const float*)gr.p + (long)n0 * gr.sn;
-		if (fuse_bias) hipLaunchKernelGGL(HIP_KERNEL_NAME(wino_outgrad_kernel<true>), dim3((unsigned)blocks), dim3(256), 0, stream, grs, W, ti, BP);
+		if (Vg) {
+			ti.oy = -1; ti.ox = -1;
+			hipLaunchKernelGGL(wino_outgrad_both_kernel, dim3((unsigned)blocks), dim3(256), 0, stream, grs, Vg, W, ti, BP);
+			tl_share.v = Vg; tl_share.v_off = p.total();
+			__atomic_fetch_add(&g_back_shared[0], 1L, __ATOMIC_RELAXED);
+		} else if (fuse_bias) hipLaunchKernelGGL(HIP_KERNEL_NAME(wino_outgrad_kernel<true>), dim3((unsigned)blocks), dim3(256), 0, stream, grs, W, ti, BP);
 		else hipLaunchKernelGGL(HIP_KERNEL_NAME(wino_outgrad_kernel<false>), dim3((unsigned)blocks), dim3(256), 0, stream, grs, W, ti, (float*)0);
 		HIP_ENFORCE(hipGetLastError());
 		MatLoader<false, true> la, lb;
@@ -586,16 +632,25 @@
 	return CCV_NNC_EXEC_SUCCESS;
 }
 
+static bool conv_dgrad_takes_fused(const conv_geom_t& g, const Image4& gr, const Image4& h, const int algo, wino_fused_plan_t* fp)
+{
+	return algo != CONV_ALGO_IMPLICIT_GEMM && algo != CONV_ALGO_WINOGRAD && g.pby <= 2 && g.pbx <= 2 && g.pby >= 0 && g.pbx >= 0 && wino_fused_plan(g, gr, h, fp) && (algo == CONV_ALGO_WINOGRAD_FUSED || wino_fused_preferred(g.K, *fp, h));
+}
+static bool conv_dgrad_takes_wino(const conv_geom_t& g, const Image4& gr, const float* w, const Image4& h, const int algo, wino_plan_t* wp)
+{
+	return algo != CONV_ALGO_IMPLICIT_GEMM && wino_plan(g, g.H, g.W, g.K, g.C, wp) && wino_images_ok(gr, h, w, 0) && (algo >= CONV_ALGO_WINOGRAD || wino_preferred(*wp, g.K, g.C));
+}
+
 static int conv_dgrad_nhwc(const conv_geom_t& g, const Image4& gr, const float* w, const Image4& h, const int algo, const int flags, ccv_nnc_stream_context_t* const ctx)
 {
 	if (gr.sc != 1 || !pixel_linear(h) || !image_fits_int(gr)) return CCV_NNC_EXEC_INVALID;
 	wino_plan_t wp;
 	wino_fused_plan_t fp;
-	if (algo != CONV_ALGO_IMPLICIT_GEMM && algo != CONV_ALGO_WINOGRAD && g.pby <= 2 && g.pbx <= 2 && g.pby >= 0 && g.pbx >= 0 && wino_fused_plan(g, gr, h, &fp) && (algo == CONV_ALGO_WINOGRAD_FUSED || wino_fused_preferred(g.K, fp, h))) {
+	if (conv_dgrad_takes_fused(g, gr, h, algo, &fp)) {
 		const int r = conv_wino_fused_run<true>("conv_dgrad_wino_fused", g, fp, gr, w, 0, h, 2 - g.pby, 2 - g.pbx, ctx);
 		if (r != CCV_NNC_EXEC_OOM) return r;
 	}
-	if (algo != CONV_ALGO_IMPLICIT_GEMM && wino_plan(g, g.H, g.W, g.K, g.C, &wp) && wino_images_ok(gr, h, w, 0) && (algo >= CONV_ALGO_WINOGRAD || wino_preferred(wp, g.K, g.C))) {
+	if (conv_dgrad_takes_wino(g, gr, w, h, algo, &wp)) {
 		const int r = conv_wino_run<true>("conv_dgrad_wino", g, wp, gr, w, 0, h, 2 - g.pby, 2 - g.pbx, flags, ctx);
 		if (r != CCV_NNC_EXEC_OOM) return r;
 	}
@@ -631,6 +686,15 @@
 #undef CONV_DGRAD
 }
 
+static bool conv_wgrad_takes_fused(const conv_geom_t& g, const Image4& gr, const Image4& a, const float* dw, const int algo, wino_wgrad_fused_plan_t* wfp)
+{
+	return algo != CONV_ALGO_IMPLICIT_GEMM && algo != CONV_ALGO_WINOGRAD && wino_wgrad_fused_plan(g, wfp) && wino_wgrad_fused_images_ok(a, gr, dw) && wino_wgrad_fused_preferred(g);
+}
+static bool conv_wgrad_takes_wino(const conv_geom_t& g, const Image4& gr, const Image4& a, const float* dw, const int algo, wino_wgrad_plan_t* wp)
+{
+	return algo != CONV_ALGO_IMPLICIT_GEMM && wino_wgrad_plan(g, wp) && wino_images_ok(a, gr, dw, 0) && (algo >= CONV_ALGO_WINOGRAD || wino_preferred(wp->t, g.C, g.K));
+}
+
 static int conv_wgrad_nhwc(const conv_geom_t& g, const Image4& gr, const Image4& a, float* dw, float* dbias, bool* bias_done, const int algo, const int flags, ccv_nnc_stream_context_t* const ctx)
 {
 	if (bias_done) *bias_done = false;
@@ -641,12 +705,12 @@
 		if (r != CCV_NNC_EXEC_OOM) return r;
 	}
 	wino_wgrad_fused_plan_t wfp;
-	if (algo != CONV_ALGO_IMPLICIT_GEMM && algo != CONV_ALGO_WINOGRAD && wino_wgrad_fused_plan(g, &wfp) && wino_wgrad_fused_images_ok(a, gr, dw) && wino_wgrad_fused_preferred(g)) {
+	if (conv_wgrad_takes_fused(g, gr, a, dw, algo, &wfp)) {
 		const int r = conv_wino_wgrad_fused(g, wfp, gr, a, dw, dbias, bias_done, flags, ctx);
 		if (r != CCV_NNC_EXEC_OOM) return r;
 	}
 	wino_wgrad_plan_t wp;
-	if (algo != CONV_ALGO_IMPLICIT_GEMM && wino_wgrad_plan(g, &wp) && wino_images_ok(a, gr, dw, 0) && (algo >= CONV_ALGO_WINOGRAD || wino_preferred(wp.t, g.C, g.K))) {
+	if (conv_wgrad_takes_wino(g, gr, a, dw, algo, &wp)) {
 		const int r = conv_wino_wgrad(g, wp, gr, a, dw, dbias, bias_done, flags, ctx);
 		if (r != CCV_NNC_EXEC_OOM) return r;
 	}
@@ -873,6 +937,29 @@
 	if (h && cmd.algorithm != CONV_ALGO_IMPLICIT_GEMM && wino_fused_scratch_bound(g.C, g.K) + wino_fused_mask_bound(g) > inner) inner = wino_fused_scratch_bound(g.C, g.K) + wino_fused_mask_bound(g);
 	if (h && cmd.algorithm != CONV_ALGO_IMPLICIT_GEMM && conv_dgrad_parity_scratch(g) > inner) inner = conv_dgrad_parity_scratch(g);
 	if (dw && cmd.algorithm != CONV_ALGO_IMPLICIT_GEMM && g.C == 3 && conv_c3_wgrad_scratch_bound(g.K) > inner) inner = conv_c3_wgrad_scratch_bound(g.K);
+	back_share_t share = { 0, 0, 0, 0, 0, 0, 0, 0, 0 };
+	const long share_on = tune(TUNE_CONV_BACK_SHARE);
+	if (h && dw && a && w && share_on && !stage_io && !stage_w && g.pby == 1 && g.pbx == 1 && g.OH == g.H && g.OW == g.W && ai.sc == 1 && gi.sc == 1 && pixel_linear(gi) && pixel_linear(hi) && image_fits_int(ai) && image_fits_int(gi)
+		&& !(cmd.algorithm != CONV_ALGO_IMPLICIT_GEMM && conv_c3_ok(g, ai, gi))) {
+		wino_wgrad_fused_plan_t wf;
+		wino_wgrad_plan_t wg;
+		wino_fused_plan_t fp;
+		wino_plan_t wp;
+		if (!conv_wgrad_takes_fused(g, gi, ai, dw->data.f32, cmd.algorithm, &wf) && conv_wgrad_takes_wino(g, gi, ai, dw->data.f32, cmd.algorithm, &wg) && wino_slice_images(g.N, wg.t.TH * wg.t.TW, g.C, g.K) == g.N) {
+			if (conv_dgrad_takes_fused(g, gi, hi, cmd.algorithm, &fp)) {
+				tl_mask = ai;
+				if ((share_on & 2) && tl_mask_want && fp.GH == 2 && mask_fits(hi) && (long)fp.groups * fp.KB <= 0x7fffffffL && fp.uf_bytes <= wg.total()) {
+					share.want_bits = 1; share.GYn = fp.GYn; share.GXn = fp.GXn; share.KB = fp.KB;
+					if (wg.total() + (size_t)fp.groups * fp.KB * 1024 > inner) inner = wg.total() + (size_t)fp.groups * fp.KB * 1024;
+				}
+				tl_mask.p = 0;
+			} else if ((share_on & 1) && dbias && 256 % (g.K / 4) == 0 && conv_dgrad_takes_wino(g, gi, w->data.f32, hi, cmd.algorithm, &wp) && wp.TH == wg.t.TH && wp.TW == wg.t.TW && wp.u_bytes + wp.m_bytes <= wg.total()) {
+				share.want_v = 1;
+				if (wg.total() + wg.w_bytes > inner) inner = wg.total() + wg.w_bytes;
+			}
+		}
+	}
+	struct share_scope_t { share_scope_t(const back_share_t& s) { tl_share = s; } ~share_scope_t() { const back_share_t none = { 0, 0, 0, 0, 0, 0, 0, 0, 0 }; tl_share = none; } } share_scope(share);
 	WorkspaceScope ws(stream_context, ng + na + nh + nw + ndw, inner);
 	char* p = (char*)ws.prefix();
 	if ((ng + na + nh + nw + ndw) && !p) return CCV_NNC_EXEC_OOM;
@@ -1389,6 +1476,13 @@
 
 }
 
+extern "C" long nnc_mi355x_debug_conv_back_shared(int what) { return what == 0 || what == 1 ? __atomic_load_n(&g_back_shared[what], __ATOMIC_RELAXED) : 0; }
+extern "C" size_t nnc_mi355x_debug_conv_mask_bits(void* dst, size_t capacity)
+{
+	g_dbg_bits_dst = dst; g_dbg_bits_cap = capacity;
+	return g_dbg_bits_got;
+}
+
 extern "C" void _register_command_CCV_NNC_CONVOLUTION_FORWARD_backend_CCV_NNC_BACKEND_GPU_CUDNN(ccv_nnc_cmd_backend_registry_t* const registry)
 {
 	registry->tensor_formats = CCV_TENSOR_FORMAT_NCHW | CCV_TENSOR_FORMAT_NHWC;
diff --git a/ccv_amd/csrc/common.h b/ccv_amd/csrc/common.h
--- a/ccv_amd/csrc/common.h
+++ b/ccv_amd/csrc/common.h
@@ -220,6 +220,7 @@
 	TUNE_GEMM_BF16X3,
 	TUNE_BN_CLUSTER_SLOTS,
 	TUNE_GEMM_BATCH_XCD,
+	TUNE_CONV_BACK_SHARE,
 	TUNE_COUNT
 };
 static_assert(TUNE_GRID_WG_PER_CU == 3, "grid_for() above names this key by value");
diff --git a/ccv_amd/csrc/device_rt.cpp b/ccv_amd/csrc/device_rt.cpp
--- a/ccv_amd/csrc/device_rt.cpp
+++ b/ccv_amd/csrc/device_rt.cpp
@@ -128,8 +128,8 @@
 namespace nnc {
 int g_force_tile = 0;
 int g_force_splits = 0;
-static const char* const g_tune_names[TUNE_COUNT] = { "WINO_SLICE_KB", "WINO_FUSED_MAX_C", "WINO_FUSED_GRID", "GRID_WG_PER_CU", "WINO_WGRAD_FUSED_MAX", "GEMM_BUFFER_LOADS", "CONV_NCHW_HALF_F16", "BN_SMALL_PLANES", "SDPA_MFMA", "BN_CLUSTER", "GEMM_VEC_EPILOGUE", "POOL_ROWS", "GEMM_HALF_CHUNK8", "LSTM_PERSISTENT", "LSTM_ROWS", "GEMM_BF16X3", "BN_CLUSTER_SLOTS", "GEMM_BATCH_XCD" };
-static long g_tune_values[TUNE_COUNT] = { 0, 128, 0, 0, 128, 1, 32, 1, 1, 1, 1, 1, 1, 1, 1, 1, 0, 1 };
+static const char* const g_tune_names[TUNE_COUNT] = { "WINO_SLICE_KB", "WINO_FUSED_MAX_C", "WINO_FUSED_GRID", "GRID_WG_PER_CU", "WINO_WGRAD_FUSED_MAX", "GEMM_BUFFER_LOADS", "CONV_NCHW_HALF_F16", "BN_SMALL_PLANES", "SDPA_MFMA", "BN_CLUSTER", "GEMM_VEC_EPILOGUE", "POOL_ROWS", "GEMM_HALF_CHUNK8", "LSTM_PERSISTENT", "LSTM_ROWS", "GEMM_BF16X3", "BN_CLUSTER_SLOTS", "GEMM_BATCH_XCD", "CONV_BACK_SHARE" };
+static long g_tune_values[TUNE_COUNT] = { 0, 128, 0, 0, 128, 1, 32, 1, 1, 1, 1, 1, 1, 1, 1, 1, 0, 1, 3 };
 static int g_tune_env_read = 0;
 long tune(int key)
 {
diff --git a/ccv_amd/csrc/wino_fused.h b/ccv_amd/csrc/wino_fused.h
--- a/ccv_amd/csrc/wino_fused.h
+++ b/ccv_amd/csrc/wino_fused.h
@@ -492,6 +492,7 @@
 {
 	constexpr int GWL = GW == 4 ? 2 : (GW == 8 ? 3 : (GW == 2 ? 1 : (GW == 16 ? 4 : 0)));
 	static_assert(GH * GW == 16, "16 tiles per group");
+	static_assert(WF_KT == WINO_MASK_KT, "winograd.h describes this layout");
 	int b = (int)blockIdx.x;
 	const int kb = b % KB; b /= KB;
 	const int gx = b % GXn; b /= GXn;
@@ -503,9 +504,8 @@
 	unsigned m = 0;
 #pragma unroll
 	for (int e = 0; e < 8; e++) {
-		const int pid = e * 8 + (lane >> 3);
-		const int gp = pid >> 4, px = pid & 15;
-		const int tile = 4 * gp + r;
+		const int pid = wino_mask_pid(e, lane), px = pid & 15;
+		const int tile = wino_mask_tile(pid, r);
 		const int oy = (gy * GH + (tile >> GWL)) * 4 + (px >> 2), ox = (gx * GW + (tile & (GW - 1))) * 4 + (px & 3);
 		if ((kq < K) & (oy < OH) & (ox < OW)) {
 			const float4 v = *(const float4*)(mp + (long)oy * m_sh + (long)ox * m_sw);
diff --git a/ccv_amd/csrc/wino_wgrad_fused.h b/ccv_amd/csrc/wino_wgrad_fused.h
--- a/ccv_amd/csrc/wino_wgrad_fused.h
+++ b/ccv_amd/csrc/wino_wgrad_fused.h
@@ -38,7 +38,7 @@
 {
 	__shared__ __attribute__((aligned(16))) float lds[2 * WG_STAGE_BYTES / 4 + 256];
 	const int t = threadIdx.x, lane = t & 63;
-	const int wave = __builtin_amdgcn_readfirstlane(t >> 6);
+	const int wave = __builtin_amdgcn_readfirstlane(t >> 6) & 3;
 	const int wk = wave >> 1, wc = wave & 1;
 	const int ch = lane & 15, slot = lane >> 4;
 	const int nb = p.kblocks * p.cblocks;
diff --git a/ccv_amd/csrc/winograd.h b/ccv_amd/csrc/winograd.h
--- a/ccv_amd/csrc/winograd.h
+++ b/ccv_amd/csrc/winograd.h
@@ -114,7 +114,22 @@
 	FastDiv d_c4, d_tw, d_th;
 };
 
-static __global__ void __launch_bounds__(256) wino_input_kernel(const float* __restrict__ a, float* __restrict__ v, const WinoTiles g)
+constexpr int WINO_MASK_KT = 32;
+__host__ __device__ __forceinline__ long wino_mask_item(const long n, const int gy, const int gx, const int kb, const int GYn, const int GXn, const int KB) { return ((n * GYn + gy) * GXn + gx) * KB + kb; }
+__host__ __device__ __forceinline__ int wino_mask_pid(const int e, const int lane) { return e * 8 + (lane >> 3); }
+__host__ __device__ __forceinline__ int wino_mask_tile(const int pid, const int r) { return 4 * (pid >> 4) + r; }
+__host__ __device__ __forceinline__ int wino_mask_round(const int tile) { return tile & 3; }
+__host__ __device__ __forceinline__ int wino_mask_pid_of(const int tile, const int px) { return 16 * (tile >> 2) + px; }
+__host__ __device__ __forceinline__ int wino_mask_nibble(const int pid) { return pid >> 3; }
+__host__ __device__ __forceinline__ int wino_mask_lane(const int pid, const int q8) { return (pid & 7) * 8 + q8; }
+
+struct WinoMaskOut {
+	unsigned char* bits;
+	int GYn, GXn, KB;
+};
+
+template <bool MASK>
+static __global__ void __launch_bounds__(256) wino_input_kernel(const float* __restrict__ a, float* __restrict__ v, const WinoTiles g, const WinoMaskOut mo)
 {
 	const long idx = (long)nnc_xcd_block(blockIdx.x, gridDim.x) * blockDim.x + threadIdx.x;
 	if (idx >= (long)g.T * g.C4) return;
@@ -124,6 +139,7 @@
 	const int y0 = ty * 4 + g.oy, x0 = tx * 4 + g.ox;
 	const float* const src = a + (long)n * g.sn + (long)c4 * 4;
 	f4 s[6][6];
+	unsigned mb[8];
 #pragma unroll
 	for (int r = 0; r < 6; r++) {
 		const int y = y0 + r;
@@ -135,7 +151,26 @@
 			const bool ok = yok & (x >= 0) & (x < g.W);
 			d[q] = ok ? f4(*(const float4*)(src + (long)y * g.sh + (long)x * g.sw)) : f4(0.f, 0.f, 0.f, 0.f);
 		}
+		if (MASK && r >= 1 && r <= 4) {
+#pragma unroll
+			for (int q = 0; q < 4; q++) {
+				const f4 m = d[q + 1];
+				const unsigned nib = (m.x > 0.f ? 1u : 0u) | (m.y > 0.f ? 2u : 0u) | (m.z > 0.f ? 4u : 0u) | (m.w > 0.f ? 8u : 0u);
+				const int px = 4 * (r - 1) + q;
+				if (px < 8) mb[px] = nib; else mb[px - 8] |= nib << 4;
+			}
+		}
 		wino_bt(d, s[r]);
+	}
+	if (MASK) {
+		const int gy = ty >> 1, gx = tx >> 3, tile = (ty & 1) * 8 + (tx & 7);
+		const long item = wino_mask_item(n, gy, gx, c4 >> 3, mo.GYn, mo.GXn, mo.KB);
+		unsigned char* const bp = mo.bits + (item * 256 + wino_mask_round(tile) * 64) * 4;
+#pragma unroll
+		for (int j = 0; j < 8; j++) {
+			const int pid = wino_mask_pid_of(tile, j);
+			bp[wino_mask_lane(pid, c4 & 7) * 4 + (wino_mask_nibble(pid) >> 1)] = (unsigned char)mb[j];
+		}
 	}
 	const long plane = (long)g.T * g.C4 * 4;
 	float* const dst = v + idx * 4;
@@ -241,6 +276,69 @@
 	}
 }
 
+static __global__ void __launch_bounds__(256) wino_outgrad_both_kernel(const float* __restrict__ gr, float* __restrict__ v, float* __restrict__ wt, const WinoTiles g, float* __restrict__ blockpart)
+{
+	__shared__ float4 red[256];
+	const unsigned block = nnc_xcd_block(blockIdx.x, gridDim.x);
+	const long idx = (long)block * blockDim.x + threadIdx.x;
+	const bool live = idx < (long)g.T * g.C4;
+	f4 sum(0.f, 0.f, 0.f, 0.f);
+	if (live) {
+		const int t = g.d_c4.div((int)idx), k4 = (int)(idx - (long)t * g.C4);
+		const int tn = g.d_tw.div(t), tx = t - tn * g.TW;
+		const int n = g.d_th.div(tn), ty = tn - n * g.TH;
+		const int y0 = ty * 4 + g.oy, x0 = tx * 4 + g.ox;
+		const float* const src = gr + (long)n * g.sn + (long)k4 * 4;
+		const long plane = (long)g.T * g.C4 * 4;
+		f4 s[6][6];
+		f4 sg[4][6];
+#pragma unroll
+		for (int r = 0; r < 6; r++) {
+			const int y = y0 + r;
+			const bool yok = (y >= 0) & (y < g.H);
+			f4 d[6];
+#pragma unroll
+			for (int q = 0; q < 6; q++) {
+				const int x = x0 + q;
+				const bool ok = yok & (x >= 0) & (x < g.W);
+				d[q] = ok ? f4(*(const float4*)(src + (long)y * g.sh + (long)x * g.sw)) : f4(0.f, 0.f, 0.f, 0.f);
+			}
+			wino_bt(d, s[r]);
+			if (r >= 1 && r <= 4) {
+				const f4 m[4] = { d[1], d[2], d[3], d[4] };
+#pragma unroll
+				for (int q = 0; q < 4; q++) sum = sum + m[q];
+				wino_g4(m, sg[r - 1]);
+			}
+		}
+		float* const dst = v + idx * 4;
+#pragma unroll
+		for (int q = 0; q < 6; q++) {
+			const f4 col[6] = { s[0][q], s[1][q], s[2][q], s[3][q], s[4][q], s[5][q] };
+			f4 y[6];
+			wino_bt(col, y);
+#pragma unroll
+			for (int r = 0; r < 6; r++) *(float4*)(dst + (long)(r * 6 + q) * plane) = y[r];
+		}
+		float* const dstw = wt + idx * 4;
+#pragma unroll
+		for (int q = 0; q < 6; q++) {
+			const f4 col[4] = { sg[0][q], sg[1][q], sg[2][q], sg[3][q] };
+			f4 y[6];
+			wino_g4(col, y);
+#pragma unroll
+			for (int r = 0; r < 6; r++) *(float4*)(dstw + (long)(r * 6 + q) * plane) = y[r];
+		}
+	}
+	red[threadIdx.x] = (float4)sum;
+	__syncthreads();
+	if ((int)threadIdx.x < g.C4) {
+		f4 acc(0.f, 0.f, 0.f, 0.f);
+		for (int j = threadIdx.x; j < 256; j += g.C4) acc = acc + f4(red[j]);
+		*(float4*)(blockpart + ((long)block * g.C4 + threadIdx.x) * 4) = (float4)acc;
+	}
+}
+
 static __global__ void __launch_bounds__(256) wino_wgrad_final_kernel(const float* __restrict__ du, float* __restrict__ dw, const int K, const int C, const int accumulate)
 {
 	const long idx = (long)blockIdx.x * blockDim.x + threadIdx.x;
diff --git a/include/nnc_mi355x.h b/include/nnc_mi355x.h
--- a/include/nnc_mi355x.h
+++ b/include/nnc_mi355x.h
@@ -297,6 +297,8 @@
 int  nnc_mi355x_profile_get(int i, char* name, int name_len, double* flops, double* bytes, float* ms, int dims[5]);
 void nnc_mi355x_debug_force_tile(int wm, int wn);
 void nnc_mi355x_debug_force_splits(int splits);
+size_t nnc_mi355x_debug_conv_mask_bits(void* dst, size_t capacity);
+long nnc_mi355x_debug_conv_back_shared(int what);
 size_t nnc_mi355x_lstm_reserve_space_size(const ccv_nnc_cmd_t cmd, int datatype, int feature_size, int batch_count, int max_seq_count);
 int nnc_mi355x_depalettize(const void* input, int datatype, size_t input_length, int qbits, int number_in_blocks, void* output, size_t output_length, ccv_nnc_stream_context_t* stream_context);
 size_t nnc_mi355x_palettized_bytes(int datatype, size_t count, int qbits, int number_in_blocks);
```

Result: faster. 3397 images/s (median of 6 runs) (+1.5%).
